# antofuller/jumbo_mae_tpu

Measured on AMD Instinct MI355X. Metric: pretrain images/sec (whole node) ViT-L/16 224 mask75% at 1/2/4/8 MI355X, higher is better.
Workload: dtype bf16; 1 GPU; model=vit_large_patch16 jumbo-MAE (3 CLS, shared jumbo MLP) + decoder 8x512x16h, global_batch=4096, seq_len=52, decoder_seq_len=199, parallelism=dp1, per_gpu_batch=4096, grad_accum=2, micro_batch=2048, grad_ckpt=False, hip_graph=False, optimizer=adamw(0.9,0.95) wd0.05 warmup-cosine

## Files before the change

jumbo_mae_tpu_amd/csrc/bindings.cpp:

```cpp
#include <torch/extension.h>
#include <c10/hip/HIPStream.h>
#include <hip/hip_runtime.h>

#include <climits>

#include "jm_api.h"

namespace {

hipStream_t stream() { return c10::hip::getCurrentHIPStream().stream(); }

#define CHECK_CUDA(x) TORCH_CHECK((x).is_cuda(), #x " must be a GPU tensor")
#define CHECK_CONTIG(x) TORCH_CHECK((x).is_contiguous(), #x " must be contiguous")
#define CHECK_DT(x, d) TORCH_CHECK((x).scalar_type() == (d), #x " has wrong dtype")

const uint16_t* bf(const torch::Tensor& t) { return reinterpret_cast<const uint16_t*>(t.data_ptr()); }
uint16_t* bfm(torch::Tensor& t) { return reinterpret_cast<uint16_t*>(t.data_ptr()); }
uint16_t* bfp(const torch::Tensor& t) { return reinterpret_cast<uint16_t*>(t.data_ptr()); }
const float* fopt(const c10::optional<torch::Tensor>& t) {
  return t.has_value() && t->defined() ? t->data_ptr<float>() : nullptr;
}
float* fopt_m(c10::optional<torch::Tensor>& t) { return t.has_value() && t->defined() ? t->data_ptr<float>() : nullptr; }

void check_rc(int rc, const char* what) { TORCH_CHECK(rc == 0, what, ": unsupported shape (rc=", rc, ")"); }
// ... 40 lines not shown
  return {y, mean, rstd};
}

std::vector<torch::Tensor> layernorm_bwd(torch::Tensor dy, torch::Tensor x, torch::Tensor mean, torch::Tensor rstd,
                                         torch::Tensor gamma, torch::Tensor dgamma, torch::Tensor dbeta, bool accum,
                                         c10::optional<torch::Tensor> dres, c10::optional<torch::Tensor> out,
                                         c10::optional<torch::Tensor> res_y, c10::optional<torch::Tensor> res_scale,
                                         c10::optional<torch::Tensor> res_mask, c10::optional<torch::Tensor> res_dscale,
                                         c10::optional<torch::Tensor> res_dbias, int64_t res_T0,
                                         c10::optional<torch::Tensor> res_out, c10::optional<torch::Tensor> res_seed,
                                         double res_rate, int64_t res_ioff, c10::optional<torch::Tensor> hx,
                                         c10::optional<torch::Tensor> beta) {
  CHECK_CONTIG(dy);
  TORCH_CHECK(x.dim() == 3 && x.stride(2) == 1, "x must be [B,T,D]");
  const int B = x.size(0), T = x.size(1), D = x.size(2);
  TORCH_CHECK(dy.numel() == (long)B * T * D, "dy shape");
  torch::Tensor dx;
  if (out.has_value() && out->defined()) {
    dx = *out;
    TORCH_CHECK(dx.dim() == 3 && dx.size(0) == B && dx.size(1) == T && dx.size(2) == D && dx.stride(2) == 1, "out view");
  } else {
    dx = torch::empty({B, T, D}, x.options());
  }
  const float* rp = nullptr;
  long rB = 0, rT = 0;
  if (dres.has_value() && dres->defined()) {
    TORCH_CHECK(dres->dim() == 3 && dres->size(0) == B && dres->size(1) == T && dres->stride(2) == 1, "dres view");
    rp = dres->data_ptr<float>();
    rB = dres->stride(0);
    rT = dres->stride(1);
  }
  const bool dyb = dy.scalar_type() == torch::kBFloat16;
  TORCH_CHECK(dyb || dy.scalar_type() == torch::kFloat32, "dy dtype");
  const bool has_res = res_y.has_value() && res_y->defined();
  JmLnRes res{};
  torch::Tensor dyr;
  if (has_res) {
    const int Tr = T - (int)res_T0;
    TORCH_CHECK(res_T0 >= 0 && Tr > 0, "res_T0");
    const auto& y = *res_y;
    CHECK_DT(y, torch::kBFloat16);
    long yB, yT;
    if (y.dim() == 3) {
      TORCH_CHECK(y.size(0) == B && y.size(1) == Tr && y.size(2) == D && y.stride(2) == 1, "res_y view");
      yB = y.stride(0);
      yT = y.stride(1);
    } else {
      TORCH_CHECK(y.is_contiguous() && y.numel() == (long)B * Tr * D, "res_y shape");
      yB = (long)Tr * D;
      yT = D;
    }
    if (res_out.has_value() && res_out->defined()) {
      dyr = *res_out;
      CHECK_DT(dyr, torch::kBFloat16);
      TORCH_CHECK(dyr.sizes() == y.sizes() && dyr.strides() == y.strides(), "res_out must match res_y's view");
    } else {
      TORCH_CHECK(y.is_contiguous(), "res_y view needs res_out");
      dyr = torch::empty_like(y);
    }
    res = JmLnRes{bf(y), bfm(dyr), yB, yT, fopt(res_scale), fopt(res_mask), (int)res_T0, fopt_m(res_dscale),
                  fopt_m(res_dbias), make_drop(res_seed, res_rate, y, res_ioff)};
  }
  const uint16_t* hxp = nullptr;
  const float* betap = nullptr;
  if (hx.has_value() && hx->defined()) {
    CHECK_DT((*hx), torch::kBFloat16);
    CHECK_CONTIG((*hx));
    TORCH_CHECK(hx->numel() == (long)B * T * D, "hx shape");
    TORCH_CHECK(beta.has_value() && beta->defined() && beta->numel() == D, "hx needs beta [D]");
    CHECK_DT((*beta), torch::kFloat32);
    hxp = bf(*hx);
    betap = beta->data_ptr<float>();
  }
  const int NP = has_res ? 4 : 2;
  auto ws = torch::empty({(accum || has_res) ? (long)jm_layernorm_bwd_blocks(B * T, D) * NP * D : 1}, x.options());
  check_rc(jm_layernorm_bwd(dy.data_ptr(), dyb, x.data_ptr<float>(), x.stride(0), x.stride(1), B, T, D,
                            mean.data_ptr<float>(), rstd.data_ptr<float>(), gamma.data_ptr<float>(),
                            dx.data_ptr<float>(), dx.stride(0), dx.stride(1), rp, rB, rT, dgamma.data_ptr<float>(),
                            dbeta.data_ptr<float>(), accum, ws.data_ptr<float>(), has_res ? &res : nullptr,
                            stream(), hxp, betap),
           "layernorm_bwd");
  if (has_res) return {dx, dyr};
  return {dx};
}

torch::Tensor gelu_fwd(torch::Tensor h) {
  CHECK_CONTIG(h);
  CHECK_DT(h, torch::kBFloat16);
  auto a = torch::empty_like(h);
  check_rc(jm_gelu_fwd(bf(h), bfm(a), h.numel(), stream()), "gelu_fwd");
  return a;
}

static torch::Tensor rowcol_ws(const torch::Tensor& like, int M, int N, int nacc) {
  const long n = jm_rowcol_ws_floats(M, N, nacc);
  return torch::empty({n > 0 ? n : 1}, like.options().dtype(torch::kFloat32));
}

torch::Tensor gelu_bwd(torch::Tensor h, torch::Tensor da, c10::optional<torch::Tensor> bias_grad, bool deriv) {
  CHECK_CONTIG(h);
  CHECK_CONTIG(da);
  CHECK_DT(h, torch::kBFloat16);
  CHECK_DT(da, torch::kBFloat16);
  const int N = h.size(-1);
  const int M = h.numel() / N;
  auto dh = torch::empty_like(h);
  float* bg = fopt_m(bias_grad);
  torch::Tensor ws;
  if (bg) ws = rowcol_ws(h, M, N, 1);
  check_rc(jm_gelu_bwd(bf(h), bf(da), bfm(dh), bg, M, N, stream(), deriv ? 1 : 0, bg ? ws.data_ptr<float>() : nullptr),
           "gelu_bwd");
  return dh;
}

void colsum(torch::Tensor x, torch::Tensor acc) {
  CHECK_CONTIG(x);
  CHECK_DT(x, torch::kBFloat16);
  const int N = x.size(-1);
  const int M = x.numel() / N;
  auto ws = rowcol_ws(x, M, N, 1);
  check_rc(jm_colsum_bf16(bf(x), acc.data_ptr<float>(), M, N, stream(), ws.data_ptr<float>()), "colsum");
}

void splitk_reduce_add(torch::Tensor part, torch::Tensor g) {
  CHECK_CONTIG(part);
  TORCH_CHECK(g.is_contiguous() && g.numel() * part.size(0) == part.numel(), "splitk_reduce_add shapes");
  check_rc(jm_splitk_reduce_add(part.data_ptr<float>(), g.data_ptr<float>(), g.numel(), part.size(0), stream()),
           "splitk_reduce_add");
}

void colsum_add_f32(torch::Tensor x, torch::Tensor g) {
  CHECK_CUDA(x);
  CHECK_DT(x, torch::kFloat32);
  CHECK_DT(g, torch::kFloat32);
  TORCH_CHECK(x.dim() == 2 && x.stride(1) == 1 && g.is_contiguous() && g.numel() == x.size(1),
              "colsum_add_f32: x [rows, n] with unit column stride, g [n]");
  TORCH_CHECK(reinterpret_cast<uintptr_t>(x.data_ptr()) % 16 == 0 && reinterpret_cast<uintptr_t>(g.data_ptr()) % 16 == 0,
              "colsum_add_f32: 16-byte aligned operands");
  check_rc(jm_colsum_add_f32(x.data_ptr<float>(), x.stride(0), x.size(0), x.size(1), g.data_ptr<float>(), stream()),
           "colsum_add_f32");
}

torch::Tensor residual_fwd(torch::Tensor x, torch::Tensor y, c10::optional<torch::Tensor> scale,
                           c10::optional<torch::Tensor> mask, c10::optional<torch::Tensor> out_opt,
                           c10::optional<torch::Tensor> seed, double rate, int64_t ioff) {
  TORCH_CHECK(x.dim() == 3 && x.stride(2) == 1, "x must be [B,T,D]");
  CHECK_DT(x, torch::kFloat32);
  CHECK_CONTIG(y);
  CHECK_DT(y, torch::kBFloat16);
  const int B = x.size(0), T = x.size(1), D = x.size(2);
  torch::Tensor out;
  if (out_opt.has_value() && out_opt->defined()) {
    out = *out_opt;
    TORCH_CHECK(out.dim() == 3 && out.size(0) == B && out.size(1) == T && out.size(2) == D && out.stride(2) == 1,
                "out view");
  } else {
    out = torch::empty({B, T, D}, x.options());
  }
  check_rc(jm_residual_fwd(x.data_ptr<float>(), x.stride(0), x.stride(1), B, T, D, bf(y), fopt(scale), fopt(mask),
                           out.data_ptr<float>(), out.stride(0), out.stride(1), stream(),
                           make_drop(seed, rate, y, ioff)),
           "residual_fwd");
  return out;
}

torch::Tensor residual_bwd(torch::Tensor dout, c10::optional<torch::Tensor> y, c10::optional<torch::Tensor> scale,
// ... 311 lines not shown
  CHECK_CONTIG(y);
  CHECK_DT(y, torch::kBFloat16);
  CHECK_CONTIG(tok);
  CHECK_CONTIG(pos);
  CHECK_DT(tok, torch::kFloat32);
  CHECK_DT(pos, torch::kFloat32);
  const long sb = ids_bstride(ids_restore);
  const int B = y.size(0), d = y.size(2), K = y.size(1) - C, N = pos.size(0);
  TORCH_CHECK(ids_restore.size(-1) == N && tok.numel() == d && pos.size(1) == d, "unshuffle_fwd shapes");
  auto out = torch::empty({B, C + N, d}, y.options().dtype(torch::kFloat32));
  check_rc(jm_unshuffle_fwd(bfp(y), tok.data_ptr<float>(), ids_restore.data_ptr<int>(), sb, pos.data_ptr<float>(),
                            out.data_ptr<float>(), B, C, K, N, d, stream()),
           "unshuffle_fwd");
  return out;
}

void zero_f32(torch::Tensor t) {
  CHECK_CUDA(t);
  CHECK_CONTIG(t);
  CHECK_DT(t, torch::kFloat32);
  jm_zero_f32(t.data_ptr<float>(), t.numel(), stream());
}

std::vector<torch::Tensor> mask_ids(torch::Tensor noise, int64_t keep) {
  CHECK_CUDA(noise);
  CHECK_CONTIG(noise);
  CHECK_DT(noise, torch::kFloat32);
  TORCH_CHECK(noise.dim() == 1 || noise.dim() == 2, "mask_ids: noise [N] or [R, N]");
  const int N = noise.size(-1), R = noise.dim() == 1 ? 1 : noise.size(0);
  TORCH_CHECK(N <= 1024 && keep >= 0 && keep <= N, "mask_ids: N <= 1024, 0 <= keep <= N");
  auto i64 = noise.options().dtype(torch::kInt64), i32 = noise.options().dtype(torch::kInt32);
  auto shuffle = torch::empty(noise.sizes(), i64), restore = torch::empty(noise.sizes(), i64);
  auto restore32 = torch::empty(noise.sizes(), i32), mask = torch::empty(noise.sizes(), noise.options());
  auto ks = noise.sizes().vec();
  ks.back() = keep;
  auto keep32 = torch::empty(ks, i32);
  check_rc(jm_mask_ids(noise.data_ptr<float>(), R, N, (int)keep, shuffle.data_ptr<int64_t>(),
                       restore.data_ptr<int64_t>(), keep32.data_ptr<int>(), restore32.data_ptr<int>(),
                       mask.data_ptr<float>(), stream()),
           "mask_ids");
  return {shuffle, restore, keep32, restore32, mask};
}

std::vector<torch::Tensor> unshuffle_bwd(torch::Tensor dout, torch::Tensor ids_restore, int64_t C, int64_t K) {
  CHECK_CONTIG(dout);
  CHECK_DT(dout, torch::kFloat32);
  const long sb = ids_bstride(ids_restore);
  const int B = dout.size(0), N = dout.size(1) - C, d = dout.size(2);
  TORCH_CHECK(ids_restore.size(-1) == N, "unshuffle_bwd shapes");
  const int rpb = 64;
  const int nb = jm_unshuffle_bwd_blocks(B, C, N, rpb);
  auto dy = torch::empty({B, C + K, d}, dout.options().dtype(torch::kBFloat16));
  auto part = torch::empty({nb, d}, dout.options().dtype(torch::kFloat64));
  check_rc(jm_unshuffle_bwd(dout.data_ptr<float>(), ids_restore.data_ptr<int>(), sb, bfp(dy), part.data_ptr<double>(), B,
                            C, K, N, d, rpb, stream()),
           "unshuffle_bwd");
  return {dy, part.sum(0, true).to(torch::kFloat32)};
}

torch::Tensor mix_patches(torch::Tensor img, c10::optional<torch::Tensor> perm, c10::optional<torch::Tensor> prm,
                          c10::optional<torch::Tensor> box, int64_t p) {
  CHECK_CONTIG(img);
  CHECK_DT(img, torch::kUInt8);
  TORCH_CHECK(img.size(1) == 3, "mix_patches: 3 channels");
  const int B = img.size(0), H = img.size(2), W = img.size(3);
  const int* pp = nullptr;
  const float* pr = nullptr;
  const int* bx = nullptr;
  if (prm) {
    TORCH_CHECK(perm && box, "mix_patches: prm needs perm and box");
    CHECK_DT((*perm), torch::kInt32);
    CHECK_DT((*prm), torch::kFloat32);
    CHECK_DT((*box), torch::kInt32);
    TORCH_CHECK(perm->numel() == B && prm->numel() >= 2 && box->numel() == 4, "mix_patches: param sizes");
    pp = perm->data_ptr<int>();
    pr = prm->data_ptr<float>();
    bx = box->data_ptr<int>();
  }
  auto out = torch::empty({(long)B * (H / p) * (W / p), 3 * p * p}, img.options().dtype(torch::kBFloat16));
  check_rc(jm_mix_patches(img.data_ptr<uint8_t>(), pp, pr, bx, bfp(out), B, H, W, p, stream()), "mix_patches");
  return out;
}

torch::Tensor patch_mse_fwd(torch::Tensor pred, torch::Tensor img, int64_t p, bool norm_pix) {
  CHECK_DT(pred, torch::kBFloat16);
  TORCH_CHECK(pred.stride(1) == 1, "pred rows must be contiguous");
  CHECK_CONTIG(img);
  CHECK_DT(img, torch::kUInt8);
  const int H = img.size(2), W = img.size(3), N = (H / p) * (W / p);
  TORCH_CHECK(pred.size(0) == img.size(0) * N && pred.size(1) == 3 * p * p, "patch_mse_fwd shapes");
  auto mse = torch::empty({pred.size(0)}, pred.options().dtype(torch::kFloat32));
  check_rc(jm_patch_mse_fwd(bfp(pred), pred.stride(0), img.data_ptr<uint8_t>(), mse.data_ptr<float>(), pred.size(0), N,
                            H, W, p, norm_pix, stream()),
           "patch_mse_fwd");
  return mse;
}

torch::Tensor patch_mse_bwd(torch::Tensor pred, torch::Tensor img, torch::Tensor dmse, int64_t p, bool norm_pix) {
  CHECK_DT(pred, torch::kBFloat16);
  TORCH_CHECK(pred.stride(1) == 1, "pred rows must be contiguous");
  CHECK_CONTIG(img);
  CHECK_CONTIG(dmse);
  CHECK_DT(dmse, torch::kFloat32);
  const int H = img.size(2), W = img.size(3), N = (H / p) * (W / p);
  TORCH_CHECK(dmse.numel() == pred.size(0) && pred.size(0) == img.size(0) * N && pred.size(1) == 3 * p * p,
              "patch_mse_bwd shapes");
  auto dpred = torch::empty({pred.size(0), pred.size(1)}, pred.options());
  check_rc(jm_patch_mse_bwd(bfp(pred), pred.stride(0), img.data_ptr<uint8_t>(), dmse.data_ptr<float>(), bfp(dpred),
                            pred.size(0), N, H, W, p, norm_pix, stream()),
           "patch_mse_bwd");
  return dpred;
}

std::vector<torch::Tensor> recon(torch::Tensor pred, torch::Tensor images, torch::Tensor mask, int64_t p, bool norm_pix,
                                 int64_t fill, c10::optional<std::vector<torch::Tensor>> out) {
  CHECK_CUDA(pred);
  CHECK_CUDA(images);
  CHECK_CUDA(mask);
  TORCH_CHECK(images.device() == pred.device() && mask.device() == pred.device(), "recon: tensors on one device");
  TORCH_CHECK(pred.scalar_type() == torch::kBFloat16 || pred.scalar_type() == torch::kFloat32,
              "recon: pred must be bf16 or fp32");
  CHECK_DT(images, torch::kUInt8);
  CHECK_DT(mask, torch::kFloat32);
  CHECK_CONTIG(pred);
  CHECK_CONTIG(images);
  CHECK_CONTIG(mask);
  TORCH_CHECK(pred.dim() == 2, "recon: pred [B*N, 3p^2]");
  TORCH_CHECK(images.dim() == 4 && images.size(1) == 3, "recon: images [B, 3, H, W]");
  TORCH_CHECK(fill >= 0 && fill <= 255, "recon: fill is a byte");
  const int64_t B = images.size(0), H = images.size(2), W = images.size(3);
  TORCH_CHECK(p > 0 && p % 2 == 0, "recon: patch size must be positive and even, got ", p);
  TORCH_CHECK(H > 0 && W > 0 && H % p == 0 && W % p == 0, "recon: image ", H, " x ", W,
              " is not a whole number of ", p, " x ", p, " patches");
  TORCH_CHECK(H <= INT_MAX && W <= INT_MAX && B <= INT_MAX, "recon: image batch too large");
  const int64_t N = (H / p) * (W / p);
  TORCH_CHECK(B * N <= INT_MAX, "recon: too many patches");
  TORCH_CHECK(pred.size(0) == B * N && pred.size(1) == 3 * p * p, "recon: pred must be [", B * N, ", ", 3 * p * p,
              "], got [", pred.size(0), ", ", pred.size(1), "]");
  TORCH_CHECK((mask.dim() == 1 && mask.size(0) == N) || (mask.dim() == 2 && mask.size(0) == B && mask.size(1) == N),
              "recon: mask must be [", N, "] or [", B, ", ", N, "]");
  const long maskB = mask.dim() == 1 ? 0 : (long)N;
  torch::Tensor rec, paste, masked, err;
  if (out.has_value()) {
    TORCH_CHECK(out->size() == 4, "recon: out = (recon, paste, masked, err)");
    for (int i = 0; i < 3; ++i) {
      const auto& t = (*out)[i];
      TORCH_CHECK(t.is_cuda() && t.device() == pred.device() && t.scalar_type() == torch::kUInt8 &&
                      t.is_contiguous() && t.sizes() == images.sizes(),
                  "recon: out[", i, "] must be a contiguous uint8 tensor shaped like images");
    }
    const auto& e = (*out)[3];
    TORCH_CHECK(e.is_cuda() && e.device() == pred.device() && e.scalar_type() == torch::kFloat32 &&
                    e.is_contiguous() && e.dim() == 2 && e.size(0) == B && e.size(1) == N,
                "recon: out[3] must be a contiguous fp32 [B, N] tensor");
    rec = (*out)[0], paste = (*out)[1], masked = (*out)[2], err = e;
  } else {
    rec = torch::empty_like(images);
    paste = torch::empty_like(images);
    masked = torch::empty_like(images);
    err = torch::empty({B, N}, images.options().dtype(torch::kFloat32));
  }
  check_rc(jm_recon(pred.data_ptr(), pred.scalar_type() == torch::kBFloat16, images.data_ptr<uint8_t>(),
                    mask.data_ptr<float>(), maskB, rec.data_ptr<uint8_t>(), paste.data_ptr<uint8_t>(),
                    masked.data_ptr<uint8_t>(), err.data_ptr<float>(), (int)B, (int)H, (int)W, (int)p, norm_pix,
                    (int)fill, stream()),
           "recon");
  return {rec, paste, masked, err};
}

}

int attach_tail(GemmEpi& ep, torch::Tensor& ws, int M, int N, int K, int epi, const torch::Tensor& like) {
  int r = 0;
  long n = 0;
  const int S = jm_gemm_nt_tail_plan(M, N, K, epi, like.stride(0), &r, &n);
  if (S < 2) return 0;
  ws = torch::empty({n}, like.options().dtype(torch::kFloat32));
  ep.tail = ws.data_ptr<float>();
  ep.tail_S = S;
  ep.t_count = r;
  return r;
}

std::vector<torch::Tensor> gemm_nt(torch::Tensor A, torch::Tensor B, c10::optional<torch::Tensor> bias, bool gelu,
                                   bool gelu_only, bool gelu_deriv, c10::optional<torch::Tensor> seed, double rate) {
  CHECK_DT(A, torch::kBFloat16);
  CHECK_DT(B, torch::kBFloat16);
  TORCH_CHECK(A.dim() == 2 && B.dim() == 2 && A.size(1) == B.size(1), "gemm_nt: A [M,K], B [N,K]");
  TORCH_CHECK(A.stride(1) == 1 && B.stride(1) == 1, "gemm_nt: K must be contiguous");
  const int M = A.size(0), N = B.size(0), K = A.size(1);
  TORCH_CHECK(!gelu_deriv || N % 8 == 0, "gemm_nt: gelu_deriv needs N % 8 == 0");
  auto out = torch::empty({M, N}, gelu_deriv ? A.options().dtype(torch::kUInt8) : A.options());
// ... 372 lines not shown
  segs.n = nb;
  int S = 1;
  const int sps = jm_gemm_tn_plan(grp, M, &S);
  torch::Tensor part;
  if (S > 1) part = torch::empty({S * total}, gs[0].options());
  int64_t off = 0;
  for (int p = 0; p < np; ++p) {
    grp.out[p] = S > 1 ? part.data_ptr<float>() + off : gs[p].data_ptr<float>();
    off += (int64_t)S * grp.N[p] * grp.K[p];
  }
  const int all_store = group_stores(stores, gs, S, np);
  check_rc(jm_gemm_tn(grp, segmented ? &segs : nullptr, M, sps, S, stream(), all_store), what);
  if (S > 1)
    for (int p = 0; p < np; ++p)
      check_rc(jm_splitk_reduce_add(grp.out[p], gs[p].data_ptr<float>(), (long)grp.N[p] * grp.K[p], S, stream(),
                                    p < (int)stores.size() && stores[p]),
               what);
  return S;
}

int64_t gemm_tn_wgrad(torch::Tensor dy, torch::Tensor x, torch::Tensor g, bool store) {
  return tn_wgrad("gemm_tn_wgrad", {Tensors{dy}}, {Tensors{x}}, {g}, {store}, false);
}

int64_t gemm_tn_wgrad_seg(Tensors dys, Tensors xs, torch::Tensor g, bool store) {
  return tn_wgrad("gemm_tn_wgrad_seg", {dys}, {xs}, {g}, {store}, true);
}

int64_t gemm_tn_wgrad_group(Tensors dys, Tensors xs, Tensors gs, std::vector<bool> stores) {
  std::vector<Tensors> d, x;
  for (const auto& t : dys) d.push_back({t});
  for (const auto& t : xs) x.push_back({t});
  return tn_wgrad("gemm_tn_wgrad_group", d, x, gs, stores, false);
}

int64_t gemm_tn_wgrad_seg_group(std::vector<Tensors> dys, std::vector<Tensors> xs, Tensors gs,
                                std::vector<bool> stores) {
  return tn_wgrad("gemm_tn_wgrad_seg_group", dys, xs, gs, stores, true);
}

void zero_ranges(torch::Tensor base, torch::Tensor desc, int64_t blocks) {
  CHECK_CONTIG(base);
  CHECK_DT(base, torch::kFloat32);
  TORCH_CHECK(desc.is_cuda() && desc.scalar_type() == torch::kInt64 && desc.dim() == 2 && desc.size(1) == 2,
              "zero_ranges: desc int64 [n, 2] on the device");
  check_rc(jm_zero_ranges(base.data_ptr<float>(), reinterpret_cast<const long long*>(desc.data_ptr<int64_t>()),
                          (int)desc.size(0), blocks, stream()),
           "zero_ranges");
}

std::vector<torch::Tensor> residual_ln_fwd(torch::Tensor x, torch::Tensor y, c10::optional<torch::Tensor> scale,
                                           c10::optional<torch::Tensor> mask, torch::Tensor gamma,
                                           torch::Tensor beta, double eps, int64_t T0, int64_t R0,
                                           c10::optional<torch::Tensor> out, c10::optional<torch::Tensor> seed,
                                           double rate) {
  CHECK_CUDA(x);
  TORCH_CHECK(x.dim() == 3 && x.stride(2) == 1, "x must be [B,T,D] with contiguous last dim");
  CHECK_DT(x, torch::kFloat32);
  CHECK_DT(y, torch::kBFloat16);
  CHECK_CONTIG(y);
  const int B = x.size(0), T = x.size(1), D = x.size(2);
  TORCH_CHECK(R0 >= 0 && R0 < T, "residual_ln_fwd: R0");
  TORCH_CHECK(y.numel() == (long)B * (T - R0) * D, "residual_ln_fwd: y must be [B*(T-R0), D]");
  TORCH_CHECK(T0 >= 0 && T0 < T, "residual_ln_fwd: T0");
  TORCH_CHECK(R0 == 0 || out.has_value(), "residual_ln_fwd: R0 > 0 needs out (its rows t < R0 are inputs)");
  torch::Tensor x1;
  if (out) {
    CHECK_DT(*out, torch::kFloat32);
    TORCH_CHECK(out->dim() == 3 && out->size(0) == B && out->size(1) == T && out->size(2) == D && out->stride(2) == 1,
                "residual_ln_fwd: out must be [B,T,D] with contiguous last dim");
    x1 = *out;
  } else {
    x1 = torch::empty({B, T, D}, x.options());
  }
  const long R = (long)B * (T - T0);
  auto h = torch::empty({R, D}, y.options());
  auto mean = torch::empty({R}, x.options());
  auto rstd = torch::empty({R}, x.options());
  check_rc(jm_residual_ln_fwd(x.data_ptr<float>(), x.stride(0), x.stride(1), bf(y), fopt(scale), fopt(mask),
                              x1.data_ptr<float>(), x1.stride(0), x1.stride(1), bfm(h), mean.data_ptr<float>(),
                              rstd.data_ptr<float>(), B, T, T0, D, gamma.data_ptr<float>(), beta.data_ptr<float>(),
                              (float)eps, stream(), (int)R0, make_drop(seed, rate, y, 0)),
           "residual_ln_fwd");
  return {x1, h, mean, rstd};
}

static std::pair<const int*, const float*> check_cls_loss(const torch::Tensor& logits, const torch::Tensor& labels,
                                                          const c10::optional<torch::Tensor>& perm,
                                                          const c10::optional<torch::Tensor>& w, double smoothing,
                                                          int64_t mode) {
  CHECK_CUDA(logits);
  TORCH_CHECK(logits.scalar_type() == torch::kBFloat16 || logits.scalar_type() == torch::kFloat32,
              "cls_loss: logits must be bf16 or fp32");
  TORCH_CHECK(logits.dim() == 2 && logits.size(0) >= 1 && logits.size(1) >= 1, "cls_loss: logits must be [B, L]");
  TORCH_CHECK(logits.stride(1) == 1, "cls_loss: logits must have a unit column stride");
  TORCH_CHECK(logits.size(0) == 1 || logits.stride(0) >= logits.size(1), "cls_loss: logits rows must not overlap");
  TORCH_CHECK(logits.size(0) < INT_MAX && logits.size(1) < INT_MAX, "cls_loss: logits too large");
  const int64_t B = logits.size(0);
  TORCH_CHECK(labels.device() == logits.device() && labels.scalar_type() == torch::kInt64 && labels.dim() == 1 &&
                  labels.size(0) == B && labels.is_contiguous(),
              "cls_loss: labels must be int64 [B] on the logits' device");
  TORCH_CHECK(mode == 0 || mode == 1, "cls_loss: mode 0 (ce) or 1 (bce)");
  TORCH_CHECK(smoothing >= 0.0 && smoothing < 1.0, "cls_loss: smoothing must be in [0, 1)");
  const bool hp = perm.has_value() && perm->defined(), hw = w.has_value() && w->defined();
  TORCH_CHECK(hp == hw, "cls_loss: perm and w come together");
  if (!hp) return {nullptr, nullptr};
  TORCH_CHECK(perm->device() == logits.device() && perm->scalar_type() == torch::kInt32 && perm->dim() == 1 &&
                  perm->size(0) == B && perm->is_contiguous(),
              "cls_loss: perm must be int32 [B] on the logits' device");
  TORCH_CHECK(w->device() == logits.device() && w->scalar_type() == torch::kFloat32 && w->numel() == 1,
              "cls_loss: w must be one fp32 element on the logits' device");
  return {perm->data_ptr<int>(), w->data_ptr<float>()};
}

static long row_stride(const torch::Tensor& logits) { return logits.size(0) == 1 ? logits.size(1) : logits.stride(0); }

std::vector<torch::Tensor> cls_loss_fwd(torch::Tensor logits, torch::Tensor labels, c10::optional<torch::Tensor> perm,
                                        c10::optional<torch::Tensor> w, double smoothing, int64_t mode) {
  const auto pw = check_cls_loss(logits, labels, perm, w, smoothing, mode);
  const int64_t B = logits.size(0);
  auto loss = torch::empty({B}, logits.options().dtype(torch::kFloat32));
  auto hit = torch::empty({B, 2}, logits.options().dtype(torch::kBool));
  auto lse = torch::empty({B, 2}, logits.options().dtype(torch::kFloat32));
  check_rc(jm_cls_loss_fwd(logits.data_ptr(), logits.scalar_type() == torch::kBFloat16, row_stride(logits),
                           labels.data_ptr<int64_t>(), pw.first, pw.second, smoothing, (int)mode, (int)B,
                           (int)logits.size(1), loss.data_ptr<float>(), reinterpret_cast<uint8_t*>(hit.data_ptr()),
                           lse.data_ptr<float>(), stream()),
           "cls_loss_fwd");
  return {loss, hit, lse};
}

torch::Tensor cls_loss_bwd(torch::Tensor dloss, torch::Tensor logits, torch::Tensor labels,
                           c10::optional<torch::Tensor> perm, c10::optional<torch::Tensor> w, double smoothing,
                           int64_t mode, torch::Tensor lse) {
  const auto pw = check_cls_loss(logits, labels, perm, w, smoothing, mode);
  const int64_t B = logits.size(0), L = logits.size(1);
  TORCH_CHECK(lse.device() == logits.device() && lse.scalar_type() == torch::kFloat32 && lse.dim() == 2 &&
                  lse.size(0) == B && lse.size(1) == 2 && lse.is_contiguous(),
              "cls_loss_bwd: lse must be the forward's fp32 [B, 2]");
  TORCH_CHECK(dloss.device() == logits.device() && dloss.scalar_type() == torch::kFloat32 && dloss.dim() == 1 &&
                  dloss.size(0) == B && dloss.is_contiguous(),
              "cls_loss_bwd: dloss must be fp32 [B] on the logits' device");
  auto dlogits = torch::empty({B, L}, logits.options());
  check_rc(jm_cls_loss_bwd(logits.data_ptr(), logits.scalar_type() == torch::kBFloat16, row_stride(logits),
                           labels.data_ptr<int64_t>(), pw.first, pw.second, smoothing, (int)mode, (int)B, (int)L,
                           lse.data_ptr<float>(), dloss.data_ptr<float>(), dlogits.data_ptr(), L, stream()),
           "cls_loss_bwd");
  return dlogits;
}

static void check_bn_mat(const torch::Tensor& t, const char* fn, const char* what, bool bf16_ok) {
  TORCH_CHECK(t.scalar_type() == torch::kFloat32 || (bf16_ok && t.scalar_type() == torch::kBFloat16), fn, ": ", what,
              bf16_ok ? " must be bf16 or fp32" : " must be fp32");
  TORCH_CHECK(t.dim() == 2 && t.size(0) >= 1 && t.size(1) >= 1, fn, ": ", what, " must be [B, J]");
  TORCH_CHECK(t.stride(1) == 1, fn, ": ", what, " must have a unit column stride");
  TORCH_CHECK(t.size(0) == 1 || t.stride(0) >= t.size(1), fn, ": ", what, " rows must not overlap");
  TORCH_CHECK(t.size(0) < INT_MAX && t.size(1) < INT_MAX, fn, ": ", what, " too large");
}

static void check_bn_like(const torch::Tensor& t, const torch::Tensor& x, const char* fn, const char* what,
                          bool bf16_ok) {
  check_bn_mat(t, fn, what, bf16_ok);
  TORCH_CHECK(t.size(0) == x.size(0) && t.size(1) == x.size(1), fn, ": ", what, " must have the shape of x");
}

static void check_bn_vec(const torch::Tensor& t, int64_t n, const char* fn, const char* what, const char* shape) {
// ... 303 lines not shown
  m.def("rrc_resize", &rrc_resize, py::arg("src"), py::arg("tab"), py::arg("size"), py::arg("tmp_bytes"),
        py::arg("tmp_rows_max"));
  m.def("rrc_kmax", &jm_rrc_kmax);
  m.def("window_resize", &window_resize, py::arg("src"), py::arg("tab"), py::arg("size"), py::arg("tmp_bytes"),
        py::arg("tmp_rows_max"));
  m.def("window_tab", &jm_window_tab);
  m.def("aug_chain", &aug_chain, py::arg("images"), py::arg("chain"), py::arg("scratch"));
  m.def("augmix_mix", &augmix_mix, py::arg("orig"), py::arg("chains"), py::arg("table"), py::arg("blended"));
  m.def("erase_paste", &erase_paste, py::arg("images"), py::arg("table"), py::arg("fill"),
        py::arg("box_bytes_max") = 0);
  m.def("gelu_drop", &gelu_drop, py::arg("a"), py::arg("b") = py::none(), py::arg("seed"), py::arg("rate"));
  m.def("softmax_dropout_fwd", &softmax_dropout_fwd);
  m.def("softmax_dropout_bwd", &softmax_dropout_bwd);
  m.def("gelu_bwd", &gelu_bwd, py::arg("h"), py::arg("da"), py::arg("bias_grad") = py::none(),
        py::arg("deriv") = false);
  m.def("colsum", &colsum);
  m.def("splitk_reduce_add", &splitk_reduce_add);
  m.def("residual_ln_fwd", &residual_ln_fwd, py::arg("x"), py::arg("y"), py::arg("scale"), py::arg("mask"),
        py::arg("gamma"), py::arg("beta"), py::arg("eps"), py::arg("T0"), py::arg("R0") = 0,
        py::arg("out") = py::none(), py::arg("seed") = py::none(), py::arg("rate") = 0.0);
  m.def("transpose_bf16", &transpose_bf16);
  m.def("residual_fwd", &residual_fwd, py::arg("x"), py::arg("y"), py::arg("scale"), py::arg("mask"),
        py::arg("out") = py::none(), py::arg("seed") = py::none(), py::arg("rate") = 0.0, py::arg("ioff") = 0);
  m.def("residual_bwd", &residual_bwd, py::arg("dout"), py::arg("y"), py::arg("scale"), py::arg("mask"),
        py::arg("dscale"), py::arg("ydtype"), py::arg("dbias") = py::none(), py::arg("out") = py::none(),
        py::arg("seed") = py::none(), py::arg("rate") = 0.0, py::arg("ioff") = 0);
  m.def("attn_fwd", &attn_fwd, py::arg("qkv"), py::arg("heads"), py::arg("seed") = py::none(), py::arg("rate") = 0.0);
  m.def("attn_bwd", &attn_bwd, py::arg("dO"), py::arg("qkv"), py::arg("o"), py::arg("lse"), py::arg("heads"),
        py::arg("dbias") = py::none(), py::arg("seed") = py::none(), py::arg("rate") = 0.0);
  m.def("attn_max_seq", &jm_attn_max_seq);
  m.def("attn_head_dims", &attn_head_dims);
  m.def("attn_fused_bias", &attn_fused_bias, py::arg("S"), py::arg("hd"));
  m.def("attn_dropout", &attn_dropout, py::arg("S"), py::arg("hd"));
  m.def("gemm_tn_wgrad", &gemm_tn_wgrad, py::arg("dy"), py::arg("x"), py::arg("g"), py::arg("store") = false);
  m.def("gemm_tn_wgrad_seg", &gemm_tn_wgrad_seg, py::arg("dys"), py::arg("xs"), py::arg("g"), py::arg("store") = false);
  m.def("zero_ranges", &zero_ranges, "zero float ranges of a flat buffer (one launch)");
  m.def("colsum_add_f32", &colsum_add_f32, "g += x.sum(0) for a row-strided fp32 [rows, n] view");
  m.def("gemm_tn_wgrad_seg_group", &gemm_tn_wgrad_seg_group, py::arg("dys"), py::arg("xs"), py::arg("gs"),
        py::arg("stores") = std::vector<bool>{}, "grouped segmented weight gradients (<= 2 problems)");
  m.def("gemm_tn_wgrad_group", &gemm_tn_wgrad_group, py::arg("dys"), py::arg("xs"), py::arg("gs"),
        py::arg("stores") = std::vector<bool>{}, "grouped weight gradients over one M (<= 4 problems)");
  m.def("gemm_test_force", &jm_gemm_test_force, py::arg("path"), py::arg("rows") = 0,
        "numerics tests only: NT GEMM kernel path 0 = by shape, 1 = 64-deep main loop everywhere, "
        "2 = 4-phase kernels at every M without tail split (rows = forced tile height)");
  m.def("gemm_nt_tiles", &jm_gemm_nt_tiles, py::arg("M"), py::arg("N"), py::arg("K") = 1024, py::arg("epi") = 0,
        py::arg("lda") = 0, "output tiles (workgroups before split-K) of an NT launch");
  m.def(
      "gemm_nt_tail_plan",
      [](int M, int N, int K, int epi, long lda) {
        int r = 0;
        long n = 0;
        const int S = jm_gemm_nt_tail_plan(M, N, K, epi, lda, &r, &n);
        return std::make_pair(S, r);
      },
      py::arg("M"), py::arg("N"), py::arg("K"), py::arg("epi") = 0, py::arg("lda") = 0,
      "(S, tail tiles) of the tail split of an NT launch (S = 0: none); read-only");
  m.def("transpose_bf16_batch", &transpose_bf16_batch);
  m.def("gemm_nt_splitk", &gemm_nt_splitk, py::arg("A"), py::arg("B"), py::arg("bias") = py::none(),
        py::arg("splits") = 8, py::arg("add") = py::none());
  m.def("gemm_nt_dgelu", &gemm_nt_dgelu, py::arg("A"), py::arg("B"), py::arg("pre"), py::arg("dbias") = py::none(),
        py::arg("deriv") = false, py::arg("rate") = 0.0);
  m.def("gemm_nt_f32", &gemm_nt_f32, py::arg("A"), py::arg("B"));
  m.def("gemm_nt", &gemm_nt, py::arg("A"), py::arg("B"), py::arg("bias") = py::none(), py::arg("gelu") = false,
        py::arg("gelu_only") = false, py::arg("gelu_deriv") = false, py::arg("seed") = py::none(),
        py::arg("rate") = 0.0);
  m.def("opt_sumsq", &opt_sumsq);
  m.def("opt_adamw", &opt_adamw);
  m.def("opt_lamb_phase1", &opt_lamb_phase1);
  m.def("opt_lars_norms", &opt_lars_norms);
  m.def("opt_apply_trust", &opt_apply_trust);
  m.def("opt_sgd", &opt_sgd);
  m.def("opt_ema", &opt_ema, py::arg("master"), py::arg("ema"), py::arg("rows"), py::arg("meta"),
        py::arg("ema_hyper"));
  m.def("ema_swap", &ema_swap, py::arg("master"), py::arg("ema"), py::arg("shadow"), py::arg("rows"));
  m.def("opt_seg_stats", &opt_seg_stats, py::arg("master"), py::arg("grad"), py::arg("p_old"), py::arg("rows"),
        py::arg("meta"), py::arg("out") = py::none());
  m.def("patchify_normalize", &patchify_normalize);
  m.def("gather_patches", &gather_patches);
  m.def("embed_finish", &embed_finish);
  m.def("zero_f32", &zero_f32, "fp32 zero fill kernel (the store-mode gradients' pre-reduce fill)");
  m.def("mask_ids", &mask_ids, "random-masking permutation ids + mask from noise (one workgroup per row)");
  m.def("unshuffle_fwd", &unshuffle_fwd);
  m.def("unshuffle_bwd", &unshuffle_bwd);
  m.def("patch_mse_fwd", &patch_mse_fwd);
  m.def("mix_patches", &mix_patches);
  m.def("patch_mse_bwd", &patch_mse_bwd);
  m.def("recon", &recon, py::arg("pred"), py::arg("images"), py::arg("mask"), py::arg("p"), py::arg("norm_pix"),
        py::arg("fill") = 127, py::arg("out") = py::none(),
        "MAE reconstruction panels -> (recon, paste, masked uint8 [B, 3, H, W], err fp32 [B, N])");
  m.def("cls_loss_fwd", &cls_loss_fwd, py::arg("logits"), py::arg("labels"), py::arg("perm") = py::none(),
        py::arg("w") = py::none(), py::arg("smoothing") = 0.0, py::arg("mode") = 0);
  m.def("cls_loss_bwd", &cls_loss_bwd, py::arg("dloss"), py::arg("logits"), py::arg("labels"),
        py::arg("perm"), py::arg("w"), py::arg("smoothing"), py::arg("mode"), py::arg("lse"));
  m.def("knn_topk", &knn_topk, py::arg("q"), py::arg("bank"), py::arg("k"), py::arg("self_idx") = py::none(),
        py::arg("splits") = 0, py::arg("out_idx") = py::none(), py::arg("out_sim") = py::none(),
        "fused similarity + top-k -> (idx int32, sim fp32) [Nq, k], ties by ascending bank index");
  m.def("knn_splits", &jm_knn_splits, py::arg("Nq"), py::arg("Nb"), py::arg("splits") = 0,
        "bank slices of a knn_topk launch");
  m.def("knn_vote", &knn_vote, py::arg("idx"), py::arg("sim"), py::arg("bank_labels"), py::arg("labels"), py::arg("T"),
        "weighted k-NN vote -> (pred int32 [Nq, 5], hit1, hit5 bool [Nq])");
  m.def("bn_stats", &bn_stats, py::arg("x"));
  m.def("bn_apply", &bn_apply, py::arg("x"), py::arg("packed"), py::arg("gamma"), py::arg("beta"),
        py::arg("running_mean"), py::arg("running_var"), py::arg("eps"), py::arg("momentum"), py::arg("out_dtype"),
        py::arg("out") = py::none());
  m.def("bn_apply_eval", &bn_apply_eval, py::arg("x"), py::arg("running_mean"), py::arg("running_var"),
        py::arg("gamma"), py::arg("beta"), py::arg("eps"), py::arg("out_dtype"), py::arg("out") = py::none());
  m.def("bn_bwd_reduce", &bn_bwd_reduce, py::arg("dy"), py::arg("x"), py::arg("stats"), py::arg("gamma"),
        py::arg("dgamma") = py::none(), py::arg("dbeta") = py::none());
  m.def("bn_bwd_dx", &bn_bwd_dx, py::arg("dy"), py::arg("x"), py::arg("stats"), py::arg("gamma"), py::arg("packed_g"),
        py::arg("n"), py::arg("out") = py::none());
  m.def("bn_chunk_rows", &jm_bn_chunk_rows, "rows per workgroup of the BatchNorm kernels");
  m.def("bn_block_cols", &jm_bn_block_cols, "columns per workgroup of the BatchNorm kernels");
  m.def("attn_stats", &attn_stats, py::arg("qkv"), py::arg("heads"), py::arg("n_cls"),
        py::arg("rows_out") = py::none(), "per-head attention statistics, fp64 [H, 6]");
  m.def("debug_lines", &debug_lines);
  m.def("debug_selftest", &debug_selftest);
#ifdef JM_DEBUG
  m.attr("debug_build") = true;
#else
  m.attr("debug_build") = false;
#endif
}
```

jumbo_mae_tpu_amd/csrc/jm_api.h:

```cpp
#pragma once
#include <cstddef>
#include <cstdint>

#include <hip/hip_runtime.h>

struct JmDrop {
  const int64_t* seed;
  uint32_t thr;
  float scale;
  long ioff;
};

struct JmLnRes {
  const uint16_t* y;
  uint16_t* dy;
  long yB, yT;
  const float* scale;
  const float* mask;
  int T0;
  float* dscale;
  float* dbias;
  JmDrop drop;
};

struct TnGroup {
  const uint16_t* a[4];
  const uint16_t* b[4];
  long lda[4], ldb[4];
  int N[4], K[4];
  float* out[4];
  int tile0[5];
  int n;
};

struct TnSegs {
  const uint16_t* a[64];
  const uint16_t* b[64];
  int rows;
  int n;
};

struct GemmEpi {
  const float* bias;
  uint16_t* out;
  long ldo;
  uint16_t* out2;
  const uint16_t* aux;
  float* colpart;
  float* part;
  int splits;
  float* tail;
  int tail_S;
  int t_begin;
  int t_count;
  const int64_t* dseed;
  uint32_t dthr;
  float dscale;
  uint8_t* dq;
  const uint8_t* dqa;
  float dqs;
};


int jm_layernorm_fwd(const float* x, long sB, long sT, int B, int T, int D, const float* gamma, const float* beta,
                     float eps, void* y, int out_bf16, float* mean, float* rstd, hipStream_t st, uint16_t* y2 = nullptr);
int jm_layernorm_bwd(const void* dy, int dy_bf16, const float* x, long sB, long sT, int B, int T, int D,
                     const float* mean, const float* rstd, const float* gamma, float* dx_ptr, long oB, long oT,
                     const float* dres, long rB, long rT, float* dgamma, float* dbeta, int accum_params, float* ws,
                     const JmLnRes* res, hipStream_t st, const uint16_t* hx = nullptr,
                     const float* beta = nullptr);
int jm_layernorm_bwd_blocks(int rows, int D);
int jm_residual_ln_fwd(const float* x, long sB, long sT, const uint16_t* y, const float* scale, const float* mask,
                       float* x1, long oB, long oT, uint16_t* h, float* mean, float* rstd, int B, int T, int T0,
                       int D, const float* gamma, const float* beta, float eps, hipStream_t st, int R0 = 0,
                       JmDrop drop = JmDrop{nullptr, 0u, 1.f, 0});
int jm_debug_line_layernorm();

int jm_gelu_fwd(const uint16_t* h, uint16_t* a, long n, hipStream_t st);
long jm_rowcol_ws_floats(int M, int N, int nacc);
int jm_gelu_bwd(const uint16_t* h, const uint16_t* da, uint16_t* dh, float* bias_grad, int M, int N, hipStream_t st,
                int deriv, float* ws);
int jm_colsum_bf16(const uint16_t* x, float* acc, int M, int N, hipStream_t st, float* ws);
int jm_residual_fwd(const float* x, long sB, long sT, int B, int T, int D, const uint16_t* y, const float* scale,
                    const float* mask, float* out, long oB, long oT, hipStream_t st, JmDrop drop);
int jm_residual_bwd(const float* dout, long dB, long dT, const uint16_t* y, const float* scale, const float* mask,
                    float* dscale, uint16_t* dy, int B, int T, int D, float* dbias, long yB, long yT, hipStream_t st,
                    JmDrop drop, float* ws);
void jm_zero_f32(float* p, long n, hipStream_t st);
int jm_splitk_reduce_add(const float* part, float* g, long n, int S, hipStream_t st, int store = 0);
int jm_colsum_add_f32(const float* x, long ld, int rows, long n, float* g, hipStream_t st);
int jm_zero_ranges(float* base, const long long* desc, int n, long long blocks, hipStream_t st);
int jm_transpose_bf16(const uint16_t* src, uint16_t* dst, int R, int C, hipStream_t st);
int jm_transpose_bf16_batch(const long long* desc, int n, int tiles, hipStream_t st);
int jm_splitk_reduce_bf16(const float* part, int S, long n, int N, const float* bias, uint16_t* out, hipStream_t st);
int jm_splitk_reduce_f32(const float* part, int S, int M, int N, const float* bias, const float* add, long add_ld,
                         float* out, hipStream_t st);
int jm_debug_line_elementwise();
void jm_debug_selftest(int v, hipStream_t st);

int jm_attn_fwd(const uint16_t* qkv, uint16_t* o, float* lse, int B, int S, int H, int hd, const int64_t* dseed,
                uint32_t dthr, float dscale, hipStream_t st);
int jm_attn_bwd(const uint16_t* qkv, const uint16_t* o, const uint16_t* dO, const float* lse, uint16_t* dqkv, int B,
                int S, int H, int hd, float* dbias_part, const int64_t* dseed, uint32_t dthr, float dscale,
                hipStream_t st);
int jm_attn_bwd_long(const uint16_t* qkv, const uint16_t* o, const uint16_t* dO, const float* lse, uint16_t* dqkv,
                     float* delta, int B, int S, int H, int hd, const int64_t* dseed, uint32_t dthr, float dscale,
                     hipStream_t st);
int jm_attn_max_seq();
int jm_attn_head_dims(const int** dims);
int jm_attn_tiled(int S, int hd);
int jm_attn_fused_bias(int S, int hd);
int jm_attn_bwd_part_rows(int B, int S, int hd);
int jm_attn_dropout(int S, int hd);
int jm_debug_line_attention();

void jm_opt_sumsq(const float* x, const int* chunks, int nchunks, float* out, float* cpart, hipStream_t st);
void jm_opt_adamw(float* p, const float* g, float* mu, float* nu, uint16_t* shadow, const int* chunks, int nchunks,
                  const float* meta, const float* hyper, const float* gnorm_sq, hipStream_t st);
void jm_opt_lamb_phase1(const float* p, const float* g, float* mu, float* nu, float* u, const int* chunks, int nchunks,
                        const float* meta, const float* hyper, const float* gnorm_sq, float* norms, float* cpart,
                        hipStream_t st);
void jm_opt_lars_norms(const float* p, const float* g, const int* chunks, int nchunks, const float* hyper,
                       const float* gnorm_sq, float* norms, float* cpart, hipStream_t st);
void jm_opt_apply_trust(float* p, const float* u_or_g, float* trace, uint16_t* shadow, const int* chunks, int nchunks,
                        const float* meta, const float* hyper, const float* norms, const float* gnorm_sq, int mode,
                        float momentum, float trust_coef, hipStream_t st);
void jm_opt_sgd(float* p, const float* g, float* trace, uint16_t* shadow, const int* chunks, int nchunks,
                const float* meta, const float* hyper, const float* gnorm_sq, float momentum, hipStream_t st);
void jm_opt_ema(const float* p, float* ema, const int* chunks, int nchunks, const float* meta, int nseg,
                const float* ema_hyper, long n, hipStream_t st);
void jm_ema_swap(float* p, float* ema, uint16_t* shadow, const int* chunks, int nchunks, long n, hipStream_t st);
constexpr int JM_SEG_STATS_COLS = 7;
void jm_opt_seg_stats(const float* p, const float* g, const float* p_old, const int* chunks, int nchunks,
                      const float* meta, int nseg, long n, double* part, double* out, hipStream_t st);
int jm_debug_line_optim();

int jm_patchify_normalize(const uint8_t* img, float* out, int B, int H, int W, int p, hipStream_t st);
int jm_gather_patches(const uint8_t* img, const int* ids, long idsB, uint16_t* out, int B, int K, int H, int W, int p,
                      hipStream_t st);
int jm_embed_finish(const uint16_t* e, const float* pos, const int* ids, long idsB, const float* cls, float* out,
                    int B, int C, int K, int D, hipStream_t st);
int jm_mask_ids(const float* noise, int R, int N, int keep, int64_t* shuffle, int64_t* restore, int* keep32,
                int* restore32, float* mask, hipStream_t st);
int jm_unshuffle_fwd(const uint16_t* y, const float* tok, const int* restore, long rsB, const float* pos, float* out,
                     int B, int C, int K, int N, int d, hipStream_t st);
int jm_unshuffle_bwd_blocks(int B, int C, int N, int rows_per_block);
int jm_unshuffle_bwd(const float* dout, const int* restore, long rsB, uint16_t* dy, double* part, int B, int C, int K,
                     int N, int d, int rows_per_block, hipStream_t st);
int jm_mix_patches(const uint8_t* img, const int* perm, const float* prm, const int* box, uint16_t* out, int B, int H,
                   int W, int p, hipStream_t st);
int jm_patch_mse_fwd(const uint16_t* pred, long ldp, const uint8_t* img, float* mse, long rows, int N, int H, int W,
                     int p, int norm_pix, hipStream_t st);
int jm_patch_mse_bwd(const uint16_t* pred, long ldp, const uint8_t* img, const float* dmse, uint16_t* dpred, long rows,
                     int N, int H, int W, int p, int norm_pix, hipStream_t st);
int jm_debug_line_mae();

int jm_recon(const void* pred, int pred_bf16, const uint8_t* img, const float* mask, long maskB, uint8_t* recon,
             uint8_t* paste, uint8_t* masked, float* err, int B, int H, int W, int p, int norm_pix, int fill,
             hipStream_t st);
int jm_debug_line_recon();

int jm_gemm_nt(const uint16_t* A, long lda, const uint16_t* B, long ldb, int M, int N, int K, int epi,
               const GemmEpi& ep, hipStream_t st);
int jm_gemm_nt_tiles(int M, int N, int K, int epi, long lda);
int jm_gemm_nt_colpart_rows(int M, int N, int K, int epi, long lda);
int jm_gemm_nt_tail_plan(int M, int N, int K, int epi, long lda, int* tail_r, long* ws_floats);
void jm_gemm_test_force(int path, int rows);
int jm_debug_line_gemm();

size_t jm_gemm_tn_smem();
int jm_gemm_tn_plan(const TnGroup& grp, int M, int* S_out);
int jm_gemm_tn(const TnGroup& grp, const TnSegs* segs, int M, int sps, int S, hipStream_t st, int store);
int jm_debug_line_gemm_tn();

int jm_dropout_apply(const void* x, void* y, long n, int bf16, const int64_t* seed, uint32_t thr, float scale,
                     hipStream_t st);
int jm_gelu_drop(const uint16_t* h, uint16_t* g, uint16_t* gp, long n, const int64_t* seed, uint32_t thr, float scale,
                 hipStream_t st);
int jm_softmax_dropout_fwd(const float* z, float* p, float* pd, long rows, int S, const int64_t* seed, uint32_t thr,
                           float scale, hipStream_t st);
int jm_softmax_dropout_bwd(const float* dpd, const float* p, float* dz, long rows, int S, const int64_t* seed,
                           uint32_t thr, float scale, hipStream_t st);
int jm_debug_line_dropout();

int jm_rrc_resize(const uint8_t* src, const int64_t* tab, int B, int S, uint8_t* tmp, int tmp_rows_max, uint8_t* out,
                  hipStream_t st);
int jm_window_resize(const uint8_t* src, const int64_t* tab, int B, int S, uint8_t* tmp, int tmp_rows_max,
                     uint8_t* out, hipStream_t st);
int jm_window_tab();
int jm_rrc_kmax();
int jm_debug_line_augment();

int jm_aug_stat_words();
int jm_aug_record_len();
int jm_aug_chain(uint8_t* images, uint8_t* scratch, const double* chain, int B, int slots, int S, uint32_t* stats,
                 hipStream_t st);
int jm_augmix_mix(const uint8_t* orig, const uint8_t* chains, const float* table, uint8_t* out, int B, int W, int S,
                  int blended, hipStream_t st);
int jm_erase_paste(uint8_t* images, const int64_t* table, const uint8_t* fill, long fill_len, int B, int S,
                   long box_bytes_max, hipStream_t st);
int jm_debug_line_augment_chain();

int jm_cls_loss_fwd(const void* logits, int bf16, long ld, const int64_t* labels, const int* perm, const float* w,
                    double smoothing, int mode, int B, int L, float* loss, uint8_t* hit, float* lse, hipStream_t st);
int jm_cls_loss_bwd(const void* logits, int bf16, long ld, const int64_t* labels, const int* perm, const float* w,
                    double smoothing, int mode, int B, int L, const float* lse, const float* dloss, void* dlogits,
                    long ldo, hipStream_t st);
int jm_debug_line_loss();

int jm_bn_chunks(int B);
int jm_bn_chunk_rows();
int jm_bn_block_cols();
int jm_bn_stats(const float* x, long ld, int B, int J, double* part, float* packed, hipStream_t st);
int jm_bn_apply(const float* x, long ld, int B, int J, const float* packed, const float* gamma, const float* beta,
                double eps, double momentum, void* y, int y_bf16, long ldy, float* stats, float* running_mean,
                float* running_var, hipStream_t st);
int jm_bn_apply_eval(const float* x, long ld, int B, int J, const float* running_mean, const float* running_var,
                     const float* gamma, const float* beta, double eps, void* y, int y_bf16, long ldy,
                     hipStream_t st);
int jm_bn_bwd_reduce(const void* dy, int dy_bf16, long lddy, const float* x, long ld, int B, int J,
                     const float* stats, const float* gamma, double* part, float* dgamma, float* dbeta, int accum,
                     float* packed_g, hipStream_t st);
int jm_bn_bwd_dx(const void* dy, int dy_bf16, long lddy, const float* x, long ld, int B, int J, const float* stats,
                 const float* gamma, const float* packed_g, double n, float* dx, long lddx, hipStream_t st);
int jm_debug_line_batchnorm();

int jm_knn_splits(int Nq, int Nb, int splits);
int jm_knn_topk(const void* q, long ldq, const void* bank, long ldb, const int* self_idx, int Nq, int Nb, int D, int k,
                int splits, int* idx, float* sim, int* sidx, float* ssim, hipStream_t st);
int jm_knn_vote(const int* idx, const float* sim, const int* bank_labels, const int* labels, double T, int Nq, int Nb,
                int k, int* pred, uint8_t* hit1, uint8_t* hit5, hipStream_t st);
int jm_debug_line_knn();

constexpr int JM_ATTN_STATS_COLS = 6;
long jm_attn_stats_part(int B, int S, int H);
int jm_attn_stats(const void* qkv, int B, int S, int H, int hd, int n_cls, double* part, float* rows_out,
                  hipStream_t st);
// ... 3 lines not shown
```

jumbo_mae_tpu_amd/csrc/layernorm.hip:

```cpp
#include <type_traits>

#include "common.h"
#include "jm_api.h"

namespace {

template <int V, typename TO>
__global__ __launch_bounds__(256) void ln_fwd_kernel(const float* __restrict__ x, long sB, long sT, int T,
                                                     int rows, int D, const float* __restrict__ gamma,
                                                     const float* __restrict__ beta, float eps,
                                                     TO* __restrict__ y, float* __restrict__ mean_out,
                                                     float* __restrict__ rstd_out, uint16_t* __restrict__ y2) {
  const int wave = threadIdx.x >> 6, lane = threadIdx.x & 63;
  const int row = blockIdx.x * 4 + wave;
  if (row >= rows) return;
  const int b = row / T, t = row - b * T;
  const float* xr = x + b * sB + t * sT;
  float v[V][4];
  float s = 0.f;
#pragma unroll
  for (int i = 0; i < V; ++i) {
    const int col = (i * 64 + lane) * 4;
    if (col < D) {
      load4(xr + col, v[i]);
// ... 48 lines not shown
  float* mean;
  float* rstd;
  DropIO drop;
};

template <int V>
__global__ __launch_bounds__(256) void res_ln_fwd_kernel(ResLnIO io, int T, int T0, int R0, int rows, int D,
                                                         const float* __restrict__ gamma,
                                                         const float* __restrict__ beta, float eps) {
  const int wave = threadIdx.x >> 6, lane = threadIdx.x & 63;
  const int row = blockIdx.x * 4 + wave;
  if (row >= rows) return;
  const int b = row / T, t = row - b * T;
  const bool rrow = t >= R0;
  float* x1r = io.x1 + b * io.oB + t * io.oT;
  const float* xr = rrow ? io.x + b * io.sB + t * io.sT : x1r;
  const uint16_t* yr = io.y + ((long)b * (T - R0) + (t - R0)) * D;
  const float m = io.mask ? io.mask[b] : 1.f;
  float v[V][4];
  float s = 0.f;
#pragma unroll
  for (int i = 0; i < V; ++i) {
    const int col = (i * 64 + lane) * 4;
    if (col < D) {
      float xv[4];
      load4(xr + col, xv);
      if (rrow) {
        float yv[4], sc[4] = {1.f, 1.f, 1.f, 1.f};
        load4(yr + col, yv);
        if (io.scale) load4(io.scale + col, sc);
        if (io.drop.seed) {
          float f[4];
          drop_factors<4>(io.drop, io.drop.ioff + (yr - io.y) + col, f);
#pragma unroll
          for (int j = 0; j < 4; ++j) yv[j] *= f[j];
        }
#pragma unroll
        for (int j = 0; j < 4; ++j) v[i][j] = xv[j] + m * sc[j] * yv[j];
        store4(x1r + col, v[i]);
      } else {
#pragma unroll
        for (int j = 0; j < 4; ++j) v[i][j] = xv[j];
      }
    } else {
      v[i][0] = v[i][1] = v[i][2] = v[i][3] = 0.f;
    }
    s += v[i][0] + v[i][1] + v[i][2] + v[i][3];
  }
  if (t < T0) return;
  const float mean = wave_sum(s) / D;
  float s2 = 0.f;
#pragma unroll
  for (int i = 0; i < V; ++i) {
    const int col = (i * 64 + lane) * 4;
    if (col < D) {
#pragma unroll
      for (int j = 0; j < 4; ++j) {
        const float d = v[i][j] - mean;
        s2 += d * d;
      }
    }
  }
  const float rstd = rsqrtf(wave_sum(s2) / D + eps);
  const long hrow = (long)b * (T - T0) + (t - T0);
  uint16_t* hr = io.h + hrow * D;
#pragma unroll
  for (int i = 0; i < V; ++i) {
    const int col = (i * 64 + lane) * 4;
    if (col < D) {
      float gg[4], bb[4], o[4];
      load4(gamma + col, gg);
      load4(beta + col, bb);
#pragma unroll
      for (int j = 0; j < 4; ++j) o[j] = (v[i][j] - mean) * rstd * gg[j] + bb[j];
      store4(hr + col, o);
    }
  }
  if (lane == 0) {
    io.mean[hrow] = mean;
    io.rstd[hrow] = rstd;
  }
}

struct LnBwdIO {
  float* dx;
  long oB, oT;
  const float* dres;
  long rB, rT;
  const uint16_t* hx;
  const float* beta;
};

JM_DEVICE bool ln_h_ok(float g, float b) { return fabsf(g) >= 1e-20f && fabsf(b) <= fabsf(g); }

struct LnResIO {
  const uint16_t* y;
  uint16_t* dy;
  long yB, yT;
  const float* scale;
  const float* mask;
  int T0;
  DropIO drop;
};

struct ParamOuts {
  float* p[4];
};

template <int V, typename TI, bool RES, bool ER = false, bool SC = true, int R = 1>
__global__ __launch_bounds__(256) void ln_bwd_kernel(const TI* __restrict__ dy, const float* __restrict__ x,
                                                     long sB, long sT, int T, int rows, int D,
                                                     const float* __restrict__ mean, const float* __restrict__ rstd,
                                                     const float* __restrict__ gamma, LnBwdIO io, LnResIO rio,
                                                     float* __restrict__ ws, int accum_params, ParamOuts outs) {
  JM_DGUARD(blockDim.x == 256 && D % 4 == 0 && D <= V * 256);
  static_assert(R == 1 || R == 2, "rows per wave");
  constexpr int NP = RES ? 4 : 2;
  constexpr int LPR = 64 / R, VL = V * R;
  extern __shared__ __attribute__((aligned(16))) float red[];
  const int wave = threadIdx.x >> 6, lane = threadIdx.x & 63;
  const int sub = lane / LPR, l = lane % LPR;
  const bool partials = accum_params || RES;
  auto acc_add = [&](float (&acc)[NP][VL][4], int k, int i, int j, float v) { acc[k][i][j] += v; };
  auto row_sum = [&](float v) {
    if constexpr (R == 1) {
      return wave_sum(v);
    } else {
      v = row16_sum(v);
      const int iv = __builtin_bit_cast(int, v);
      const float lo = __builtin_bit_cast(float, __builtin_amdgcn_readlane(iv, 0)) +
                       __builtin_bit_cast(float, __builtin_amdgcn_readlane(iv, 16));
      const float hi = __builtin_bit_cast(float, __builtin_amdgcn_readlane(iv, 32)) +
                       __builtin_bit_cast(float, __builtin_amdgcn_readlane(iv, 48));
      return sub ? hi : lo;
    }
  };
  float acc[NP][VL][4], gg[VL][4], sc[VL][4];
  float* hbi = red + (partials ? NP * D : 0);
  const bool use_h = io.hx != nullptr;
  uint32_t xchunk = 0;
#pragma unroll
  for (int i = 0; i < VL; ++i) {
    const int col = (i * LPR + l) * 4;
#pragma unroll
    for (int j = 0; j < 4; ++j) {
#pragma unroll
      for (int k = 0; k < NP; ++k) acc[k][i][j] = 0.f;
      sc[i][j] = 1.f;
    }
    if (col < D) {
      load4(gamma + col, gg[i]);
      if constexpr (RES && SC) {
        if (rio.scale) load4(rio.scale + col, sc[i]);
      }
      if (use_h) {
        float bb[4], ig[4];
        load4(io.beta + col, bb);
        bool ok = true;
#pragma unroll
        for (int j = 0; j < 4; ++j) {
          ok = ok && ln_h_ok(gg[i][j], bb[j]);
          ig[j] = 1.f / gg[i][j];
        }
        if (!ok) xchunk |= 1u << i;
        if (wave == 0 && sub == 0) {
          store4(hbi + col, bb);
          store4(hbi + D + col, ig);
        }
      }
    }
  }
  const bool hpath = use_h && !__syncthreads_or(xchunk != 0u);
  auto row_loop = [&](auto hp) {
    constexpr bool HP = decltype(hp)::value;
    for (int rw = blockIdx.x * 4 + wave; rw * R < rows; rw += gridDim.x * 4) {
      const int row = rw * R + sub;
      const bool valid = R == 1 || row < rows;
      const int b = row / T, t = row - b * T;
      const float* xr = x + b * sB + t * sT;
      const TI* dyr = dy + (long)row * D;
      const float mu = valid ? mean[row] : 0.f, rs = valid ? rstd[row] : 0.f;
      const bool rrow = RES && t >= rio.T0;
      const long yoff = RES ? b * rio.yB + (long)(t - rio.T0) * rio.yT : 0;
      float xh[VL][4], g[VL][4], yv[VL][4];
      float rvp[ER ? VL : 1][4];
      const float* rr = io.dres ? io.dres + b * io.rB + t * io.rT : nullptr;
      float sg = 0.f, sgx = 0.f;
      if constexpr (HP) {
        const uint16_t* hr = io.hx + (long)row * D;
#pragma unroll
        for (int i = 0; i < VL; ++i) {
          const int col = (i * LPR + l) * 4;
          if (valid && col < D) load4(hr + col, xh[i]);
        }
      } else {
#pragma unroll
        for (int i = 0; i < VL; ++i) {
          const int col = (i * LPR + l) * 4;
          if (valid && col < D) load4(xr + col, xh[i]);
        }
      }
#pragma unroll
      for (int i = 0; i < VL; ++i) {
        const int col = (i * LPR + l) * 4;
        if (valid && col < D) {
          float dv[4];
          if constexpr (HP) {
            float bb[4], ig[4];
            load4(hbi + col, bb);
            load4(hbi + D + col, ig);
#pragma unroll
            for (int j = 0; j < 4; ++j) xh[i][j] = (xh[i][j] - bb[j]) * ig[j];
          } else {
#pragma unroll
            for (int j = 0; j < 4; ++j) xh[i][j] = (xh[i][j] - mu) * rs;
          }
          load4(dyr + col, dv);
          if constexpr (RES && SC) {
            if (rrow && rio.scale) load4(rio.y + yoff + col, yv[i]);
          }
          if constexpr (ER) {
            if (rr) load4(rr + col, rvp[i]);
            else rvp[i][0] = rvp[i][1] = rvp[i][2] = rvp[i][3] = 0.f;
          }
#pragma unroll
          for (int j = 0; j < 4; ++j) {
            g[i][j] = dv[j] * gg[i][j];
            sg += g[i][j];
            sgx += g[i][j] * xh[i][j];
            acc_add(acc, 0, i, j, dv[j] * xh[i][j]);
            acc_add(acc, 1, i, j, dv[j]);
          }
        } else {
#pragma unroll
          for (int j = 0; j < 4; ++j) xh[i][j] = g[i][j] = 0.f;
        }
      }
      sg = row_sum(sg) / D;
      sgx = row_sum(sgx) / D;
      float* dxr = io.dx + b * io.oB + t * io.oT;
      const float m = (RES && rio.mask) ? rio.mask[valid ? b : 0] : 1.f;
#pragma unroll
      for (int i = 0; i < VL; ++i) {
        const int col = (i * LPR + l) * 4;
        if (valid && col < D) {
          float o[4], rv[4] = {0.f, 0.f, 0.f, 0.f};
          if constexpr (ER) {
#pragma unroll
            for (int j = 0; j < 4; ++j) rv[j] = rvp[i][j];
          } else if (rr) {
            load4(rr + col, rv);
          }
#pragma unroll
          for (int j = 0; j < 4; ++j) o[j] = rs * (g[i][j] - sg - xh[i][j] * sgx) + rv[j];
          store4(dxr + col, o);
          if (RES && rrow) {
            float d[4], f[4] = {1.f, 1.f, 1.f, 1.f};
            if (rio.drop.seed) drop_factors<4>(rio.drop, rio.drop.ioff + yoff + col, f);
#pragma unroll
            for (int j = 0; j < 4; ++j) {
              const float md = m * o[j] * f[j];
              d[j] = SC ? md * sc[i][j] : md;
              if constexpr (SC) {
                if (rio.scale) acc_add(acc, 2, i, j, md * yv[i][j]);
              }
              acc_add(acc, 3 % NP, i, j, bf2f(f2bf(d[j])));
            }
            store4(rio.dy + yoff + col, d);
          }
        }
      }
    }
  };
  if (hpath) row_loop(std::true_type{});
  else row_loop(std::false_type{});
  if (!partials) return;
  if constexpr (R == 2) {
#pragma unroll
    for (int k = 0; k < NP; ++k)
#pragma unroll
      for (int i = 0; i < VL; ++i)
#pragma unroll
        for (int j = 0; j < 4; ++j) acc[k][i][j] += __shfl_xor(acc[k][i][j], 32, WAVE);
  }
  for (int w = 0; w < 4; ++w) {
    if (wave == w && sub == 0) {
#pragma unroll
      for (int i = 0; i < VL; ++i) {
        const int col = (i * LPR + l) * 4;
        if (col < D) {
#pragma unroll
          for (int k = 0; k < NP; ++k) {
            float a[4] = {0.f, 0.f, 0.f, 0.f};
            if (w > 0) load4(red + k * D + col, a);
#pragma unroll
            for (int j = 0; j < 4; ++j) a[j] += acc[k][i][j];
            store4(red + k * D + col, a);
          }
        }
      }
    }
    __syncthreads();
  }
  for (int i = threadIdx.x * 4; i < NP * D; i += 256 * 4) {
    float a[4];
    load4(red + i, a);
    store4(ws + (long)blockIdx.x * NP * D + i, a);
  }
}

template <int RL>
__global__ __launch_bounds__(256) void ln_param_reduce_kernel(const float* __restrict__ ws, int nb, int D, int NP,
                                                              ParamOuts outs) {
  constexpr int CW = 256 / RL;
  __shared__ float4 red[256];
  const int c = threadIdx.x % CW, rl = threadIdx.x / CW;
  const int i4 = blockIdx.x * CW + c;
  const int n4 = NP * D / 4;
  const long l4 = (long)NP * D / 4;
  float4 acc = make_float4(0.f, 0.f, 0.f, 0.f);
  if (i4 < n4) {
    const float4* p = reinterpret_cast<const float4*>(ws) + i4;
    int b = rl;
    for (; b + 3 * RL < nb; b += 4 * RL) {
      const float4 a0 = p[b * l4], a1 = p[(b + RL) * l4], a2 = p[(b + 2 * RL) * l4], a3 = p[(b + 3 * RL) * l4];
      acc.x += (a0.x + a1.x) + (a2.x + a3.x);
      acc.y += (a0.y + a1.y) + (a2.y + a3.y);
      acc.z += (a0.z + a1.z) + (a2.z + a3.z);
// ... 121 lines not shown
  if (threadIdx.x == 0) {
    mean_out[row] = mean;
    rstd_out[row] = rstd;
  }
}

template <int VW, typename TI>
__global__ __launch_bounds__(256) void ln_bwd_wide_kernel(const TI* __restrict__ dy, const float* __restrict__ x,
                                                          long sB, long sT, int T, int rows, int D,
                                                          const float* __restrict__ mean,
                                                          const float* __restrict__ rstd,
                                                          const float* __restrict__ gamma, LnBwdIO io,
                                                          float* __restrict__ ws, int accum_params) {
  JM_DGUARD(blockDim.x == 256 && D % 4 == 0 && D <= VW * 1024);
  __shared__ float red[4];
  float ag[VW][4], ab[VW][4], gg[VW][4];
#pragma unroll
  for (int i = 0; i < VW; ++i) {
    const int col = (i * 256 + threadIdx.x) * 4;
#pragma unroll
    for (int j = 0; j < 4; ++j) ag[i][j] = ab[i][j] = gg[i][j] = 0.f;
    if (col < D) load4(gamma + col, gg[i]);
  }
  for (int row = blockIdx.x; row < rows; row += gridDim.x) {
    const int b = row / T, t = row - b * T;
    const float* xr = x + b * sB + t * sT;
    const TI* dyr = dy + (long)row * D;
    const float* rr = io.dres ? io.dres + b * io.rB + t * io.rT : nullptr;
    const float mu = mean[row], rs = rstd[row];
    float xh[VW][4], g[VW][4], rv[VW][4];
    float sg = 0.f, sgx = 0.f;
#pragma unroll
    for (int i = 0; i < VW; ++i) {
      const int col = (i * 256 + threadIdx.x) * 4;
#pragma unroll
      for (int j = 0; j < 4; ++j) xh[i][j] = g[i][j] = rv[i][j] = 0.f;
      if (col < D) {
        float xv[4], dv[4];
        load4(xr + col, xv);
        load4(dyr + col, dv);
        if (rr) load4(rr + col, rv[i]);
#pragma unroll
        for (int j = 0; j < 4; ++j) {
          xh[i][j] = (xv[j] - mu) * rs;
          g[i][j] = dv[j] * gg[i][j];
          sg += g[i][j];
          sgx += g[i][j] * xh[i][j];
          ag[i][j] += dv[j] * xh[i][j];
          ab[i][j] += dv[j];
        }
      }
    }
    sg = block_sum256(sg, red) / D;
    sgx = block_sum256(sgx, red) / D;
    float* dxr = io.dx + b * io.oB + t * io.oT;
#pragma unroll
    for (int i = 0; i < VW; ++i) {
      const int col = (i * 256 + threadIdx.x) * 4;
      if (col < D) {
        float o[4];
#pragma unroll
        for (int j = 0; j < 4; ++j) o[j] = rs * (g[i][j] - sg - xh[i][j] * sgx) + rv[i][j];
        store4(dxr + col, o);
      }
    }
  }
  if (!accum_params) return;
#pragma unroll
  for (int i = 0; i < VW; ++i) {
    const int col = (i * 256 + threadIdx.x) * 4;
    if (col < D) {
      store4(ws + (long)blockIdx.x * 2 * D + col, ag[i]);
      store4(ws + (long)blockIdx.x * 2 * D + D + col, ab[i]);
    }
  }
}

constexpr int LN_WIDE_MAX_ROWS = 8192;
int pick_vw(int D) { return D <= 2048 ? 2 : D <= 3072 ? 3 : D <= 4096 ? 4 : -1; }
bool use_wide(int rows, int D) { return D > 1024 && rows <= LN_WIDE_MAX_ROWS && pick_vw(D) > 0; }


#define LN_BWD_R(VV) ((VV) == 2 ? 2 : 1)
template <typename TI, bool RES, bool SC = true>
void launch_bwd(int V, dim3 grid, size_t smem, hipStream_t st, const TI* dy, const float* x, long sB, long sT,
                int T, int rows, int D, const float* m, const float* r, const float* g, LnBwdIO dx, LnResIO rio,
                float* ws, int acc, ParamOuts outs) {
#define JM_LNB(VV)                                                                                          \
  case VV:                                                                                                  \
    ln_bwd_kernel<VV, TI, RES, (VV >= 2 && VV <= 4), SC, LN_BWD_R(VV)><<<grid, 256, smem, st>>>(             \
        dy, x, sB, sT, T, rows, D, m, r, g, dx, rio, ws, acc, outs);                                         \
    break;
  switch (V) {
    JM_LNB(1) JM_LNB(2) JM_LNB(3) JM_LNB(4) JM_LNB(6) JM_LNB(8) JM_LNB(9) JM_LNB(12) JM_LNB(16)
    default: break;
  }
#undef JM_LNB
}

int pick_v(int D) {
  const int need = (D + 255) / 256;
  const int opts[] = {1, 2, 3, 4, 6, 8, 9, 12, 16};
  for (int o : opts)
    if (o >= need) return o;
  return -1;
}

}

int jm_layernorm_fwd(const float* x, long sB, long sT, int B, int T, int D, const float* gamma,
                     const float* beta, float eps, void* y, int out_bf16, float* mean, float* rstd,
                     hipStream_t st, uint16_t* y2) {
  const int V = pick_v(D);
  if (V < 0 || (D % 4) != 0) return -1;
  const int rows = B * T;
  if (use_wide(rows, D)) {
    const int VW = pick_vw(D);
#define JM_LNFW(VV, TO, YP, Y2)                                                                                    \
  case VV:                                                                                                         \
    ln_fwd_wide_kernel<VV, TO><<<rows, 256, 0, st>>>(x, sB, sT, T, rows, D, gamma, beta, eps, YP, mean, rstd, Y2); \
    break;
    if (out_bf16) {
      switch (VW) { JM_LNFW(2, uint16_t, (uint16_t*)y, nullptr) JM_LNFW(3, uint16_t, (uint16_t*)y, nullptr)
                    JM_LNFW(4, uint16_t, (uint16_t*)y, nullptr) default: return -1; }
    } else {
      switch (VW) { JM_LNFW(2, float, (float*)y, y2) JM_LNFW(3, float, (float*)y, y2) JM_LNFW(4, float, (float*)y, y2)
                    default: return -1; }
    }
#undef JM_LNFW
    return 0;
  }
  dim3 grid((rows + 3) / 4);
  if (out_bf16)
    launch_fwd<uint16_t>(V, grid, st, x, sB, sT, T, rows, D, gamma, beta, eps, (uint16_t*)y, mean, rstd, nullptr);
  else
    launch_fwd<float>(V, grid, st, x, sB, sT, T, rows, D, gamma, beta, eps, (float*)y, mean, rstd, y2);
  return 0;
}

int jm_residual_ln_fwd(const float* x, long sB, long sT, const uint16_t* y, const float* scale, const float* mask,
                       float* x1, long oB, long oT, uint16_t* h, float* mean, float* rstd, int B, int T, int T0,
                       int D, const float* gamma, const float* beta, float eps, hipStream_t st, int R0,
                       JmDrop drop) {
  const ResLnIO io{x, sB, sT, y, scale, mask, x1, oB, oT, h, mean, rstd, drop};
  if (R0 < 0 || R0 >= T) return -2;
  const int V = pick_v(D);
  if (V < 0 || (D % 4) != 0) return -1;
  const int rows = B * T;
  dim3 grid((rows + 3) / 4);
#define JM_RLN(VV) \
  case VV: res_ln_fwd_kernel<VV><<<grid, 256, 0, st>>>(io, T, T0, R0, rows, D, gamma, beta, eps); break;
  switch (V) {
    JM_RLN(1) JM_RLN(2) JM_RLN(3) JM_RLN(4) JM_RLN(6) JM_RLN(8) JM_RLN(9) JM_RLN(12) JM_RLN(16)
    default: return -1;
  }
#undef JM_RLN
  return 0;
}

constexpr int LN_BWD_CUS = 256;
int ln_bwd_blocks_per_cu(int V) { return V <= 1 ? 4 : V <= 4 ? 3 : 2; }

int jm_layernorm_bwd_blocks(int rows, int D) {
  if (use_wide(rows, D)) return rows > 1024 ? 1024 : rows;
  const int V = pick_v(D), cap = LN_BWD_CUS * ln_bwd_blocks_per_cu(V < 0 ? 16 : V);
  const int rpb = 4 * LN_BWD_R(V);
  int nb = (rows + rpb - 1) / rpb;
  return nb > cap ? cap : nb;
}

int jm_layernorm_bwd(const void* dy, int dy_bf16, const float* x, long sB, long sT, int B, int T, int D,
                     const float* mean, const float* rstd, const float* gamma, float* dx_ptr, long oB, long oT,
                     const float* dres, long rB, long rT, float* dgamma, float* dbeta, int accum_params, float* ws,
                     const JmLnRes* res, hipStream_t st, const uint16_t* hx, const float* beta) {
  if (hx != nullptr && beta == nullptr) return -3;
  const LnBwdIO dx{dx_ptr, oB, oT, dres, rB, rT, hx, beta};
  const int V = pick_v(D);
  if (V < 0 || (D % 4) != 0) return -1;
  const int rows = B * T;
  const int nb = jm_layernorm_bwd_blocks(rows, D);
  dim3 grid(nb);
  const int NP = res ? 4 : 2;
  const bool partials = accum_params || res;
  if (!res && use_wide(rows, D)) {
    const int VW = pick_vw(D);
#define JM_LNBW(VV, TI)                                                                                     \
  case VV:                                                                                                  \
    ln_bwd_wide_kernel<VV, TI><<<nb, 256, 0, st>>>((const TI*)dy, x, sB, sT, T, rows, D, mean, rstd, gamma, \
                                                   dx, ws, accum_params);                                   \
    break;
    if (dy_bf16) {
      switch (VW) { JM_LNBW(2, uint16_t) JM_LNBW(3, uint16_t) JM_LNBW(4, uint16_t) default: return -1; }
    } else {
      switch (VW) { JM_LNBW(2, float) JM_LNBW(3, float) JM_LNBW(4, float) default: return -1; }
    }
#undef JM_LNBW
    if (accum_params) {
      ParamOuts outs{{dgamma, dbeta, nullptr, nullptr}};
      launch_param_reduce(ws, nb, D, 2, outs, st);
    }
    return 0;
  }
  const size_t smem = ((partials ? NP * D : 0) + (hx ? 2 * D : 0)) * sizeof(float);
  const ParamOuts outs{{accum_params ? dgamma : nullptr, accum_params ? dbeta : nullptr,
                        res ? res->dscale : nullptr, res ? res->dbias : nullptr}};
  float* wsk = ws;
  LnResIO rio{nullptr, nullptr, 0, 0, nullptr, nullptr, 0, JmDrop{nullptr, 0u, 1.f, 0}};
  if (res) rio = LnResIO{res->y, res->dy, res->yB, res->yT, res->scale, res->mask, res->T0, res->drop};
  if (dy_bf16) {
    if (res && res->scale)
      launch_bwd<uint16_t, true>(V, grid, smem, st, (const uint16_t*)dy, x, sB, sT, T, rows, D, mean, rstd, gamma,
                                 dx, rio, wsk, accum_params, outs);
    else if (res)
      launch_bwd<uint16_t, true, false>(V, grid, smem, st, (const uint16_t*)dy, x, sB, sT, T, rows, D, mean, rstd,
                                        gamma, dx, rio, wsk, accum_params, outs);
    else
      launch_bwd<uint16_t, false>(V, grid, smem, st, (const uint16_t*)dy, x, sB, sT, T, rows, D, mean, rstd, gamma,
                                  dx, rio, wsk, accum_params, outs);
  } else {
    if (res && res->scale)
      launch_bwd<float, true>(V, grid, smem, st, (const float*)dy, x, sB, sT, T, rows, D, mean, rstd, gamma, dx, rio,
                              wsk, accum_params, outs);
    else if (res)
      launch_bwd<float, true, false>(V, grid, smem, st, (const float*)dy, x, sB, sT, T, rows, D, mean, rstd, gamma,
                                     dx, rio, wsk, accum_params, outs);
    else
      launch_bwd<float, false>(V, grid, smem, st, (const float*)dy, x, sB, sT, T, rows, D, mean, rstd, gamma, dx, rio,
                               wsk, accum_params, outs);
  }
  if (partials)
    launch_param_reduce(ws, nb, D, NP, outs, st);
  return 0;
}

JM_DEBUG_EXPORT(layernorm)
```

jumbo_mae_tpu_amd/csrc/mae.hip:

```cpp
#include "common.h"
#include "jm_api.h"

namespace {

__constant__ float c_mean[3] = {0.485f, 0.456f, 0.406f};
__constant__ float c_std[3] = {0.229f, 0.224f, 0.225f};

__global__ __launch_bounds__(256) void patchify_kernel(const uint8_t* __restrict__ img, float* __restrict__ out, int H,
                                                       int W, int p, int word) {
  extern __shared__ __attribute__((aligned(16))) uint8_t strip[];
  const int g = W / p;
  const int gh = H / p;
  const int b = blockIdx.x / gh, gy = blockIdx.x - (blockIdx.x / gh) * gh;
  const int W4 = W / 4;
  if (word) {
    for (int i = threadIdx.x; i < 3 * p * W4; i += 256) {
      const int c = i / (p * W4);
      const int rem = i - c * p * W4;
      const int ph = rem / W4, x4 = rem - ph * W4;
      const uint32_t v =
          *reinterpret_cast<const uint32_t*>(img + (((long)b * 3 + c) * H + gy * p + ph) * W + x4 * 4);
      *reinterpret_cast<uint32_t*>(strip + (c * p + ph) * W + x4 * 4) = v;
    }
  } else {
// ... 226 lines not shown
      const int ph = o / (3 * p), r = o - ph * 3 * p;
      const int pw = r / 3, c = r - (r / 3) * 3;
      v = norm_px64(lds[(c * p + ph) * p + pw], c);
    }
    t[j] = v;
  }
  if (norm_pix) {
    double s = 0.0;
#pragma unroll
    for (int j = 0; j < NJ; ++j) s += t[j];
    const double mean = wave_sum_f64(s) / P3;
    double v = 0.0;
#pragma unroll
    for (int j = 0; j < NJ; ++j) {
      const int o = lane + 64 * j;
      const double dlt = o < P3 ? t[j] - mean : 0.0;
      v += dlt * dlt;
    }
    const double rs = 1.0 / sqrt(wave_sum_f64(v) / P3 + 1e-6);
#pragma unroll
    for (int j = 0; j < NJ; ++j) t[j] = (t[j] - mean) * rs;
  }
}

constexpr int P16_PRED = 1, P16_IMG = 2;

JM_DEVICE void p16_load_pred(const uint16_t* __restrict__ pr, float* f, bool vec) {
  if (!vec) {
#pragma unroll
    for (int j = 0; j < 12; ++j) f[j] = bf2f(pr[j]);
    return;
  }
#pragma unroll
  for (int q = 0; q < 3; ++q) {
    const uint2 v = *reinterpret_cast<const uint2*>(pr + 4 * q);
    f[4 * q + 0] = __uint_as_float(v.x << 16);
    f[4 * q + 1] = __uint_as_float(v.x & 0xffff0000u);
    f[4 * q + 2] = __uint_as_float(v.y << 16);
    f[4 * q + 3] = __uint_as_float(v.y & 0xffff0000u);
  }
}

JM_DEVICE void p16_target(const uint8_t* __restrict__ img, long row, int N, int H, int W, bool norm_pix, bool img16,
                          uint8_t* lds, double* t) {
  const int g = W / 16;
  const int b = (int)(row / N), n = (int)(row - (long)b * N);
  const int gy = n / g, gx = n - (n / g) * g;
  const int lane = threadIdx.x & 63;
  const uint8_t* src = img + ((long)b * 3 * H + gy * 16) * W + gx * 16;
  if (img16) {
    if (lane < 48) {
      const int c = lane >> 4, ph = lane & 15;
      *reinterpret_cast<uint4*>(lds + lane * 16) = *reinterpret_cast<const uint4*>(src + ((long)c * H + ph) * W);
    }
  } else {
    for (int i = lane; i < 768; i += 64) lds[i] = src[((long)(i >> 8) * H + ((i >> 4) & 15)) * W + (i & 15)];
  }
  __builtin_amdgcn_wave_barrier();
  __builtin_amdgcn_fence(__ATOMIC_RELEASE, "wavefront");
  __builtin_amdgcn_s_waitcnt(0xc07f);
  __builtin_amdgcn_wave_barrier();
  const int ph = lane >> 2, pw0 = (lane & 3) * 4;
#pragma unroll
  for (int c = 0; c < 3; ++c) {
    const uint32_t px = *reinterpret_cast<const uint32_t*>(lds + (c * 16 + ph) * 16 + pw0);
#pragma unroll
    for (int k = 0; k < 4; ++k)
      t[3 * k + c] = norm_px64((px >> (8 * k)) & 0xffu, c);
  }
  if (norm_pix) {
    double s = 0.0;
#pragma unroll
    for (int j = 0; j < 12; ++j) s += t[j];
    const double mean = wave_sum_f64(s) / 768.0;
    double v = 0.0;
#pragma unroll
    for (int j = 0; j < 12; ++j) v += (t[j] - mean) * (t[j] - mean);
    const double rs = 1.0 / sqrt(wave_sum_f64(v) / 768.0 + 1e-6);
#pragma unroll
    for (int j = 0; j < 12; ++j) t[j] = (t[j] - mean) * rs;
  }
}

template <int NJ, bool P16>
__global__ __launch_bounds__(256) void patch_mse_fwd_kernel(const uint16_t* __restrict__ pred, long ldp,
                                                            const uint8_t* __restrict__ img, float* __restrict__ mse,
                                                            long rows, int N, int H, int W, int p, int norm_pix,
                                                            int vec) {
  const long row = (long)blockIdx.x * 4 + (threadIdx.x >> 6);
  if (row >= rows) return;
  const int P3 = 3 * p * p;
  __shared__ __attribute__((aligned(16))) uint8_t pix[4][64 * NJ];
  double t[NJ];
  const int lane = threadIdx.x & 63;
  if constexpr (P16) {
    float f[12];
    p16_load_pred(pred + row * ldp + 12 * lane, f, vec & P16_PRED);
    p16_target(img, row, N, H, W, norm_pix != 0, vec & P16_IMG, pix[threadIdx.x >> 6], t);
    double s = 0.0;
#pragma unroll
    for (int j = 0; j < 12; ++j) s += (t[j] - (double)f[j]) * (t[j] - (double)f[j]);
    s = wave_sum_f64(s);
    if (lane == 0) mse[row] = (float)(s / 768.0);
    return;
  }
  patch_target<NJ>(img, row, N, H, W, p, P3, norm_pix != 0, pix[threadIdx.x >> 6], t);
  double s = 0.0;
#pragma unroll
  for (int j = 0; j < NJ; ++j) {
    const int o = lane + 64 * j;
    if (o < P3) {
      const double dlt = t[j] - (double)bf2f(pred[row * ldp + o]);
      s += dlt * dlt;
    }
  }
  s = wave_sum_f64(s);
  if (lane == 0) mse[row] = (float)(s / P3);
}

template <int NJ, bool P16>
__global__ __launch_bounds__(256) void patch_mse_bwd_kernel(const uint16_t* __restrict__ pred, long ldp,
                                                            const uint8_t* __restrict__ img,
                                                            const float* __restrict__ dmse, uint16_t* __restrict__ dpred,
                                                            long rows, int N, int H, int W, int p, int norm_pix,
                                                            int vec) {
  const long row = (long)blockIdx.x * 4 + (threadIdx.x >> 6);
  if (row >= rows) return;
  const int P3 = 3 * p * p;
  const int lane = threadIdx.x & 63;
  const float gsc = dmse[row];
  __shared__ __attribute__((aligned(16))) uint8_t pix[4][64 * NJ];
  double t[NJ];
  if constexpr (P16) {
    const bool pv = vec & P16_PRED;
    uint16_t* o1 = dpred + row * 768 + 12 * lane;
    uint2* o = reinterpret_cast<uint2*>(o1);
    if (gsc == 0.f) {
      if (pv) {
#pragma unroll
        for (int q = 0; q < 3; ++q) o[q] = make_uint2(0u, 0u);
      } else {
#pragma unroll
        for (int j = 0; j < 12; ++j) o1[j] = 0;
      }
      return;
    }
    float f[12];
    p16_load_pred(pred + row * ldp + 12 * lane, f, pv);
    p16_target(img, row, N, H, W, norm_pix != 0, vec & P16_IMG, pix[threadIdx.x >> 6], t);
    const double k = 2.0 * (double)gsc / 768.0;
    float r[12];
#pragma unroll
    for (int j = 0; j < 12; ++j) r[j] = (float)(k * ((double)f[j] - t[j]));
    if (pv) {
#pragma unroll
      for (int q = 0; q < 3; ++q)
        o[q] = make_uint2(pack_bf2(r[4 * q], r[4 * q + 1]), pack_bf2(r[4 * q + 2], r[4 * q + 3]));
    } else {
#pragma unroll
      for (int j = 0; j < 12; ++j) o1[j] = f2bf(r[j]);
    }
    return;
  }
  if (gsc == 0.f) {
    for (int o = lane; o < P3; o += 64) dpred[row * P3 + o] = 0;
    return;
  }
  patch_target<NJ>(img, row, N, H, W, p, P3, norm_pix != 0, pix[threadIdx.x >> 6], t);
  const double k = 2.0 * (double)gsc / P3;
#pragma unroll
  for (int j = 0; j < NJ; ++j) {
    const int o = lane + 64 * j;
    if (o < P3) dpred[row * P3 + o] = f2bf((float)(k * ((double)bf2f(pred[row * ldp + o]) - t[j])));
  }
}

inline int cdiv(long a, long b) { return (int)((a + b - 1) / b); }

}

int jm_gather_patches(const uint8_t* img, const int* ids, long idsB, uint16_t* out, int B, int K, int H, int W, int p,
                      hipStream_t st) {
  if ((3 * p * p) % 4 || H % p || W % p) return -1;
  const long n = (long)B * K * (3 * p * p / 4);
  if (n == 0) return 0;
  if (p == 16 && W % 4 == 0 && (reinterpret_cast<uintptr_t>(img) & 3) == 0) {
    gather_patches16_kernel<<<cdiv((long)B * K * 64, 256), 256, 0, st>>>(img, ids, idsB, out, B, K, H, W);
    return 0;
  }
  gather_patches_kernel<<<cdiv(n, 256), 256, 0, st>>>(img, ids, idsB, out, B, K, H, W, p);
  return 0;
}

int jm_embed_finish(const uint16_t* e, const float* pos, const int* ids, long idsB, const float* cls, float* out,
                    int B, int C, int K, int D, hipStream_t st) {
  if (D % 4) return -1;
  const long n = (long)B * (C + K) * (D / 4);
  if (n == 0) return 0;
  embed_finish_kernel<<<cdiv(n, 256), 256, 0, st>>>(e, pos, ids, idsB, cls, out, B, C, K, D);
  return 0;
}

int jm_unshuffle_fwd(const uint16_t* y, const float* tok, const int* restore, long rsB, const float* pos, float* out,
                     int B, int C, int K, int N, int d, hipStream_t st) {
  if (d % 4) return -1;
  const long n = (long)B * (C + N) * (d / 4);
  if (n == 0) return 0;
  unshuffle_fwd_kernel<<<cdiv(n, 256), 256, 0, st>>>(y, tok, restore, rsB, pos, out, B, C, K, N, d);
  return 0;
}

int jm_unshuffle_bwd_blocks(int B, int C, int N, int rows_per_block) {
  return cdiv((long)B * (C + N), rows_per_block);
}

int jm_unshuffle_bwd(const float* dout, const int* restore, long rsB, uint16_t* dy, double* part, int B, int C, int K,
                     int N, int d, int rows_per_block, hipStream_t st) {
  if (d % 4 || d / 4 > 256) return -1;
  const int nb = jm_unshuffle_bwd_blocks(B, C, N, rows_per_block);
  const size_t sm = (size_t)(256 / (d / 4)) * d * sizeof(double);
  unshuffle_bwd_kernel<<<nb, 256, sm, st>>>(dout, restore, rsB, dy, part, B, C, K, N, d, rows_per_block);
  return 0;
}

int jm_patch_mse_fwd(const uint16_t* pred, long ldp, const uint8_t* img, float* mse, long rows, int N, int H, int W,
                     int p, int norm_pix, hipStream_t st) {
  const int P3 = 3 * p * p;
  if (H % p || W % p || P3 > 64 * 16) return -1;
  const int nb = cdiv(rows, 4);
  if (nb == 0) return 0;
  if (p == 16) {
    const int vec = (ldp % 4 == 0 && aligned(pred, 8) ? P16_PRED : 0) | (aligned(img, 16) ? P16_IMG : 0);
    patch_mse_fwd_kernel<12, true><<<nb, 256, 0, st>>>(pred, ldp, img, mse, rows, N, H, W, p, norm_pix, vec);
  } else if (P3 <= 64 * 4)
    patch_mse_fwd_kernel<4, false><<<nb, 256, 0, st>>>(pred, ldp, img, mse, rows, N, H, W, p, norm_pix, 0);
  else if (P3 <= 64 * 12)
    patch_mse_fwd_kernel<12, false><<<nb, 256, 0, st>>>(pred, ldp, img, mse, rows, N, H, W, p, norm_pix, 0);
  else patch_mse_fwd_kernel<16, false><<<nb, 256, 0, st>>>(pred, ldp, img, mse, rows, N, H, W, p, norm_pix, 0);
  return 0;
}

int jm_patch_mse_bwd(const uint16_t* pred, long ldp, const uint8_t* img, const float* dmse, uint16_t* dpred, long rows,
                     int N, int H, int W, int p, int norm_pix, hipStream_t st) {
  const int P3 = 3 * p * p;
  if (H % p || W % p || P3 > 64 * 16) return -1;
  const int nb = cdiv(rows, 4);
  if (nb == 0) return 0;
  if (p == 16) {
    const int vec =
        (ldp % 4 == 0 && aligned(pred, 8) && aligned(dpred, 8) ? P16_PRED : 0) | (aligned(img, 16) ? P16_IMG : 0);
    patch_mse_bwd_kernel<12, true><<<nb, 256, 0, st>>>(pred, ldp, img, dmse, dpred, rows, N, H, W, p, norm_pix, vec);
  } else if (P3 <= 64 * 4)
    patch_mse_bwd_kernel<4, false><<<nb, 256, 0, st>>>(pred, ldp, img, dmse, dpred, rows, N, H, W, p, norm_pix, 0);
  else if (P3 <= 64 * 12)
    patch_mse_bwd_kernel<12, false><<<nb, 256, 0, st>>>(pred, ldp, img, dmse, dpred, rows, N, H, W, p, norm_pix, 0);
  else
    patch_mse_bwd_kernel<16, false><<<nb, 256, 0, st>>>(pred, ldp, img, dmse, dpred, rows, N, H, W, p, norm_pix, 0);
  return 0;
}

namespace {
__global__ __launch_bounds__(256) void mix_patches_kernel(const uint8_t* __restrict__ img, const int* __restrict__ perm,
                                                          const float* __restrict__ prm, const int* __restrict__ box,
                                                          uint16_t* __restrict__ out, int B, int H, int W, int p) {
  const int P3 = 3 * p * p, q = P3 / 4, g = W / p, N = (H / p) * g;
  const long i = (long)blockIdx.x * 256 + threadIdx.x;
  if (i >= (long)B * N * q) return;
  const int mode = prm ? (int)prm[0] : 0;
  const float r = prm ? prm[1] : 1.f;
  int y0 = 0, y1 = 0, x0 = 0, x1 = 0;
  if (mode == 2) {
    y0 = box[0];
    y1 = box[1];
    x0 = box[2];
    x1 = box[3];
  }
  const long row = i / q;
  const int o0 = (int)(i - row * q) * 4;
  const int b = (int)(row / N), n = (int)(row - (long)b * N);
  const int gy = n / g, gx = n - (n / g) * g;
  const int bo = mode ? perm[b] : b;
  float f[4];
#pragma unroll
  for (int j = 0; j < 4; ++j) {
    const int o = o0 + j;
    const int ph = o / (3 * p);
    const int rr = o - ph * 3 * p;
    const int pw = rr / 3;
    const int y = gy * p + ph, x = gx * p + pw;
    const float a = patch_pixel(img, b, H, W, p, gy, gx, o);
    if (mode == 1) {
      f[j] = r * a + (1.f - r) * patch_pixel(img, bo, H, W, p, gy, gx, o);
    } else if (mode == 2 && y >= y0 && y < y1 && x >= x0 && x < x1) {
      f[j] = patch_pixel(img, bo, H, W, p, gy, gx, o);
    } else {
      f[j] = a;
    }
  }
  store4(out + row * P3 + o0, f);
}

__global__ __launch_bounds__(256) void mix_patches16_kernel(const uint8_t* __restrict__ img,
                                                            const int* __restrict__ perm,
                                                            const float* __restrict__ prm,
                                                            const int* __restrict__ box,
                                                            uint16_t* __restrict__ out, int B, int H, int W) {
  const int g = W / 16, N = (H / 16) * g;
  const long i = (long)blockIdx.x * 256 + threadIdx.x;
  if (i >= (long)B * N * 64) return;
  const int mode = prm ? (int)prm[0] : 0;
  const float r = prm ? prm[1] : 1.f;
  const long row = i >> 6;
  const int lane = (int)(i & 63);
  const int b = (int)(row / N), n = (int)(row - (long)b * N);
  const int gy = n / g, gx = n - (n / g) * g;
  uint32_t pa[3], pb[3];
  p16_raw(img, b, H, W, gy, gx, lane, pa);
  float f[12];
  if (mode == 0) {
#pragma unroll
    for (int j = 0; j < 12; ++j) f[j] = p16_norm(pa, j);
  } else {
    p16_raw(img, perm[b], H, W, gy, gx, lane, pb);
    if (mode == 1) {
#pragma unroll
      for (int j = 0; j < 12; ++j) f[j] = r * p16_norm(pa, j) + (1.f - r) * p16_norm(pb, j);
    } else {
      const int y = gy * 16 + (lane >> 2), x0 = gx * 16 + (lane & 3) * 4;
      const bool yin = y >= box[0] && y < box[1];
#pragma unroll
      for (int j = 0; j < 12; ++j) {
        const int x = x0 + j / 3;
        f[j] = (yin && x >= box[2] && x < box[3]) ? p16_norm(pb, j) : p16_norm(pa, j);
      }
    }
  }
  p16_store12(out + row * 768 + 12 * lane, f);
}
}

int jm_mix_patches(const uint8_t* img, const int* perm, const float* prm, const int* box, uint16_t* out, int B, int H,
                   int W, int p, hipStream_t st) {
  if ((3 * p * p) % 4 || H % p || W % p) return -1;
  if (prm != nullptr && (perm == nullptr || box == nullptr)) return -2;
  const long n = (long)B * (H / p) * (W / p) * (3 * p * p / 4);
  if (n == 0) return 0;
  if (p == 16 && W % 4 == 0 && (reinterpret_cast<uintptr_t>(img) & 3) == 0) {
    mix_patches16_kernel<<<cdiv((long)B * (H / 16) * (W / 16) * 64, 256), 256, 0, st>>>(img, perm, prm, box, out, B,
                                                                                         H, W);
    return 0;
  }
  mix_patches_kernel<<<cdiv(n, 256), 256, 0, st>>>(img, perm, prm, box, out, B, H, W, p);
  return 0;
}

namespace {
__global__ __launch_bounds__(256) void mask_ids_kernel(const float* __restrict__ noise, int N, int keep,
                                                       int64_t* __restrict__ shuffle, int64_t* __restrict__ restore,
                                                       int* __restrict__ keep32, int* __restrict__ restore32,
                                                       float* __restrict__ mask) {
  __shared__ float v[1024];
  const long r = blockIdx.x;
  for (int i = threadIdx.x; i < N; i += 256) v[i] = noise[r * N + i];
  __syncthreads();
  for (int i = threadIdx.x; i < N; i += 256) {
    const float x = v[i];
    int rank = 0;
    for (int j = 0; j < N; ++j) {
      const float y = v[j];
      rank += (y < x) || (y == x && j < i);
    }
    shuffle[r * N + rank] = i;
    restore[r * N + i] = rank;
    restore32[r * N + i] = rank;
    if (rank < keep) keep32[r * keep + rank] = i;
    mask[r * N + i] = rank >= keep ? 1.f : 0.f;
  }
}
}

int jm_mask_ids(const float* noise, int R, int N, int keep, int64_t* shuffle, int64_t* restore, int* keep32,
                int* restore32, float* mask, hipStream_t st) {
  if (N > 1024 || keep > N || keep < 0 || R <= 0) return -1;
  mask_ids_kernel<<<R, 256, 0, st>>>(noise, N, keep, shuffle, restore, keep32, restore32, mask);
  return 0;
}

JM_DEBUG_EXPORT(mae)
```

jumbo_mae_tpu_amd/models/mae.py:

```python

from __future__ import annotations

import torch

from ..config import DecoderConfig, ViTConfig
from ..data.constants import IMAGENET_DEFAULT_MEAN, IMAGENET_DEFAULT_STD
from ..ops import attn_stats as AS
from ..ops import mae as mae_ops
from ..utils.mae import masking_ids
from .params import ParamStore, trunc_normal_
from .vit import Dense, JumboViT, MAEDecoder, cls_features


class PretrainModel:
    def __init__(self, vit_cfg: ViTConfig, dec_cfg: DecoderConfig, norm_pix_loss: bool = False,
                 mask_mode: str = "shared"):
        assert vit_cfg.image_mask_ratio is not None
        self.cfg, self.dec_cfg = vit_cfg, dec_cfg
        self.norm_pix_loss = norm_pix_loss
        self.mask_mode = mask_mode
        self.store = ParamStore()
        s = self.store
        self.encoder = JumboViT(s, vit_cfg, ("model",))
        d = dec_cfg.dec_dim
        self.mask_token = s.handle(s.add(("image_mask_embedding",), (1, 1, d), trunc_normal_))
        self.decoder_proj = Dense(s, ("decoder_proj",), vit_cfg.dim, d)
        s.pad()
        self.decoder = MAEDecoder(s, dec_cfg, ("decoder_model",))
        self.decoder_image_output = Dense(s, ("decoder_image_output",), d, vit_cfg.patch_size ** 2 * 3)
        s.pad()

    def to(self, device, compute_dtype=torch.float32, seed: int = 0):
        g = torch.Generator(device=device).manual_seed(seed)
        self.store.finalize(device, compute_dtype, g)
        return self

    @property
    def device(self):
        return self.store.master.device

    def normalize(self, images_u8: torch.Tensor) -> torch.Tensor:
        return mae_ops.normalized_patches(images_u8, self.cfg.patch_size)

    def draw_mask(self, batch: int, noise_rng: torch.Generator | None, noise: torch.Tensor | None = None):
        n = self.cfg.seq_patches
        if noise is None:
            shape = (n,) if self.mask_mode == "shared" else (batch, n)
            noise = torch.rand(shape, generator=noise_rng, device=self.device)
        return masking_ids(noise, self.cfg.keep_len)

    def _predict(self, images_u8: torch.Tensor, rngs: dict, det: bool, enc_det: bool,
                 noise: torch.Tensor | None):
        cfg = self.cfg
        B = images_u8.shape[0]
        C = cfg.num_cls_tokens
        N, K = cfg.seq_patches, cfg.keep_len
        ids_shuffle, ids_restore, ids_keep, mask = self.draw_mask(B, rngs.get("noise"), noise)
        rows = mae_ops.kept_patches(images_u8, ids_keep, cfg.patch_size, self.store.compute_dtype)
        drop = rngs.get("dropout")
        x = self.encoder.embed_rows(rows, ids_keep, B)
        x = self.encoder.blocks(x, drop, det=enc_det)
        h = self.encoder.norm(x)
        y = self.decoder_proj(h).view(B, C + K, -1)
        dec_in = mae_ops.unshuffle_fused(y, self.mask_token, ids_restore, self.decoder.posemb_table(y.device), C)
        xd = self.decoder.blocks(dec_in, drop, det=det)
        hd = self.decoder.dec_norm(xd, row0=C)
        pred = self.decoder_image_output(hd)
        return pred.view(B, N, -1), mask, (ids_shuffle, ids_restore, ids_keep)

    def forward(self, images_u8: torch.Tensor, rngs: dict | None = None, det: bool = False,
                noise: torch.Tensor | None = None, per_sample: bool = False) -> dict:
        pred, mask, _ = self._predict(images_u8, rngs or {}, det, False, noise)
        per_patch = mae_ops.patch_mse(pred, images_u8, self.cfg.patch_size, self.norm_pix_loss)
        loss = mae_ops.masked_mean_loss(per_patch, mask, per_sample)
        return {"loss": loss}

    __call__ = forward

    @torch.no_grad()
    def reconstruct(self, images_u8: torch.Tensor, noise: torch.Tensor | None = None, rngs: dict | None = None,
                    det: bool = True, fill: int = 127) -> dict:
        B = images_u8.shape[0]
        pred, mask, _ = self._predict(images_u8, rngs or {}, det, det, noise)
        out = mae_ops.reconstruct_panels(pred, images_u8, mask, self.cfg.patch_size, self.norm_pix_loss, fill)
        mask = (mask if mask.dim() == 2 else mask.unsqueeze(0).expand(B, mask.shape[0])).contiguous()
        mse = (out["err"] * mask).sum(-1) / mask.sum(-1)
        out["mask"] = mask
        out["psnr_masked"] = -10.0 * torch.log10(mse)
        return out

    @torch.no_grad()
    def features(self, images_u8: torch.Tensor) -> torch.Tensor:
        rows = mae_ops.mixed_patches(images_u8, None, self.cfg.patch_size, self.store.compute_dtype)
        return cls_features(self.encoder, rows, images_u8.shape[0], None, True)

    @torch.no_grad()
    def attention_stats(self, images_u8: torch.Tensor, noise: torch.Tensor | None = None) -> dict:
        names = [f"layer_{i}" for i in range(len(self.encoder.layers))] + \
                [f"decoder/dec_layer_{i}" for i in range(len(self.decoder.layers))]
        return AS.collect_layers(names, lambda: self._predict(images_u8, {}, True, True, noise),
                                 self.cfg.num_cls_tokens)

    @torch.no_grad()
    def evaluate(self, images_u8: torch.Tensor, valid: torch.Tensor | None = None, rngs: dict | None = None) -> dict:
        per = self.forward(images_u8, rngs, det=False, per_sample=True)["loss"]
        v = torch.ones_like(per) if valid is None else valid.float()
        return {"loss": (per * v).sum(), "num_samples": v.sum()}

    def flax_params(self) -> dict:
        return self.store.to_flax_tree()

    def load_flax_params(self, tree: dict, strict: bool = True):
        return self.store.load_flax_tree(tree, strict=strict)


IMAGENET_MEAN = IMAGENET_DEFAULT_MEAN
IMAGENET_STD = IMAGENET_DEFAULT_STD
```

jumbo_mae_tpu_amd/models/vit.py:

```python

from __future__ import annotations

import math
import os

import numpy as np
import torch

from ..config import DecoderConfig, ViTConfig
from ..ops import attn_stats as AS
from ..ops import blocks
from ..ops import dropout as Dr
from ..ops import functional as Fn
from ..ops import mae as mae_ops
from ..utils.posemb import fixed_sincos2d_embeddings
from .params import ParamStore, const_, ones_, trunc_normal_, trunc_normal_t, zeros_


def use_fused_blocks() -> bool:
    return os.environ.get("JMAE_PER_OP", "0") != "1"


def _dense_kernel(store: ParamStore, path, in_shape, out_shape, trainable=True):
    fin, fout = int(np.prod(in_shape)), int(np.prod(out_shape))
# ... 160 lines not shown
        return masks[k]
    return droppath_mask(rate, batch, rng, device, det)


class JumboLayer:

    def __init__(self, store, path, cfg: ViTConfig, jumbo_mlp: FeedForward, trainable=True):
        D, J = cfg.dim, cfg.jumbo_dim
        self.cfg = cfg
        self.C = cfg.num_cls_tokens
        self.attn = Attention(store, path + ("attn",), D, cfg.heads, cfg.dropout, trainable)
        self.ff = FeedForward(store, path + ("ff",), D, cfg.hidden_dim, cfg.dropout, trainable)
        self.norm1 = LayerNorm(store, path + ("norm1",), D, trainable)
        self.norm2 = LayerNorm(store, path + ("norm2",), D, trainable)
        self.norm3 = LayerNorm(store, path + ("norm3",), J, trainable)
        self.jumbo_mlp = jumbo_mlp
        self.scale1 = self.scale2 = self.scale3 = None
        if cfg.layerscale:
            self.scale1 = store.handle(store.add(path + ("scale1",), (D,), const_(1e-4), trainable=trainable))
            self.scale2 = store.handle(store.add(path + ("scale2",), (D,), const_(1e-4), trainable=trainable))
            self.scale3 = store.handle(store.add(path + ("scale3",), (J,), const_(1e-4), trainable=trainable))

    n_droppath = 3
    n_seeds = 6

    @property
    def droppath_rate(self):
        return self.cfg.droppath

    @property
    def dropout_rate(self):
        return self.cfg.dropout

    def __call__(self, x, rng=None, det=True, link_in=None, link_out=None, masks=None, seeds=None):
        B, S, D = x.shape
        C = self.C
        p = self.cfg.droppath
        sd = seeds if seeds is not None else _layer_seeds(self.cfg.dropout, rng, x.device, det, 6)
        if use_fused_blocks() and self.cfg.dropout < 1.0:
            m1 = _mask(masks, 0, p, B, rng, x.device, det)
            m3 = _mask(masks, 1, p, B, rng, x.device, det)
            m2 = _mask(masks, 2, p, B, rng, x.device, det)
            return blocks.jumbo_block(self, x, m1, m2, m3, link_in, link_out, _drops(sd, self.cfg.dropout, True))
        h = self.norm1(x)
        a = self.attn(h, B, S, rng, det, sd and sd[0:2])
        x = Fn.residual(x, a, self.scale1, _mask(masks, 0, p, B, rng, x.device, det))

        cls = x[:, :C].reshape(B, 1, C * D)
        hc = self.norm3(cls, out_dtype=torch.float32)
        yc = self.jumbo_mlp(hc.to(self.norm3.g.store.compute_dtype), rng, det, sd and sd[2:4])
        xc = Fn.residual(hc.view(B, 1, C * D), yc, self.scale3, _mask(masks, 1, p, B, rng, x.device, det))

        pt = x[:, C:]
        hp = self.norm2(pt)
        yp = self.ff(hp, rng, det, sd and sd[4:6])
        xp = Fn.residual(pt, yp, self.scale2, _mask(masks, 2, p, B, rng, x.device, det))
        return torch.cat([xc.view(B, C, D), xp], 1)


class ViTLayer:

    def __init__(self, store, path, dim, heads, layerscale, dropout, droppath, trainable=True):
        self.attn = Attention(store, path + ("attn",), dim, heads, dropout, trainable)
        self.ff = FeedForward(store, path + ("ff",), dim, 4 * dim, dropout, trainable)
        self.norm1 = LayerNorm(store, path + ("norm1",), dim, trainable)
        self.norm2 = LayerNorm(store, path + ("norm2",), dim, trainable)
        self.droppath = droppath
        self.scale1 = self.scale2 = None
        if layerscale:
            self.scale1 = store.handle(store.add(path + ("scale1",), (dim,), const_(1e-4), trainable=trainable))
            self.scale2 = store.handle(store.add(path + ("scale2",), (dim,), const_(1e-4), trainable=trainable))

    n_droppath = 2
    n_seeds = 4

    @property
    def droppath_rate(self):
        return self.droppath

    @property
    def dropout_rate(self):
        return self.attn.dropout

    def __call__(self, x, rng=None, det=True, link_in=None, link_out=None, masks=None, seeds=None):
        B, S, D = x.shape
        p = self.droppath
        sd = seeds if seeds is not None else _layer_seeds(self.attn.dropout, rng, x.device, det, 4)
        if use_fused_blocks() and self.attn.dropout < 1.0:
            m1 = _mask(masks, 0, p, B, rng, x.device, det)
            m2 = _mask(masks, 1, p, B, rng, x.device, det)
            return blocks.vit_block(self, x, m1, m2, link_in, link_out, _drops(sd, self.attn.dropout, False))
        h = self.norm1(x)
        a = self.attn(h, B, S, rng, det, sd and sd[0:2])
        x = Fn.residual(x, a, self.scale1, _mask(masks, 0, p, B, rng, x.device, det))
        h = self.norm2(x)
        f = self.ff(h, rng, det, sd and sd[2:4])
        return Fn.residual(x, f, self.scale2, _mask(masks, 1, p, B, rng, x.device, det))


class JumboViT:

    def __init__(self, store: ParamStore, cfg: ViTConfig, prefix=("model",), trainable=True):
        self.cfg = cfg
        D, p, g = cfg.dim, cfg.patch_size, cfg.grid
        P = prefix
        self.wte_k = store.handle(_dense_kernel(store, P + ("embed", "wte", "kernel"), (p, p, 3), (D,), trainable))
        self.wte_b = store.handle(_bias(store, P + ("embed", "wte", "bias"), (D,), trainable))
        self.wpe = None
        if cfg.posemb == "learnable":
            self.wpe = store.handle(store.add(P + ("embed", "wpe"), (g * g, D), trunc_normal_,
                                              flax_shape=(g, g, D),
                                              to_flax=lambda a, s=(g, g, D): a.reshape(s),
                                              from_flax=lambda a, n=g * g, d=D: a.reshape(n, d),
                                              trainable=trainable))
        self.cls_tokens = store.handle(store.add(P + ("cls_tokens",), (1, cfg.num_cls_tokens, D), zeros_,
                                                 trainable=trainable))
        self.jumbo_mlp = FeedForward(store, P + ("jumbo_mlp",), cfg.jumbo_dim, 4 * cfg.jumbo_dim,
                                     cfg.dropout, trainable)
        self.jumbo_mlp.w1.k.defer_wgrad = True
        self.jumbo_mlp.w2.k.defer_wgrad = True
        store.pad()
        self.layers = []
        for i in range(cfg.layers):
            self.layers.append(JumboLayer(store, P + (f"layer_{i}",), cfg, self.jumbo_mlp, trainable))
            store.pad()
        self.norm = LayerNorm(store, P + ("norm",), D, trainable)
        store.pad()
        self._posemb_cache = {}

    def posemb_table(self, device) -> torch.Tensor | None:
        if self.cfg.posemb != "sincos2d":
            return None
        key = str(device)
        if key not in self._posemb_cache:
            g = self.cfg.grid
            self._posemb_cache[key] = fixed_sincos2d_embeddings(g, g, self.cfg.dim, device).reshape(g * g, -1)
        return self._posemb_cache[key]

    def embed(self, patches: torch.Tensor, ids: torch.Tensor | None) -> torch.Tensor:
        B, n, K = patches.shape
        dt = self.wte_k.store.compute_dtype
        return self.embed_rows(patches.reshape(B * n, K).to(dt), ids, B)

    def embed_rows(self, rows: torch.Tensor, ids: torch.Tensor | None, B: int) -> torch.Tensor:
        e = Fn.linear(rows, self.wte_k, self.wte_b)
        if ids is None:
            ids = self._arange(rows.shape[0] // B, rows.device)
        return mae_ops.embed_finish(e, self.cls_tokens, self.wpe, self.posemb_table(rows.device), ids, B)

    def _arange(self, n, device):
        key = ("arange", n, str(device))
        if key not in self._posemb_cache:
            self._posemb_cache[key] = torch.arange(n, device=device)
        return self._posemb_cache[key]

    def blocks(self, x: torch.Tensor, rng=None, det=True) -> torch.Tensor:
        return _run_layers(self.layers, x, rng, det, self.cfg.grad_ckpt, in_dropout=self.cfg.dropout)


def cls_features(encoder: "JumboViT", rows: torch.Tensor, B: int, drop=None, det: bool = True) -> torch.Tensor:
    cfg = encoder.cfg
    x = encoder.embed_rows(rows, None, B)
    x = encoder.blocks(x, drop, det)
    C = cfg.num_cls_tokens
    h = Fn.layer_norm(x[:, :C], encoder.norm.g, encoder.norm.b, torch.float32)
    return h.reshape(B, C * cfg.dim)


def _run_layers(layers, x, rng, det, grad_ckpt, in_dropout=0.0):
    masks = droppath_masks(layers, x.shape[0], rng, x.device, det)
    x, seeds = dropout_seed_pool(layers, rng, x.device, det, head=(x, in_dropout))
    if grad_ckpt and torch.is_grad_enabled():
        for layer, m, sd in zip(layers, masks, seeds):
            x = _checkpointed(layer, x, rng, det, m, sd)
        return x
    link = None
    for i, layer in enumerate(layers):
        nxt = None
        if blocks.LINKS and torch.is_grad_enabled():
            up = layers[i + 1] if i + 1 < len(layers) else None
            ln1 = (up.norm1.g, up.norm1.b) if up is not None and blocks.FWD_LINKS else None
            nxt = blocks.Link(ln1)
        x = layer(x, rng, det, link_in=link, link_out=nxt, masks=masks[i], seeds=seeds[i])
        link = nxt
    return x


def _checkpointed(layer, x, rng, det, masks=None, seeds=None):
    store = layer.norm1.g.store
    state = rng.get_state() if rng is not None else None
    calls = [0]

    def run(inp):
        calls[0] += 1
        if calls[0] == 1:
            return layer(inp, rng, det, masks=masks, seeds=seeds)
        g = None
        if rng is not None:
            g = torch.Generator(device=rng.device)
            g.set_state(state)
        with store.uses_suppressed():
            return layer(inp, g, det, masks=masks, seeds=seeds)

    return torch.utils.checkpoint.checkpoint(run, x, use_reentrant=False)


class MAEDecoder:

    def __init__(self, store: ParamStore, cfg: DecoderConfig, prefix=("decoder_model",)):
        self.cfg = cfg
        self.layers = []
        for i in range(cfg.dec_layers):
            self.layers.append(ViTLayer(store, prefix + (f"dec_layer_{i}",), cfg.dec_dim, cfg.dec_heads,
                                        cfg.dec_layerscale, cfg.dec_dropout, cfg.dec_droppath))
            store.pad()
        self.dec_norm = LayerNorm(store, prefix + ("dec_norm",), cfg.dec_dim)
        store.pad()
        self._posemb_cache = {}

    def posemb_table(self, device) -> torch.Tensor:
        key = str(device)
        if key not in self._posemb_cache:
            g = self.cfg.grid
            self._posemb_cache[key] = fixed_sincos2d_embeddings(g, g, self.cfg.dec_dim, device).reshape(g * g, -1)
        return self._posemb_cache[key]

    def blocks(self, x, rng=None, det=True):
        return _run_layers(self.layers, x, rng, det, self.cfg.grad_ckpt)


class LinearCLS:

    def __init__(self, store: ParamStore, path, dim: int, labels: int, batch_norm: bool):
        self.batch_norm = batch_norm
        self.bn_scale = self.bn_bias = None
        if batch_norm:
            self.bn_scale = store.handle(store.add(path + ("BatchNorm_0", "scale"), (dim,), ones_))
            self.bn_bias = store.handle(store.add(path + ("BatchNorm_0", "bias"), (dim,), zeros_))
        self.dense = Dense(store, path + ("Dense_0",), dim, labels)
        store.pad()
        self.dim = dim
        self.running_mean: torch.Tensor | None = None
        self.running_var: torch.Tensor | None = None

    def init_stats(self, device):
        if self.batch_norm:
            self.running_mean = torch.zeros(self.dim, device=device)
            self.running_var = torch.ones(self.dim, device=device)

    def __call__(self, x: torch.Tensor, det: bool, group=None, raw: bool = False) -> torch.Tensor:
        if self.batch_norm:
            from ..parallel.syncbn import sync_batch_norm
            x = sync_batch_norm(x, self.bn_scale, self.bn_bias, self.running_mean, self.running_var,
                                training=not det, momentum=0.99, eps=1e-5, group=group,
                                out_dtype=self.dense.k.store.compute_dtype)
        dt = self.dense.k.store.compute_dtype
        y = self.dense(x.to(dt))
        return y if raw else y.float()
```

jumbo_mae_tpu_amd/ops/blocks.py:

```python

from __future__ import annotations


import torch

from typing import NamedTuple

from . import attn_stats as AS
from . import dropout as Dr
from . import prims as P


LINKS = True
FWD_LINKS = True


class Link:

    __slots__ = ("spec", "dy", "done", "dx_key", "ln1", "h1")

    def __init__(self, ln1=None):
        self.spec = None
        self.dy = None
        self.done = False
# ... 112 lines not shown
        ctx.save_for_backward(x, mu1, rs1, h1, qkv, o, lse, a, x1, muc, rsc, hcb, jpre, jg, jy,
                              hp, mup, rsp, fpre, fg, fy, m1, m2, m3)
        ctx.layer = layer
        ctx.link_in, ctx.link_out = link_in, link_out
        ctx.gelu_deriv = (jd, fd)
        ctx.gelu_rate = rate
        ctx.dr = dr
        if link_out is not None:
            link_out.spec = P.ResSpec(fy, layer.scale2, m2, layer.ff.w2.b, C, drop=_od(dr, "fo", fy))
        return x2

    @staticmethod
    def backward(ctx, dx2):
        with P.paired_wgrads():
            dx = _jumbo_bwd(ctx, dx2)
        return dx, None, None, None, None, None, None, None, None, None


def _jumbo_bwd(ctx, dx2):
    (x, mu1, rs1, h1, qkv, o, lse, a, x1, muc, rsc, hcb, jpre, jg, jy,
     hp, mup, rsp, fpre, fg, fy, m1, m2, m3) = ctx.saved_tensors
    layer = ctx.layer
    dr = ctx.dr
    B, S, D = x.shape
    C = layer.C
    J = C * D
    dt = h1.dtype
    dx2 = dx2.contiguous()
    dx1 = torch.empty_like(dx2)
    a3 = a.view(B, S, D)
    da = torch.empty_like(a)
    da3 = da.view(B, S, D)
    dcls = dx2[:, :C].reshape(B, 1, J)
    djy, bd = P.residual_bwd(dcls, jy, layer.scale3, m3, dt, layer.jumbo_mlp.w2.b, drop=_od(dr, "jo", jy))
    dhc = _ff_bwd(layer.jumbo_mlp, djy, hcb, jpre, jg, bd, dx_add=dcls.reshape(B, J),
                  deriv=ctx.gelu_deriv[0], rate=ctx.gelu_rate)
    P.ln_bwd(dhc, x1[:, :C].reshape(B, 1, J), muc, rsc, layer.norm3.g, layer.norm3.b,
             out=dx1[:, :C].reshape(B, 1, J))
    P.residual_bwd(dx1[:, :C], a3[:, :C], layer.scale1, m1, dt, layer.attn.wo_b, out=da3[:, :C], mark_ready=False,
                   drop=_od(dr, "wo", a))
    fused = ctx.link_out.take(dx2) if ctx.link_out is not None else None
    if fused is not None:
        dfy, bd = fused
    else:
        dfy, bd = P.residual_bwd(dx2[:, C:], fy, layer.scale2, m2, dt, layer.ff.w2.b, drop=_od(dr, "fo", fy))
    dhp = _ff_bwd(layer.ff, dfy, hp, fpre, fg, bd, deriv=ctx.gelu_deriv[1], rate=ctx.gelu_rate)
    _, _, bd = P.ln_bwd(dhp, x1[:, C:], mup, rsp, layer.norm2.g, layer.norm2.b, dres=dx2[:, C:],
                        out=dx1[:, C:],
                        res=P.ResSpec(a3[:, C:], layer.scale1, m1, layer.attn.wo_b, 0, da3[:, C:],
                                      drop=_od(dr, "wo", a)), h=hp)
    dh1 = _attn_bwd(layer.attn, da, h1, qkv, o, lse, B, S, bd, dr)
    return _ln1_bwd(ctx, dh1, x, mu1, rs1, layer, dx1, h1)


def _ln1_fwd(x, layer, link_in, dt):
    pre = link_in.take_h1(x) if link_in is not None else None
    if pre is not None:
        return pre
    return P.ln_fwd(x, layer.norm1.g, layer.norm1.b, dt)


def _ln1_bwd(ctx, dh1, x, mu1, rs1, layer, dx1, h1=None):
    li = ctx.link_in
    if li is None or li.spec is None:
        return P.ln_bwd(dh1, x, mu1, rs1, layer.norm1.g, layer.norm1.b, dres=dx1, out=dx1, h=h1)
    dx, li.dy, li.done = P.ln_bwd(dh1, x, mu1, rs1, layer.norm1.g, layer.norm1.b, dres=dx1, out=dx1, res=li.spec,
                                  h=h1)
    li.dx_key = (dx.data_ptr(), tuple(dx.shape))
    li.spec = None
    return dx


def jumbo_block(layer, x, m1=None, m2=None, m3=None, link_in: Link | None = None, link_out: Link | None = None,
                dr: Drops | None = None):
    _note_uses(layer.norm1.g, layer.norm1.b, layer.norm2.g, layer.norm2.b, layer.norm3.g, layer.norm3.b,
               layer.scale1, layer.scale2, layer.scale3, *_attn_handles(layer.attn), *_ff_handles(layer.ff),
               *_ff_handles(layer.jumbo_mlp))
    return JumboBlockFn.apply(x.contiguous(), layer.norm1.g.param, layer, m1, m2, m3, link_in, link_out,
                              torch.is_grad_enabled(), dr)


class ViTBlockFn(torch.autograd.Function):
    @staticmethod
    def forward(ctx, x, anchor, layer, m1, m2, link_in, link_out, train=True, dr=None):
        B, S, D = x.shape
        dt = layer.norm1.g.store.compute_dtype
        h1, mu1, rs1 = _ln1_fwd(x, layer, link_in, dt)
        qkv, o, lse, a = _attn_fwd(layer.attn, h1, B, S, dr)
        x1, h2, mu2, rs2 = P.residual_ln_fwd(x, a, layer.scale1, m1, layer.norm2.g, layer.norm2.b, 0,
                                             drop=_od(dr, "wo", a))
        fpre, fg, fy, fd = _ff_fwd(layer.ff, h2, train, dr.rate if dr is not None else 0.0, dr and dr.fh,
                                   dr and dr.fo)
        nl = link_out.ln1 if link_out is not None else None
        if nl is not None:
            x2, h1n, mun, rsn = P.residual_ln_fwd(x1, fy, layer.scale2, m2, nl[0], nl[1], 0, drop=_od(dr, "fo", fy))
            link_out.put_h1(x2, h1n, mun, rsn)
        else:
            x2 = P.residual_fwd(x1, fy, layer.scale2, m2, drop=_od(dr, "fo", fy))
        ctx.save_for_backward(x, mu1, rs1, h1, qkv, o, lse, a, x1, mu2, rs2, h2, fpre, fg, fy, m1, m2)
        ctx.layer = layer
        ctx.link_in, ctx.link_out = link_in, link_out
        ctx.gelu_deriv = (False, fd)
        ctx.gelu_rate = dr.rate if dr is not None else 0.0
        ctx.dr = dr
        if link_out is not None:
            link_out.spec = P.ResSpec(fy, layer.scale2, m2, layer.ff.w2.b, 0, drop=_od(dr, "fo", fy))
        return x2

    @staticmethod
    def backward(ctx, dx2):
        with P.paired_wgrads():
            dx = _vit_bwd(ctx, dx2)
        return dx, None, None, None, None, None, None, None, None


def _vit_bwd(ctx, dx2):
    x, mu1, rs1, h1, qkv, o, lse, a, x1, mu2, rs2, h2, fpre, fg, fy, m1, m2 = ctx.saved_tensors
    layer = ctx.layer
    dr = ctx.dr
    B, S, D = x.shape
    dt = h1.dtype
    dx2 = dx2.contiguous()
    fused = ctx.link_out.take(dx2) if ctx.link_out is not None else None
    if fused is not None:
        dfy, bd = fused
    else:
        dfy, bd = P.residual_bwd(dx2, fy, layer.scale2, m2, dt, layer.ff.w2.b, drop=_od(dr, "fo", fy))
    dh2 = _ff_bwd(layer.ff, dfy, h2, fpre, fg, bd, deriv=ctx.gelu_deriv[1], rate=ctx.gelu_rate)
    dx1, da, bd = P.ln_bwd(dh2, x1, mu2, rs2, layer.norm2.g, layer.norm2.b, dres=dx2,
                           res=P.ResSpec(a, layer.scale1, m1, layer.attn.wo_b, drop=_od(dr, "wo", a)), h=h2)
    dh1 = _attn_bwd(layer.attn, da, h1, qkv, o, lse, B, S, bd, dr)
    return _ln1_bwd(ctx, dh1, x, mu1, rs1, layer, dx1, h1)


def vit_block(layer, x, m1=None, m2=None, link_in: Link | None = None, link_out: Link | None = None,
              dr: Drops | None = None):
    _note_uses(layer.norm1.g, layer.norm1.b, layer.norm2.g, layer.norm2.b, layer.scale1, layer.scale2,
               *_attn_handles(layer.attn), *_ff_handles(layer.ff))
    return ViTBlockFn.apply(x.contiguous(), layer.norm1.g.param, layer, m1, m2, link_in, link_out,
                            torch.is_grad_enabled(), dr)
```

jumbo_mae_tpu_amd/ops/mae.py:

```python

from __future__ import annotations

import torch

from ..data.constants import IMAGENET_DEFAULT_MEAN, IMAGENET_DEFAULT_STD
from ..utils.mae import extract_patches_nchw, index_sequence, patch_mse_loss
from . import _ext

_MEAN_STD_CACHE: dict = {}


def _mean_std(device):
    key = str(device)
    if key not in _MEAN_STD_CACHE:
        m = torch.tensor(IMAGENET_DEFAULT_MEAN, dtype=torch.float32, device=device).view(1, 3, 1, 1)
        s = torch.tensor(IMAGENET_DEFAULT_STD, dtype=torch.float32, device=device).view(1, 3, 1, 1)
        _MEAN_STD_CACHE[key] = (m, s)
    return _MEAN_STD_CACHE[key]


def normalize_images(images_u8: torch.Tensor) -> torch.Tensor:
    m, s = _mean_std(images_u8.device)
    return (images_u8.float() / 255.0 - m) / s

# ... 48 lines not shown
        return _ext.load().gather_patches(images_u8.contiguous(), _i32(ids_keep), patch_size)
    kept = index_sequence(normalized_patches(images_u8, patch_size), ids_keep)
    return kept.reshape(B * kept.shape[1], -1).to(dtype)


class _EmbedFinish(torch.autograd.Function):

    @staticmethod
    def forward(ctx, e, cls_p, wpe_p, h_cls, h_wpe, pos, ids, B):
        D = e.shape[-1]
        C = h_cls.numel // D
        K = ids.shape[-1]
        if _ext.use_hip(e) and e.dtype == torch.bfloat16:
            out = _ext.load().embed_finish(e.contiguous(), pos, _i32(ids), h_cls.master.contiguous(), B)
        else:
            ev = e.float().view(B, K, D)
            if pos is not None:
                ev = ev + (pos[ids] if ids.dim() == 1 else pos[ids])
            out = torch.cat([h_cls.master.view(1, C, D).expand(B, C, D), ev], 1)
        ctx.h_cls, ctx.h_wpe, ctx.C, ctx.B, ctx.K = h_cls, h_wpe, C, B, K
        ctx.edtype = e.dtype
        ctx.save_for_backward(ids)
        return out

    @staticmethod
    def backward(ctx, dx):
        (ids,) = ctx.saved_tensors
        C, B, K = ctx.C, ctx.B, ctx.K
        D = dx.shape[-1]
        dpatch = dx[:, C:]
        if ctx.h_cls.segs[0].trainable:
            ctx.h_cls.accumulate_grad_rows(dx[:, :C].reshape(B, C * D))
        h = ctx.h_wpe
        if h is not None and h.segs[0].trainable:
            if ids.dim() == 1:
                h.grad.index_add_(0, ids, dpatch.sum(0))
            else:
                h.grad.index_add_(0, ids.reshape(-1), dpatch.reshape(-1, D))
            h.ready()
        de = dpatch.to(ctx.edtype).reshape(B * K, D)
        return de, None, None, None, None, None, None, None


def embed_finish(e: torch.Tensor, h_cls, h_wpe, pos: torch.Tensor | None, ids: torch.Tensor, B: int) -> torch.Tensor:
    h_cls.note_use()
    if h_wpe is not None:
        h_wpe.note_use()
        pos = h_wpe.master
    return _EmbedFinish.apply(e, h_cls.param, h_wpe.param if h_wpe is not None else None, h_cls, h_wpe,
                              pos, ids, B)


class _Unshuffle(torch.autograd.Function):

    @staticmethod
    def forward(ctx, y, tok_p, h_tok, ids_restore, pos, C):
        ids32 = _i32(ids_restore)
        out = _ext.load().unshuffle_fwd(y.contiguous(), h_tok.master.reshape(-1).contiguous(), ids32,
                                        pos.contiguous(), C)
        ctx.save_for_backward(ids32)
        ctx.h_tok, ctx.C, ctx.K = h_tok, C, y.shape[1] - C
        return out

    @staticmethod
    def backward(ctx, dout):
        (ids32,) = ctx.saved_tensors
        dy, dtok_part = _ext.load().unshuffle_bwd(dout.contiguous(), ids32, ctx.C, ctx.K)
        if ctx.h_tok.segs[0].trainable:
            ctx.h_tok.accumulate_grad_rows(dtok_part)
        return dy, None, None, None, None, None


def unshuffle_fused(y: torch.Tensor, h_tok, ids_restore: torch.Tensor, pos: torch.Tensor, num_cls: int):
    if _ext.use_hip(y) and y.dtype == torch.bfloat16 and y.shape[-1] % 4 == 0 and y.shape[-1] <= 1024:
        h_tok.note_use()
        return _Unshuffle.apply(y, h_tok.param, h_tok, ids_restore, pos, num_cls)
    from .params_fn import param_value
    return unshuffle(y, param_value(h_tok).view(-1), ids_restore, pos, num_cls)


class _PatchMSE(torch.autograd.Function):

    @staticmethod
    def forward(ctx, pred, images_u8, patch_size, norm_pix):
        B = images_u8.shape[0]
        pred2 = pred.reshape(-1, pred.shape[-1])
        mse = _ext.load().patch_mse_fwd(pred2, images_u8.contiguous(), patch_size, norm_pix)
        ctx.save_for_backward(pred2, images_u8)
        ctx.p, ctx.norm_pix, ctx.pshape = patch_size, norm_pix, pred.shape
        return mse.view(B, -1)

    @staticmethod
    def backward(ctx, dmse):
        pred2, images_u8 = ctx.saved_tensors
        dpred = _ext.load().patch_mse_bwd(pred2, images_u8.contiguous(), dmse.reshape(-1).contiguous().float(),
                                          ctx.p, ctx.norm_pix)
        return dpred.view(ctx.pshape), None, None, None


def patch_mse(pred: torch.Tensor, images_u8: torch.Tensor, patch_size: int, norm_pix_loss: bool) -> torch.Tensor:
    B = images_u8.shape[0]
    fits = 3 * patch_size * patch_size <= 1024
    if fits and _ext.use_hip(pred) and pred.dtype == torch.bfloat16 and pred.stride(-1) == 1:
        return _PatchMSE.apply(pred, images_u8, patch_size, bool(norm_pix_loss))
    t = normalized_patches(images_u8, patch_size)
    if norm_pix_loss:
        t = norm_pix(t)
    return (t - pred.float().view(B, t.shape[1], -1)).square().mean(-1)


def masked_mean_loss(per_patch: torch.Tensor, mask: torch.Tensor, per_sample: bool = False) -> torch.Tensor:
    if mask.dim() == 1:
        mask = mask.unsqueeze(0).expand_as(per_patch)
    if per_sample:
        return (per_patch * mask).sum(-1) / mask.sum(-1)
    valid_ratio = mask.sum(-1) / mask.shape[-1]
    pp = torch.where(mask > 0.0, per_patch, torch.zeros_like(per_patch))
    return (pp.mean(-1) / valid_ratio).mean()


def unpatchify(patches: torch.Tensor, p: int, H: int, W: int) -> torch.Tensor:
    B = patches.shape[0]
    gh, gw = H // p, W // p
    x = patches.reshape(B, gh, gw, p, p, 3)
    return x.permute(0, 5, 1, 3, 2, 4).reshape(B, 3, H, W)


def _pixel_mask(mask: torch.Tensor, B: int, p: int, H: int, W: int) -> torch.Tensor:
    gh, gw = H // p, W // p
    m = (mask if mask.dim() == 2 else mask.unsqueeze(0).expand(B, gh * gw)) > 0
    return m.reshape(B, 1, gh, gw).repeat_interleave(p, 2).repeat_interleave(p, 3)


def reconstruct_torch(pred: torch.Tensor, images_u8: torch.Tensor, mask: torch.Tensor, p: int, norm_pix: bool,
                      fill: int = 127, fp64: bool = False) -> dict:
    dt = torch.float64 if fp64 else torch.float32
    B, _, H, W = images_u8.shape
    N = (H // p) * (W // p)
    m, s = _mean_std(images_u8.device)
    m, s = m.to(dt), s.to(dt)
    orig = images_u8.to(dt) / 255.0
    v = pred.to(dt).reshape(B, N, 3 * p * p)
    if norm_pix:
        t = extract_patches_nchw((orig - m) / s, p)
        mean = t.mean(-1, keepdim=True)
        var = t.var(-1, keepdim=True, unbiased=False)
        v = v * torch.sqrt(var + 1e-6) + mean
    x = (unpatchify(v, p, H, W) * s + m) * 255.0
    x = torch.where(x > 0, x, torch.zeros_like(x)).clamp(max=255.0)
    recon = torch.round(x).to(torch.uint8)
    err = extract_patches_nchw((x / 255.0 - orig).square(), p).mean(-1)
    mpix = _pixel_mask(mask, B, p, H, W)
    return {"recon": recon, "paste": torch.where(mpix, recon, images_u8),
            "masked": torch.where(mpix, torch.full_like(images_u8, fill), images_u8), "err": err, "x": x}


def reconstruct_panels(pred: torch.Tensor, images_u8: torch.Tensor, mask: torch.Tensor, p: int, norm_pix: bool,
                       fill: int = 127) -> dict:
    if _ext.use_hip(pred):
        B = images_u8.shape[0]
        pr = pred.reshape(-1, pred.shape[-1])
        if pr.dtype != torch.bfloat16:
            pr = pr.float()
        rec, paste, masked, err = _ext.load().recon(pr.contiguous(), images_u8.contiguous(),
                                                    mask.float().contiguous(), p, bool(norm_pix), fill)
        return {"recon": rec, "paste": paste, "masked": masked, "err": err.view(B, -1)}
    out = reconstruct_torch(pred, images_u8, mask, p, norm_pix, fill)
    del out["x"]
    return out


def mixed_patches(images_u8: torch.Tensor, plan: dict | None, patch_size: int, dtype) -> torch.Tensor:
    from ..utils.mixup import Mixup

    B = images_u8.shape[0]
    if _ext.use_hip(images_u8) and dtype == torch.bfloat16:
        if plan is None:
            return _ext.load().mix_patches(images_u8.contiguous(), None, None, None, patch_size)
        d = plan["dev"]
        return _ext.load().mix_patches(images_u8.contiguous(), d["perm"], d["params"], d["box"], patch_size)
    x = Mixup.mix_images(normalize_images(images_u8), plan)
    return extract_patches_nchw(x, patch_size).reshape(B * (x.shape[-1] // patch_size) ** 2, -1).to(dtype)
```

jumbo_mae_tpu_amd/ops/prims.py:

```python

from __future__ import annotations

import contextlib
import math
import os

from typing import NamedTuple

import torch
import torch.nn.functional as F

from ..models.params import Handle
from . import _ext

LN_EPS = 1e-6
_GELU_C = math.sqrt(2.0 / math.pi)


def hip(t: torch.Tensor) -> bool:
    return _ext.use_hip(t)


def _trainable(h: Handle | None) -> bool:
    return h is not None and h.segs[0].trainable
# ... 19 lines not shown
def wgrad(h: Handle, dy: torch.Tensor, x: torch.Tensor, rows: tuple[int, int] | None = None) -> None:
    g = h.grad if rows is None else h.grad[rows[0]:rows[1]]
    if dy.is_cuda and dy.dtype != torch.float32:
        M, N = dy.shape
        K = x.shape[1]
        if _tn_ok(dy, x):
            store = h.take_store() if rows is None else False
            if rows is not None:
                h.settle()
            _ext.load().gemm_tn_wgrad(dy, x, g, store)
            return
        h.settle()
        if (_WGRAD_OURS and hip(dy) and dy.dtype == torch.bfloat16 and x.dtype == torch.bfloat16
                and M < NARROW_MAX_M and K % 8 == 0):
            g.add_(_ext.load().gemm_nt_f32(_pad_cols(dy.t()), _pad_cols(x.t())))
            return
        s = wgrad_split(M, N, K)
        if s > 1:
            part = torch.bmm(dy.view(s, M // s, N).transpose(1, 2), x.view(s, M // s, K), out_dtype=torch.float32)
            if hip(part):
                _ext.load().splitk_reduce_add(part, g)
            else:
                g.add_(part.sum(0))
        else:
            torch.addmm(g, dy.t(), x, out_dtype=torch.float32, out=g)
    else:
        g.addmm_(dy.t().float(), x.float())


PAIR_WGRAD = True
_pair: dict = {"depth": 0, "held": None}


@contextlib.contextmanager
def paired_wgrads():
    _pair["depth"] += 1
    try:
        yield
    finally:
        _pair["depth"] -= 1
        if _pair["depth"] == 0:
            _flush_pair()


def _flush_pair() -> None:
    held, _pair["held"] = _pair["held"], None
    if held is not None:
        hw, dy, x = held
        wgrad(hw, dy, x)
        hw.ready()


def _wgrad_ready(hw: Handle, dy: torch.Tensor, x: torch.Tensor) -> None:
    if PAIR_WGRAD and _pair["depth"] > 0 and _tn_ok(dy, x):
        held = _pair["held"]
        if held is not None and held[1].shape[0] == dy.shape[0] and held[0] is not hw:
            _pair["held"] = None
            _ext.load().gemm_tn_wgrad_group([held[1], dy], [held[2], x], [held[0].grad, hw.grad],
                                            [held[0].take_store(), hw.take_store()])
            held[0].ready()
            hw.ready()
            return
        _flush_pair()
        _pair["held"] = (hw, dy, x)
        return
    wgrad(hw, dy, x)
    hw.ready()


def bias_grad(hb: Handle, dy: torch.Tensor) -> None:
    if hip(dy) and dy.dtype == torch.bfloat16 and dy.shape[-1] % 8 == 0 and dy.stride(-1) == 1:
        _ext.load().colsum(dy, hb.grad)
    else:
        hb.grad.add_(dy.sum(0, dtype=torch.float32))


_GEMM_MODE = "auto"
_DGRAD_OURS = True
_CLS_LOSS_OURS = True
_BN_OURS = True
_KNN_OURS = True
_NORMS_OURS = True
_ATTN_STATS_OURS = True


NARROW_MAX_M = 4096
_NARROW_FUSED_MIN_TILES = 160


def nt_tiles(M: int, N: int) -> int:
    if M < NARROW_MAX_M:
        return -(-M // 128) * -(-N // 192)
    return -(-M // 256) * -(-N // 256)


def use_our_gemm(M: int, N: int, K: int, fused_gelu: bool = False, kind: str = "fwd") -> bool:
    if _GEMM_MODE == "blas" or K % 64 or N % 8:
        return False
    if M >= NARROW_MAX_M:
        return True
    return not fused_gelu or nt_tiles(M, N) >= _NARROW_FUSED_MIN_TILES


def splitk_plan(M: int, N: int, K: int) -> int:
    if _GEMM_MODE == "blas" or M >= NARROW_MAX_M or K % 64 or N % 8:
        return 0
    if nt_tiles(M, N) >= _NARROW_FUSED_MIN_TILES:
        return 0
    s = min(256 // nt_tiles(M, N), K // 512, 16)
    return s if s >= 2 else 0


def _pad_cols(t: torch.Tensor, mult: int = 64) -> torch.Tensor:
    c = t.shape[1]
    pad = -c % mult
    return F.pad(t, (0, pad)) if pad else t.contiguous()


def linear_fwd(x2: torch.Tensor, hw: Handle, hb: Handle | None) -> torch.Tensor:
    w = hw.weight()
    if hip(x2) and x2.dtype == torch.bfloat16:
        s = splitk_plan(x2.shape[0], w.shape[0], x2.shape[1])
        if s:
            return _ext.load().gemm_nt_splitk(x2, w, hb.master if hb is not None else None, s)
    if hip(x2) and x2.dtype == torch.bfloat16 and use_our_gemm(x2.shape[0], w.shape[0], x2.shape[1]):
        return _ext.load().gemm_nt(x2, w, hb.master if hb is not None else None, False)[0]
    if hb is not None:
        return torch.addmm(hb.weight(), x2, w.t())
    return x2 @ w.t()


def linear_gelu_fwd(x2: torch.Tensor, hw: Handle, hb: Handle | None, need_pre: bool = True):
    w = hw.weight()
    if hip(x2) and x2.dtype == torch.bfloat16 and use_our_gemm(x2.shape[0], w.shape[0], x2.shape[1], True):
        if not need_pre:
            return None, _ext.load().gemm_nt(x2, w, hb.master if hb is not None else None, True, True)[0]
        pre, g = _ext.load().gemm_nt(x2, w, hb.master if hb is not None else None, True)
        return pre, g
    pre = linear_fwd(x2, hw, hb)
    return pre, gelu_fwd(pre)


_GELU_DERIV = os.environ.get("JMAE_GELU_CODES", "1") != "0"


GD_Q, GD_Z = 195.0, 34


def gd_encode(d: torch.Tensor) -> torch.Tensor:
    return torch.clamp(torch.round(d.float() * GD_Q + GD_Z), 0, 255).to(torch.uint8)


def gd_decode(q: torch.Tensor, rate: float = 0.0, dtype=torch.bfloat16) -> torch.Tensor:
    s = (1.0 / (1.0 - rate) if rate > 0 else 1.0) / GD_Q
    return ((q.float() - GD_Z) * s).to(dtype)


def linear_gelu_fwd_saved(x2: torch.Tensor, hw: Handle, hb: Handle | None, need_pre: bool = True, drop=None):
    w = hw.weight()
    if (_GELU_DERIV and need_pre and hip(x2) and x2.dtype == torch.bfloat16 and w.shape[0] % 8 == 0
            and use_our_gemm(x2.shape[0], w.shape[0], x2.shape[1], True)):
        bias = hb.master if hb is not None else None
        if drop is not None:
            gp, g = _ext.load().gemm_nt(x2, w, bias, True, False, True, drop[0], drop[1])
            return gp, g, True, True
        gp, g = _ext.load().gemm_nt(x2, w, bias, True, False, True)
# ... 229 lines not shown


_FUSE_LN_RES = True


class ResSpec(NamedTuple):
    y: torch.Tensor
    hs: Handle | None
    mask: torch.Tensor | None
    hbias: Handle | None
    t0: int = 0
    out: torch.Tensor | None = None
    drop: tuple | None = None


def _drop_args(y: torch.Tensor, drop) -> tuple:
    if drop is None:
        return None, 0.0, 0
    seed, rate, base = drop
    return seed, rate, y.storage_offset() - base.storage_offset()


def _drop_factor(y: torch.Tensor, drop) -> torch.Tensor:
    from . import dropout as Dr
    seed, rate, base = drop
    _, scale = Dr.keep_threshold(rate)
    full = Dr.keep_mask(seed.cpu(), base.numel(), rate).to(y.device).float() * scale
    return full.as_strided(y.shape, y.stride(), y.storage_offset() - base.storage_offset())


_LN_BWD_FROM_H = False


def ln_bwd(dy: torch.Tensor, x3: torch.Tensor, mean, rstd, hg: Handle, hb: Handle, dres=None, out=None,
           res: ResSpec | None = None, h: torch.Tensor | None = None):
    B, T, D = x3.shape
    dy = dy.contiguous()
    tr = _trainable(hg)
    fused = res is not None and _FUSE_LN_RES and hip(x3) and res.y.dtype == torch.bfloat16
    dyr = None
    if hip(x3):
        hx = h if (_LN_BWD_FROM_H and h is not None and h.dtype == torch.bfloat16 and h.is_contiguous()
                   and h.numel() == dy.numel()) else None
        beta = hb.master if hx is not None else None
        if fused:
            hs, hbias = res.hs, res.hbias
            dseed, drate, dioff = _drop_args(res.y, res.drop)
            dx, dyr = _ext.load().layernorm_bwd(
                dy, x3, mean, rstd, hg.master, hg.grad, hb.grad, tr, dres, out, res.y,
                hs.master if hs is not None else None, res.mask, hs.grad if _trainable(hs) else None,
                hbias.grad if _trainable(hbias) else None, res.t0, res.out, dseed, drate, dioff, hx, beta)
        else:
            dx = _ext.load().layernorm_bwd(dy, x3, mean, rstd, hg.master, hg.grad, hb.grad, tr, dres, out,
                                           hx=hx, beta=beta)[0]
    else:
        xf = x3.reshape(B * T, D).float()
        xhat = (xf - mean[:, None]) * rstd[:, None]
        dyf = dy.reshape(B * T, D).float()
        if tr:
            hg.grad.add_((dyf * xhat).sum(0))
            hb.grad.add_(dyf.sum(0))
        g = dyf * hg.master
        dx = rstd[:, None] * (g - g.mean(-1, keepdim=True) - xhat * (g * xhat).mean(-1, keepdim=True))
        dx = dx.reshape(B, T, D)
        if dres is not None:
            dx = dx + dres
        if out is not None:
            out.copy_(dx)
            dx = out
    if tr:
        hg.ready()
        hb.ready()
    if res is None:
        return dx
    if fused:
        if _trainable(res.hs):
            res.hs.ready()
        return dx, dyr, _trainable(res.hbias)
    dyr, done = residual_bwd(dx[:, res.t0:], res.y, res.hs, res.mask, res.y.dtype, res.hbias, out=res.out,
                             drop=res.drop)
    return dx, dyr, done


def residual_fwd(x3: torch.Tensor, y2: torch.Tensor, hs: Handle | None, mask, out=None, drop=None) -> torch.Tensor:
    B, T, D = x3.shape
    if hip(x3):
        y2r = y2.reshape(B * T, D)
        dseed, drate, dioff = _drop_args(y2r, drop)
        return _ext.load().residual_fwd(x3, y2r, hs.master if hs is not None else None, mask, out, dseed, drate,
                                        dioff)
    r = y2.float()
    if drop is not None:
        r = r * _drop_factor(y2, drop)
    r = r.reshape(B, T, D)
    if hs is not None:
        r = r * hs.master
    if mask is not None:
        r = r * mask.view(B, 1, 1)
    res = x3.float() + r
    if out is not None:
        out.copy_(res)
        return out
    return res


def residual_ln_fwd(x3: torch.Tensor, y2: torch.Tensor, hs: Handle | None, mask, hg: Handle, hb: Handle,
                    t0: int = 0, r0: int = 0, out: torch.Tensor | None = None, drop=None):
    B, T, D = x3.shape
    if hip(x3) and y2.dtype == torch.bfloat16:
        if drop is not None:
            assert y2.data_ptr() == drop[2].data_ptr() and y2.numel() == drop[2].numel()
        return tuple(_ext.load().residual_ln_fwd(x3, y2.reshape(B * (T - r0), D),
                                                 hs.master if hs is not None else None, mask, hg.master, hb.master,
                                                 LN_EPS, t0, r0, out, drop[0] if drop else None,
                                                 drop[1] if drop else 0.0))
    if r0 == 0 and out is None:
        x1 = residual_fwd(x3, y2, hs, mask, drop=drop)
    else:
        x1 = out if out is not None else torch.empty_like(x3)
        residual_fwd(x3[:, r0:], y2, hs, mask, out=x1[:, r0:], drop=drop)
    h, mean, rstd = ln_fwd(x1[:, t0:], hg, hb, hg.store.compute_dtype)
    return x1, h, mean, rstd


def residual_bwd(dout3: torch.Tensor, y2: torch.Tensor | None, hs: Handle | None, mask, ydtype,
                 hbias: Handle | None = None, out: torch.Tensor | None = None, mark_ready: bool = True, drop=None):
    B, T, D = dout3.shape
    bg = hbias.grad if _trainable(hbias) else None
    if hip(dout3) and ydtype == torch.bfloat16 and (hs is not None or mask is not None or bg is not None
                                                    or drop is not None):
        dseed, drate, dioff = _drop_args(y2 if y2 is not None else out, drop)
        dy = _ext.load().residual_bwd(dout3, y2, hs.master if hs is not None else None, mask,
                                      hs.grad if _trainable(hs) else None, ydtype, bg, out, dseed, drate, dioff)
        done = bg is not None
    else:
        d = dout3.float()
        if mask is not None:
            d = d * mask.view(B, 1, 1)
        if drop is not None:
            d = d * _drop_factor(y2, drop).reshape(B, T, D)
        if hs is not None:
            if _trainable(hs):
                hs.grad.add_((d * y2.float().reshape(B, T, D)).sum((0, 1)))
            d = d * hs.master
        dy = d.to(ydtype)
        if out is not None:
            out.copy_(dy.reshape(out.shape))
            dy = out
        else:
            dy = dy.reshape(B * T, D)
        done = False
    if mark_ready and _trainable(hs):
        hs.ready()
    return dy, done


def _attn_hip(qkv: torch.Tensor, heads: int) -> bool:
    if not hip(qkv):
        return False
    hd = qkv.shape[2] // 3 // heads
    return hd in _ext.load().attn_head_dims()


_ATTN_DROP_TILED = True


def _attn_drop_hip(S: int, hd: int) -> bool:
    ext = _ext.load()
    return ext.attn_dropout(S, hd) and (_ATTN_DROP_TILED or ext.attn_fused_bias(S, hd))


def _drop_mask(drop, B: int, heads: int, S: int, device):
    from . import dropout as Dr
    seed, rate = drop
    _, scale = Dr.keep_threshold(rate)
    m = Dr.keep_mask_rows(seed.cpu(), B * heads * S, S, rate).view(B, heads, S, S).to(device)
    return m.float() * scale


def attn_fwd(qkv: torch.Tensor, heads: int, drop=None):
    B, S, three_d = qkv.shape
    D = three_d // 3
    hd = D // heads
    if _attn_hip(qkv, heads) and (drop is None or _attn_drop_hip(S, hd)):
        if drop is None:
            return _ext.load().attn_fwd(qkv, heads)
        return _ext.load().attn_fwd(qkv, heads, drop[0], drop[1])
    q, k, v = qkv.float().view(B, S, 3, heads, hd).unbind(2)
    z = torch.einsum("bqhd,bkhd->bhqk", q / math.sqrt(hd), k)
    lse = torch.logsumexp(z, -1)
    p = torch.exp(z - lse[..., None])
    if drop is not None:
        p = p * _drop_mask(drop, B, heads, S, qkv.device)
    o = torch.einsum("bhqk,bkhd->bqhd", p, v).reshape(B, S, D).to(qkv.dtype)
    return o, lse


def attn_bwd(do: torch.Tensor, qkv: torch.Tensor, o: torch.Tensor, lse: torch.Tensor, heads: int,
             hbias: Handle | None = None, drop=None):
    B, S, three_d = qkv.shape
    D = three_d // 3
    hd = D // heads
    do = do.contiguous().view(B, S, D)
    if _attn_hip(qkv, heads) and (drop is None or _attn_drop_hip(S, hd)):
        ext = _ext.load()
# ... 20 lines not shown
```

Measured before the change: 6690 images/sec.

## Prune decoder last block MLP and loss to masked rows only

Adds a masked-row index path so the decoder's final block computes the post-attention residual+LayerNorm, MLP, prediction head and patch MSE only for masked patch rows (compact [B*Nm, D]). Visible rows and CLS tokens carry no loss there, so this skips roughly a quarter of the last-block MLP and head GEMM work plus the loss work on unmasked rows. Backward scatters gradients back through an inverse index map in a new LayerNorm-backward variant. It adds gather/scatter indexing and a mask_rows kernel, and does not support dropout on that path.

```diff
diff --git a/jumbo_mae_tpu_amd/csrc/bindings.cpp b/jumbo_mae_tpu_amd/csrc/bindings.cpp
--- a/jumbo_mae_tpu_amd/csrc/bindings.cpp
+++ b/jumbo_mae_tpu_amd/csrc/bindings.cpp
@@ -146,6 +146,89 @@
            "layernorm_bwd");
   if (has_res) return {dx, dyr};
   return {dx};
+}
+
+static long idx_bstride(const torch::Tensor& ids, int64_t B, int64_t n, const char* what) {
+  CHECK_CUDA(ids);
+  CHECK_DT(ids, torch::kInt32);
+  CHECK_CONTIG(ids);
+  TORCH_CHECK((ids.dim() == 1 && ids.size(0) == n) || (ids.dim() == 2 && ids.size(0) == B && ids.size(1) == n), what,
+              ": index tensor must be int32 [n] or [B, n]");
+  return ids.dim() == 1 ? 0 : n;
+}
+
+std::vector<torch::Tensor> layernorm_bwd_rows(torch::Tensor dy, torch::Tensor x, torch::Tensor mean, torch::Tensor rstd,
+                                              torch::Tensor gamma, torch::Tensor dgamma, torch::Tensor dbeta, bool accum,
+                                              c10::optional<torch::Tensor> dres, torch::Tensor inv, int64_t B,
+                                              torch::Tensor res_y, c10::optional<torch::Tensor> res_scale,
+                                              c10::optional<torch::Tensor> res_mask,
+                                              c10::optional<torch::Tensor> res_dscale,
+                                              c10::optional<torch::Tensor> res_dbias,
+                                              c10::optional<torch::Tensor> res_seed, double res_rate, int64_t res_ioff,
+                                              c10::optional<torch::Tensor> hx, c10::optional<torch::Tensor> beta,
+                                              c10::optional<torch::Tensor> out, c10::optional<torch::Tensor> res_out) {
+  CHECK_CUDA(dy);
+  CHECK_CONTIG(dy);
+  CHECK_DT(dy, torch::kBFloat16);
+  CHECK_CONTIG(x);
+  CHECK_DT(x, torch::kFloat32);
+  CHECK_CONTIG(mean);
+  CHECK_CONTIG(rstd);
+  CHECK_CONTIG(res_y);
+  CHECK_DT(res_y, torch::kBFloat16);
+  TORCH_CHECK(B > 0 && res_y.dim() == 2 && res_y.size(0) % B == 0, "layernorm_bwd_rows: res_y must be [B*T, D]");
+  const int T = res_y.size(0) / B, D = res_y.size(1);
+  TORCH_CHECK(x.numel() % ((long)B * D) == 0, "layernorm_bwd_rows: x must be [B*Nm, D]");
+  const int Nm = x.numel() / ((long)B * D);
+  const long R = (long)B * Nm;
+  TORCH_CHECK(Nm > 0 && Nm <= T && dy.numel() == R * D && mean.numel() == R && rstd.numel() == R,
+              "layernorm_bwd_rows: compact shapes");
+  TORCH_CHECK(gamma.numel() == D && dgamma.numel() == D && dbeta.numel() == D, "layernorm_bwd_rows: parameter shapes");
+  const long ib = idx_bstride(inv, B, T, "layernorm_bwd_rows");
+  const float* rp = nullptr;
+  if (dres.has_value() && dres->defined()) {
+    CHECK_CONTIG((*dres));
+    CHECK_DT((*dres), torch::kFloat32);
+    TORCH_CHECK(dres->numel() == R * D, "layernorm_bwd_rows: dres must be [B*Nm, D]");
+    rp = dres->data_ptr<float>();
+  }
+  const uint16_t* hxp = nullptr;
+  const float* betap = nullptr;
+  if (hx.has_value() && hx->defined()) {
+    CHECK_DT((*hx), torch::kBFloat16);
+    CHECK_CONTIG((*hx));
+    TORCH_CHECK(hx->numel() == R * D, "hx shape");
+    TORCH_CHECK(beta.has_value() && beta->defined() && beta->numel() == D, "hx needs beta [D]");
+    CHECK_DT((*beta), torch::kFloat32);
+    hxp = bf(*hx);
+    betap = beta->data_ptr<float>();
+  }
+  torch::Tensor dx, dyr;
+  if (out.has_value() && out->defined()) {
+    dx = *out;
+    CHECK_CONTIG(dx);
+    CHECK_DT(dx, torch::kFloat32);
+    TORCH_CHECK(dx.dim() == 3 && dx.size(0) == B && dx.size(1) == T && dx.size(2) == D, "layernorm_bwd_rows: out [B,T,D]");
+  } else {
+    dx = torch::empty({(long)B, T, D}, x.options());
+  }
+  if (res_out.has_value() && res_out->defined()) {
+    dyr = *res_out;
+    CHECK_CONTIG(dyr);
+    CHECK_DT(dyr, torch::kBFloat16);
+    TORCH_CHECK(dyr.sizes() == res_y.sizes(), "layernorm_bwd_rows: res_out must match res_y");
+  } else {
+    dyr = torch::empty_like(res_y);
+  }
+  JmLnRes res{bf(res_y), bfm(dyr), (long)T * D, D, fopt(res_scale), fopt(res_mask), 0, fopt_m(res_dscale),
+              fopt_m(res_dbias), make_drop(res_seed, res_rate, res_y, res_ioff)};
+  auto ws = torch::empty({(long)jm_layernorm_bwd_blocks(B * T, D) * 4 * D}, x.options());
+  check_rc(jm_layernorm_bwd(dy.data_ptr(), 1, x.data_ptr<float>(), 0, 0, B, T, D, mean.data_ptr<float>(),
+                            rstd.data_ptr<float>(), gamma.data_ptr<float>(), dx.data_ptr<float>(), dx.stride(0),
+                            dx.stride(1), rp, 0, 0, dgamma.data_ptr<float>(), dbeta.data_ptr<float>(), accum,
+                            ws.data_ptr<float>(), &res, stream(), hxp, betap, inv.data_ptr<int>(), ib, Nm),
+           "layernorm_bwd_rows");
+  return {dx, dyr};
 }
 
 torch::Tensor gelu_fwd(torch::Tensor h) {
@@ -623,32 +706,70 @@
   return out;
 }
 
-torch::Tensor patch_mse_fwd(torch::Tensor pred, torch::Tensor img, int64_t p, bool norm_pix) {
+std::vector<torch::Tensor> mask_rows(torch::Tensor mask, int64_t C, int64_t Nm) {
+  CHECK_CUDA(mask);
+  CHECK_CONTIG(mask);
+  CHECK_DT(mask, torch::kFloat32);
+  TORCH_CHECK(mask.dim() == 1 || mask.dim() == 2, "mask_rows: mask [N] or [R, N]");
+  const int N = mask.size(-1), R = mask.dim() == 1 ? 1 : mask.size(0);
+  TORCH_CHECK(N >= 1 && N <= 1024 && Nm >= 1 && Nm <= N && C >= 0, "mask_rows: 1 <= Nm <= N <= 1024, C >= 0");
+  auto i32 = mask.options().dtype(torch::kInt32);
+  auto rs = mask.sizes().vec(), is = mask.sizes().vec();
+  rs.back() = Nm;
+  is.back() = C + N;
+  auto rows = torch::empty(rs, i32), inv = torch::empty(is, i32);
+  check_rc(jm_mask_rows(mask.data_ptr<float>(), R, N, (int)C, (int)Nm, rows.data_ptr<int>(), inv.data_ptr<int>(),
+                        stream()),
+           "mask_rows");
+  return {rows, inv};
+}
+
+struct MseIdx {
+  const int* idx = nullptr;
+  long idsB = 0;
+  int Nm = 0;
+};
+static MseIdx mse_idx(const c10::optional<torch::Tensor>& rows, int64_t B, const char* what) {
+  MseIdx m;
+  if (rows.has_value() && rows->defined()) {
+    m.Nm = rows->size(-1);
+    m.idsB = idx_bstride(*rows, B, m.Nm, what);
+    m.idx = rows->data_ptr<int>();
+  }
+  return m;
+}
+
+torch::Tensor patch_mse_fwd(torch::Tensor pred, torch::Tensor img, int64_t p, bool norm_pix,
+                            c10::optional<torch::Tensor> rows, int64_t C) {
   CHECK_DT(pred, torch::kBFloat16);
   TORCH_CHECK(pred.stride(1) == 1, "pred rows must be contiguous");
   CHECK_CONTIG(img);
   CHECK_DT(img, torch::kUInt8);
   const int H = img.size(2), W = img.size(3), N = (H / p) * (W / p);
-  TORCH_CHECK(pred.size(0) == img.size(0) * N && pred.size(1) == 3 * p * p, "patch_mse_fwd shapes");
+  const MseIdx mi = mse_idx(rows, img.size(0), "patch_mse_fwd");
+  TORCH_CHECK(pred.size(0) == img.size(0) * (mi.idx ? mi.Nm : N) && pred.size(1) == 3 * p * p, "patch_mse_fwd shapes");
   auto mse = torch::empty({pred.size(0)}, pred.options().dtype(torch::kFloat32));
   check_rc(jm_patch_mse_fwd(bfp(pred), pred.stride(0), img.data_ptr<uint8_t>(), mse.data_ptr<float>(), pred.size(0), N,
-                            H, W, p, norm_pix, stream()),
+                            H, W, p, norm_pix, stream(), mi.idx, mi.idsB, mi.Nm, (int)C),
            "patch_mse_fwd");
   return mse;
 }
 
-torch::Tensor patch_mse_bwd(torch::Tensor pred, torch::Tensor img, torch::Tensor dmse, int64_t p, bool norm_pix) {
+torch::Tensor patch_mse_bwd(torch::Tensor pred, torch::Tensor img, torch::Tensor dmse, int64_t p, bool norm_pix,
+                            c10::optional<torch::Tensor> rows, int64_t C) {
   CHECK_DT(pred, torch::kBFloat16);
   TORCH_CHECK(pred.stride(1) == 1, "pred rows must be contiguous");
   CHECK_CONTIG(img);
   CHECK_CONTIG(dmse);
   CHECK_DT(dmse, torch::kFloat32);
   const int H = img.size(2), W = img.size(3), N = (H / p) * (W / p);
-  TORCH_CHECK(dmse.numel() == pred.size(0) && pred.size(0) == img.size(0) * N && pred.size(1) == 3 * p * p,
+  const MseIdx mi = mse_idx(rows, img.size(0), "patch_mse_bwd");
+  TORCH_CHECK(dmse.numel() == pred.size(0) && pred.size(0) == img.size(0) * (mi.idx ? mi.Nm : N) &&
+                  pred.size(1) == 3 * p * p,
               "patch_mse_bwd shapes");
   auto dpred = torch::empty({pred.size(0), pred.size(1)}, pred.options());
   check_rc(jm_patch_mse_bwd(bfp(pred), pred.stride(0), img.data_ptr<uint8_t>(), dmse.data_ptr<float>(), bfp(dpred),
-                            pred.size(0), N, H, W, p, norm_pix, stream()),
+                            pred.size(0), N, H, W, p, norm_pix, stream(), mi.idx, mi.idsB, mi.Nm, (int)C),
            "patch_mse_bwd");
   return dpred;
 }
@@ -1187,6 +1308,34 @@
                               rstd.data_ptr<float>(), B, T, T0, D, gamma.data_ptr<float>(), beta.data_ptr<float>(),
                               (float)eps, stream(), (int)R0, make_drop(seed, rate, y, 0)),
            "residual_ln_fwd");
+  return {x1, h, mean, rstd};
+}
+
+std::vector<torch::Tensor> residual_ln_fwd_rows(torch::Tensor x, torch::Tensor y, c10::optional<torch::Tensor> scale,
+                                                c10::optional<torch::Tensor> mask, torch::Tensor gamma,
+                                                torch::Tensor beta, double eps, torch::Tensor rows,
+                                                c10::optional<torch::Tensor> seed, double rate) {
+  CHECK_CUDA(x);
+  TORCH_CHECK(x.dim() == 3 && x.stride(2) == 1, "x must be [B,T,D] with contiguous last dim");
+  CHECK_DT(x, torch::kFloat32);
+  CHECK_DT(y, torch::kBFloat16);
+  CHECK_CONTIG(y);
+  const int B = x.size(0), T = x.size(1), D = x.size(2);
+  TORCH_CHECK(y.numel() == (long)B * T * D, "residual_ln_fwd_rows: y must be [B*T, D]");
+  TORCH_CHECK(gamma.numel() == D && beta.numel() == D, "residual_ln_fwd_rows: parameter shapes");
+  const int Nm = rows.size(-1);
+  TORCH_CHECK(Nm >= 1 && Nm <= T, "residual_ln_fwd_rows: 1 <= Nm <= T");
+  const long ib = idx_bstride(rows, B, Nm, "residual_ln_fwd_rows");
+  const long R = (long)B * Nm;
+  auto x1 = torch::empty({B, Nm, D}, x.options());
+  auto h = torch::empty({R, D}, y.options());
+  auto mean = torch::empty({R}, x.options());
+  auto rstd = torch::empty({R}, x.options());
+  check_rc(jm_residual_ln_fwd_idx(x.data_ptr<float>(), x.stride(0), x.stride(1), bf(y), fopt(scale), fopt(mask),
+                                  rows.data_ptr<int>(), ib, x1.data_ptr<float>(), bfm(h), mean.data_ptr<float>(),
+                                  rstd.data_ptr<float>(), B, T, Nm, D, gamma.data_ptr<float>(), beta.data_ptr<float>(),
+                                  (float)eps, stream(), make_drop(seed, rate, y, 0)),
+           "residual_ln_fwd_rows");
   return {x1, h, mean, rstd};
 }
 
@@ -1656,9 +1805,21 @@
   m.def("mask_ids", &mask_ids, "random-masking permutation ids + mask from noise (one workgroup per row)");
   m.def("unshuffle_fwd", &unshuffle_fwd);
   m.def("unshuffle_bwd", &unshuffle_bwd);
-  m.def("patch_mse_fwd", &patch_mse_fwd);
+  m.def("patch_mse_fwd", &patch_mse_fwd, py::arg("pred"), py::arg("img"), py::arg("p"), py::arg("norm_pix"),
+        py::arg("rows") = py::none(), py::arg("C") = 0);
+  m.def("mask_rows", &mask_rows, "masked decoder rows (ascending) and their inverse map from the patch mask");
+  m.def("residual_ln_fwd_rows", &residual_ln_fwd_rows, py::arg("x"), py::arg("y"), py::arg("scale"), py::arg("mask"),
+        py::arg("gamma"), py::arg("beta"), py::arg("eps"), py::arg("rows"), py::arg("seed") = py::none(),
+        py::arg("rate") = 0.0);
+  m.def("layernorm_bwd_rows", &layernorm_bwd_rows, py::arg("dy"), py::arg("x"), py::arg("mean"), py::arg("rstd"),
+        py::arg("gamma"), py::arg("dgamma"), py::arg("dbeta"), py::arg("accum"), py::arg("dres"), py::arg("inv"),
+        py::arg("B"), py::arg("res_y"), py::arg("res_scale") = py::none(), py::arg("res_mask") = py::none(),
+        py::arg("res_dscale") = py::none(), py::arg("res_dbias") = py::none(), py::arg("res_seed") = py::none(),
+        py::arg("res_rate") = 0.0, py::arg("res_ioff") = 0, py::arg("hx") = py::none(), py::arg("beta") = py::none(),
+        py::arg("out") = py::none(), py::arg("res_out") = py::none());
   m.def("mix_patches", &mix_patches);
-  m.def("patch_mse_bwd", &patch_mse_bwd);
+  m.def("patch_mse_bwd", &patch_mse_bwd, py::arg("pred"), py::arg("img"), py::arg("dmse"), py::arg("p"),
+        py::arg("norm_pix"), py::arg("rows") = py::none(), py::arg("C") = 0);
   m.def("recon", &recon, py::arg("pred"), py::arg("images"), py::arg("mask"), py::arg("p"), py::arg("norm_pix"),
         py::arg("fill") = 127, py::arg("out") = py::none(),
         "MAE reconstruction panels -> (recon, paste, masked uint8 [B, 3, H, W], err fp32 [B, N])");
diff --git a/jumbo_mae_tpu_amd/csrc/jm_api.h b/jumbo_mae_tpu_amd/csrc/jm_api.h
--- a/jumbo_mae_tpu_amd/csrc/jm_api.h
+++ b/jumbo_mae_tpu_amd/csrc/jm_api.h
@@ -68,12 +68,16 @@
                      const float* mean, const float* rstd, const float* gamma, float* dx_ptr, long oB, long oT,
                      const float* dres, long rB, long rT, float* dgamma, float* dbeta, int accum_params, float* ws,
                      const JmLnRes* res, hipStream_t st, const uint16_t* hx = nullptr,
-                     const float* beta = nullptr);
+                     const float* beta = nullptr, const int* inv = nullptr, long invB = 0, int Nm = 0);
 int jm_layernorm_bwd_blocks(int rows, int D);
 int jm_residual_ln_fwd(const float* x, long sB, long sT, const uint16_t* y, const float* scale, const float* mask,
                        float* x1, long oB, long oT, uint16_t* h, float* mean, float* rstd, int B, int T, int T0,
                        int D, const float* gamma, const float* beta, float eps, hipStream_t st, int R0 = 0,
                        JmDrop drop = JmDrop{nullptr, 0u, 1.f, 0});
+int jm_residual_ln_fwd_idx(const float* x, long sB, long sT, const uint16_t* y, const float* scale, const float* mask,
+                           const int* idx, long idsB, float* x1, uint16_t* h, float* mean, float* rstd, int B, int T,
+                           int Nm, int D, const float* gamma, const float* beta, float eps, hipStream_t st,
+                           JmDrop drop = JmDrop{nullptr, 0u, 1.f, 0});
 int jm_debug_line_layernorm();
 
 int jm_gelu_fwd(const uint16_t* h, uint16_t* a, long n, hipStream_t st);
@@ -150,9 +154,12 @@
 int jm_mix_patches(const uint8_t* img, const int* perm, const float* prm, const int* box, uint16_t* out, int B, int H,
                    int W, int p, hipStream_t st);
 int jm_patch_mse_fwd(const uint16_t* pred, long ldp, const uint8_t* img, float* mse, long rows, int N, int H, int W,
-                     int p, int norm_pix, hipStream_t st);
+                     int p, int norm_pix, hipStream_t st, const int* idx = nullptr, long idsB = 0, int Nm = 0,
+                     int C = 0);
 int jm_patch_mse_bwd(const uint16_t* pred, long ldp, const uint8_t* img, const float* dmse, uint16_t* dpred, long rows,
-                     int N, int H, int W, int p, int norm_pix, hipStream_t st);
+                     int N, int H, int W, int p, int norm_pix, hipStream_t st, const int* idx = nullptr,
+                     long idsB = 0, int Nm = 0, int C = 0);
+int jm_mask_rows(const float* mask, int R, int N, int C, int Nm, int* rows, int* inv, hipStream_t st);
 int jm_debug_line_mae();
 
 int jm_recon(const void* pred, int pred_bf16, const uint8_t* img, const float* mask, long maskB, uint8_t* recon,
diff --git a/jumbo_mae_tpu_amd/csrc/layernorm.hip b/jumbo_mae_tpu_amd/csrc/layernorm.hip
--- a/jumbo_mae_tpu_amd/csrc/layernorm.hip
+++ b/jumbo_mae_tpu_amd/csrc/layernorm.hip
@@ -154,6 +154,79 @@
   }
 }
 
+template <int V>
+__global__ __launch_bounds__(256) void res_ln_fwd_idx_kernel(ResLnIO io, const int* __restrict__ idx, long idsB,
+                                                             int T, int Nm, int rows, int D,
+                                                             const float* __restrict__ gamma,
+                                                             const float* __restrict__ beta, float eps) {
+  const int wave = threadIdx.x >> 6, lane = threadIdx.x & 63;
+  const int row = blockIdx.x * 4 + wave;
+  if (row >= rows) return;
+  const int b = row / Nm;
+  int t = idx[b * idsB + (row - b * Nm)];
+  JM_DASSERT(t >= 0 && t < T);
+  t = min(max(t, 0), T - 1);
+  const float* xr = io.x + b * io.sB + t * io.sT;
+  const uint16_t* yr = io.y + ((long)b * T + t) * D;
+  float* x1r = io.x1 + (long)row * D;
+  const float m = io.mask ? io.mask[b] : 1.f;
+  float v[V][4];
+  float s = 0.f;
+#pragma unroll
+  for (int i = 0; i < V; ++i) {
+    const int col = (i * 64 + lane) * 4;
+    if (col < D) {
+      float xv[4], yv[4], sc[4] = {1.f, 1.f, 1.f, 1.f};
+      load4(xr + col, xv);
+      load4(yr + col, yv);
+      if (io.scale) load4(io.scale + col, sc);
+      if (io.drop.seed) {
+        float f[4];
+        drop_factors<4>(io.drop, io.drop.ioff + (yr - io.y) + col, f);
+#pragma unroll
+        for (int j = 0; j < 4; ++j) yv[j] *= f[j];
+      }
+#pragma unroll
+      for (int j = 0; j < 4; ++j) v[i][j] = xv[j] + m * sc[j] * yv[j];
+      store4(x1r + col, v[i]);
+    } else {
+      v[i][0] = v[i][1] = v[i][2] = v[i][3] = 0.f;
+    }
+    s += v[i][0] + v[i][1] + v[i][2] + v[i][3];
+  }
+  const float mean = wave_sum(s) / D;
+  float s2 = 0.f;
+#pragma unroll
+  for (int i = 0; i < V; ++i) {
+    const int col = (i * 64 + lane) * 4;
+    if (col < D) {
+#pragma unroll
+      for (int j = 0; j < 4; ++j) {
+        const float d = v[i][j] - mean;
+        s2 += d * d;
+      }
+    }
+  }
+  const float rstd = rsqrtf(wave_sum(s2) / D + eps);
+  uint16_t* hr = io.h + (long)row * D;
+#pragma unroll
+  for (int i = 0; i < V; ++i) {
+    const int col = (i * 64 + lane) * 4;
+    if (col < D) {
+      float gg[4], bb[4], o[4];
+      load4(gamma + col, gg);
+      load4(beta + col, bb);
+#pragma unroll
+      for (int j = 0; j < 4; ++j) o[j] = (v[i][j] - mean) * rstd * gg[j] + bb[j];
+      store4(hr + col, o);
+    }
+  }
+  if (lane == 0) {
+    io.mean[row] = mean;
+    io.rstd[row] = rstd;
+  }
+}
+
 struct LnBwdIO {
   float* dx;
   long oB, oT;
@@ -161,6 +234,9 @@
   long rB, rT;
   const uint16_t* hx;
   const float* beta;
+  const int* inv;
+  long invB;
+  int Nm;
 };
 
 JM_DEVICE bool ln_h_ok(float g, float b) { return fabsf(g) >= 1e-20f && fabsf(b) <= fabsf(g); }
@@ -179,7 +255,7 @@
   float* p[4];
 };
 
-template <int V, typename TI, bool RES, bool ER = false, bool SC = true, int R = 1>
+template <int V, typename TI, bool RES, bool ER = false, bool SC = true, int R = 1, bool IDX = false>
 __global__ __launch_bounds__(256) void ln_bwd_kernel(const TI* __restrict__ dy, const float* __restrict__ x,
                                                      long sB, long sT, int T, int rows, int D,
                                                      const float* __restrict__ mean, const float* __restrict__ rstd,
@@ -249,33 +325,37 @@
       const int row = rw * R + sub;
       const bool valid = R == 1 || row < rows;
       const int b = row / T, t = row - b * T;
-      const float* xr = x + b * sB + t * sT;
-      const TI* dyr = dy + (long)row * D;
-      const float mu = valid ? mean[row] : 0.f, rs = valid ? rstd[row] : 0.f;
+      const int ci = (IDX && valid) ? io.inv[b * io.invB + t] : 0;
+      JM_DASSERT(!IDX || ci < io.Nm);
+      const bool live = IDX ? (valid && ci >= 0 && ci < io.Nm) : valid;
+      const long lrow = IDX ? (live ? (long)b * io.Nm + ci : 0) : row;
+      const float* xr = IDX ? x + lrow * D : x + b * sB + t * sT;
+      const TI* dyr = dy + lrow * D;
+      const float mu = live ? mean[lrow] : 0.f, rs = live ? rstd[lrow] : 0.f;
       const bool rrow = RES && t >= rio.T0;
       const long yoff = RES ? b * rio.yB + (long)(t - rio.T0) * rio.yT : 0;
       float xh[VL][4], g[VL][4], yv[VL][4];
       float rvp[ER ? VL : 1][4];
-      const float* rr = io.dres ? io.dres + b * io.rB + t * io.rT : nullptr;
+      const float* rr = !io.dres ? nullptr : IDX ? io.dres + lrow * D : io.dres + b * io.rB + t * io.rT;
       float sg = 0.f, sgx = 0.f;
       if constexpr (HP) {
-        const uint16_t* hr = io.hx + (long)row * D;
+        const uint16_t* hr = io.hx + lrow * D;
 #pragma unroll
         for (int i = 0; i < VL; ++i) {
           const int col = (i * LPR + l) * 4;
-          if (valid && col < D) load4(hr + col, xh[i]);
+          if (live && col < D) load4(hr + col, xh[i]);
         }
       } else {
 #pragma unroll
         for (int i = 0; i < VL; ++i) {
           const int col = (i * LPR + l) * 4;
-          if (valid && col < D) load4(xr + col, xh[i]);
+          if (live && col < D) load4(xr + col, xh[i]);
         }
       }
 #pragma unroll
       for (int i = 0; i < VL; ++i) {
         const int col = (i * LPR + l) * 4;
-        if (valid && col < D) {
+        if (live && col < D) {
           float dv[4];
           if constexpr (HP) {
             float bb[4], ig[4];
@@ -316,6 +396,14 @@
       for (int i = 0; i < VL; ++i) {
         const int col = (i * LPR + l) * 4;
         if (valid && col < D) {
+          if constexpr (IDX) {
+            if (!live) {
+              const float z[4] = {0.f, 0.f, 0.f, 0.f};
+              store4(dxr + col, z);
+              if (RES && rrow) store4(rio.dy + yoff + col, z);
+              continue;
+            }
+          }
           float o[4], rv[4] = {0.f, 0.f, 0.f, 0.f};
           if constexpr (ER) {
 #pragma unroll
@@ -603,13 +691,13 @@
 
 
 #define LN_BWD_R(VV) ((VV) == 2 ? 2 : 1)
-template <typename TI, bool RES, bool SC = true>
+template <typename TI, bool RES, bool SC = true, bool IDX = false>
 void launch_bwd(int V, dim3 grid, size_t smem, hipStream_t st, const TI* dy, const float* x, long sB, long sT,
                 int T, int rows, int D, const float* m, const float* r, const float* g, LnBwdIO dx, LnResIO rio,
                 float* ws, int acc, ParamOuts outs) {
 #define JM_LNB(VV)                                                                                          \
   case VV:                                                                                                  \
-    ln_bwd_kernel<VV, TI, RES, (VV >= 2 && VV <= 4), SC, LN_BWD_R(VV)><<<grid, 256, smem, st>>>(             \
+    ln_bwd_kernel<VV, TI, RES, (VV >= 2 && VV <= 4), SC, LN_BWD_R(VV), IDX><<<grid, 256, smem, st>>>(        \
         dy, x, sB, sT, T, rows, D, m, r, g, dx, rio, ws, acc, outs);                                         \
     break;
   switch (V) {
@@ -679,6 +767,28 @@
   return 0;
 }
 
+int jm_residual_ln_fwd_idx(const float* x, long sB, long sT, const uint16_t* y, const float* scale, const float* mask,
+                           const int* idx, long idsB, float* x1, uint16_t* h, float* mean, float* rstd, int B, int T,
+                           int Nm, int D, const float* gamma, const float* beta, float eps, hipStream_t st,
+                           JmDrop drop) {
+  const ResLnIO io{x, sB, sT, y, scale, mask, x1, (long)Nm * D, D, h, mean, rstd, drop};
+  const int V = pick_v(D);
+  if (V < 0 || (D % 4) != 0 || idx == nullptr || Nm <= 0 || Nm > T) return -1;
+  const int rows = B * Nm;
+  if (rows == 0) return 0;
+  dim3 grid((rows + 3) / 4);
+#define JM_RLNI(VV)                                                                                          \
+  case VV:                                                                                                   \
+    res_ln_fwd_idx_kernel<VV><<<grid, 256, 0, st>>>(io, idx, idsB, T, Nm, rows, D, gamma, beta, eps);        \
+    break;
+  switch (V) {
+    JM_RLNI(1) JM_RLNI(2) JM_RLNI(3) JM_RLNI(4) JM_RLNI(6) JM_RLNI(8) JM_RLNI(9) JM_RLNI(12) JM_RLNI(16)
+    default: return -1;
+  }
+#undef JM_RLNI
+  return 0;
+}
+
 constexpr int LN_BWD_CUS = 256;
 int ln_bwd_blocks_per_cu(int V) { return V <= 1 ? 4 : V <= 4 ? 3 : 2; }
 
@@ -693,9 +803,11 @@
 int jm_layernorm_bwd(const void* dy, int dy_bf16, const float* x, long sB, long sT, int B, int T, int D,
                      const float* mean, const float* rstd, const float* gamma, float* dx_ptr, long oB, long oT,
                      const float* dres, long rB, long rT, float* dgamma, float* dbeta, int accum_params, float* ws,
-                     const JmLnRes* res, hipStream_t st, const uint16_t* hx, const float* beta) {
+                     const JmLnRes* res, hipStream_t st, const uint16_t* hx, const float* beta, const int* inv,
+                     long invB, int Nm) {
   if (hx != nullptr && beta == nullptr) return -3;
-  const LnBwdIO dx{dx_ptr, oB, oT, dres, rB, rT, hx, beta};
+  if (inv != nullptr && (res == nullptr || !dy_bf16 || Nm <= 0 || Nm > T)) return -4;
+  const LnBwdIO dx{dx_ptr, oB, oT, dres, rB, rT, hx, beta, inv, invB, Nm};
   const int V = pick_v(D);
   if (V < 0 || (D % 4) != 0) return -1;
   const int rows = B * T;
@@ -728,7 +840,14 @@
   float* wsk = ws;
   LnResIO rio{nullptr, nullptr, 0, 0, nullptr, nullptr, 0, JmDrop{nullptr, 0u, 1.f, 0}};
   if (res) rio = LnResIO{res->y, res->dy, res->yB, res->yT, res->scale, res->mask, res->T0, res->drop};
-  if (dy_bf16) {
+  if (inv != nullptr) {
+    if (res->scale)
+      launch_bwd<uint16_t, true, true, true>(V, grid, smem, st, (const uint16_t*)dy, x, sB, sT, T, rows, D, mean, rstd,
+                                             gamma, dx, rio, wsk, accum_params, outs);
+    else
+      launch_bwd<uint16_t, true, false, true>(V, grid, smem, st, (const uint16_t*)dy, x, sB, sT, T, rows, D, mean,
+                                              rstd, gamma, dx, rio, wsk, accum_params, outs);
+  } else if (dy_bf16) {
     if (res && res->scale)
       launch_bwd<uint16_t, true>(V, grid, smem, st, (const uint16_t*)dy, x, sB, sT, T, rows, D, mean, rstd, gamma,
                                  dx, rio, wsk, accum_params, outs);
diff --git a/jumbo_mae_tpu_amd/csrc/mae.hip b/jumbo_mae_tpu_amd/csrc/mae.hip
--- a/jumbo_mae_tpu_amd/csrc/mae.hip
+++ b/jumbo_mae_tpu_amd/csrc/mae.hip
@@ -332,13 +332,29 @@
   }
 }
 
+struct MseRows {
+  const int* idx;
+  long idsB;
+  int Nm, C;
+};
+
+JM_DEVICE long mse_image_row(const MseRows& mr, long row, int N) {
+  if (mr.idx == nullptr) return row;
+  const long b = row / mr.Nm;
+  int n = mr.idx[b * mr.idsB + (row - b * mr.Nm)] - mr.C;
+  JM_DASSERT(n >= 0 && n < N);
+  n = min(max(n, 0), N - 1);
+  return b * N + n;
+}
+
 template <int NJ, bool P16>
 __global__ __launch_bounds__(256) void patch_mse_fwd_kernel(const uint16_t* __restrict__ pred, long ldp,
                                                             const uint8_t* __restrict__ img, float* __restrict__ mse,
                                                             long rows, int N, int H, int W, int p, int norm_pix,
-                                                            int vec) {
+                                                            int vec, MseRows mr) {
   const long row = (long)blockIdx.x * 4 + (threadIdx.x >> 6);
   if (row >= rows) return;
+  const long irow = mse_image_row(mr, row, N);
   const int P3 = 3 * p * p;
   __shared__ __attribute__((aligned(16))) uint8_t pix[4][64 * NJ];
   double t[NJ];
@@ -346,7 +362,7 @@
   if constexpr (P16) {
     float f[12];
     p16_load_pred(pred + row * ldp + 12 * lane, f, vec & P16_PRED);
-    p16_target(img, row, N, H, W, norm_pix != 0, vec & P16_IMG, pix[threadIdx.x >> 6], t);
+    p16_target(img, irow, N, H, W, norm_pix != 0, vec & P16_IMG, pix[threadIdx.x >> 6], t);
     double s = 0.0;
 #pragma unroll
     for (int j = 0; j < 12; ++j) s += (t[j] - (double)f[j]) * (t[j] - (double)f[j]);
@@ -354,7 +370,7 @@
     if (lane == 0) mse[row] = (float)(s / 768.0);
     return;
   }
-  patch_target<NJ>(img, row, N, H, W, p, P3, norm_pix != 0, pix[threadIdx.x >> 6], t);
+  patch_target<NJ>(img, irow, N, H, W, p, P3, norm_pix != 0, pix[threadIdx.x >> 6], t);
   double s = 0.0;
 #pragma unroll
   for (int j = 0; j < NJ; ++j) {
@@ -373,9 +389,10 @@
                                                             const uint8_t* __restrict__ img,
                                                             const float* __restrict__ dmse, uint16_t* __restrict__ dpred,
                                                             long rows, int N, int H, int W, int p, int norm_pix,
-                                                            int vec) {
+                                                            int vec, MseRows mr) {
   const long row = (long)blockIdx.x * 4 + (threadIdx.x >> 6);
   if (row >= rows) return;
+  const long irow = mse_image_row(mr, row, N);
   const int P3 = 3 * p * p;
   const int lane = threadIdx.x & 63;
   const float gsc = dmse[row];
@@ -397,7 +414,7 @@
     }
     float f[12];
     p16_load_pred(pred + row * ldp + 12 * lane, f, pv);
-    p16_target(img, row, N, H, W, norm_pix != 0, vec & P16_IMG, pix[threadIdx.x >> 6], t);
+    p16_target(img, irow, N, H, W, norm_pix != 0, vec & P16_IMG, pix[threadIdx.x >> 6], t);
     const double k = 2.0 * (double)gsc / 768.0;
     float r[12];
 #pragma unroll
@@ -416,7 +433,7 @@
     for (int o = lane; o < P3; o += 64) dpred[row * P3 + o] = 0;
     return;
   }
-  patch_target<NJ>(img, row, N, H, W, p, P3, norm_pix != 0, pix[threadIdx.x >> 6], t);
+  patch_target<NJ>(img, irow, N, H, W, p, P3, norm_pix != 0, pix[threadIdx.x >> 6], t);
   const double k = 2.0 * (double)gsc / P3;
 #pragma unroll
   for (int j = 0; j < NJ; ++j) {
@@ -474,38 +491,43 @@
 }
 
 int jm_patch_mse_fwd(const uint16_t* pred, long ldp, const uint8_t* img, float* mse, long rows, int N, int H, int W,
-                     int p, int norm_pix, hipStream_t st) {
+                     int p, int norm_pix, hipStream_t st, const int* idx, long idsB, int Nm, int C) {
   const int P3 = 3 * p * p;
   if (H % p || W % p || P3 > 64 * 16) return -1;
+  if (idx != nullptr && (Nm <= 0 || Nm > N || C < 0)) return -2;
+  const MseRows mr{idx, idsB, Nm, C};
   const int nb = cdiv(rows, 4);
   if (nb == 0) return 0;
   if (p == 16) {
     const int vec = (ldp % 4 == 0 && aligned(pred, 8) ? P16_PRED : 0) | (aligned(img, 16) ? P16_IMG : 0);
-    patch_mse_fwd_kernel<12, true><<<nb, 256, 0, st>>>(pred, ldp, img, mse, rows, N, H, W, p, norm_pix, vec);
+    patch_mse_fwd_kernel<12, true><<<nb, 256, 0, st>>>(pred, ldp, img, mse, rows, N, H, W, p, norm_pix, vec, mr);
   } else if (P3 <= 64 * 4)
-    patch_mse_fwd_kernel<4, false><<<nb, 256, 0, st>>>(pred, ldp, img, mse, rows, N, H, W, p, norm_pix, 0);
+    patch_mse_fwd_kernel<4, false><<<nb, 256, 0, st>>>(pred, ldp, img, mse, rows, N, H, W, p, norm_pix, 0, mr);
   else if (P3 <= 64 * 12)
-    patch_mse_fwd_kernel<12, false><<<nb, 256, 0, st>>>(pred, ldp, img, mse, rows, N, H, W, p, norm_pix, 0);
-  else patch_mse_fwd_kernel<16, false><<<nb, 256, 0, st>>>(pred, ldp, img, mse, rows, N, H, W, p, norm_pix, 0);
+    patch_mse_fwd_kernel<12, false><<<nb, 256, 0, st>>>(pred, ldp, img, mse, rows, N, H, W, p, norm_pix, 0, mr);
+  else patch_mse_fwd_kernel<16, false><<<nb, 256, 0, st>>>(pred, ldp, img, mse, rows, N, H, W, p, norm_pix, 0, mr);
   return 0;
 }
 
 int jm_patch_mse_bwd(const uint16_t* pred, long ldp, const uint8_t* img, const float* dmse, uint16_t* dpred, long rows,
-                     int N, int H, int W, int p, int norm_pix, hipStream_t st) {
+                     int N, int H, int W, int p, int norm_pix, hipStream_t st, const int* idx, long idsB, int Nm,
+                     int C) {
   const int P3 = 3 * p * p;
   if (H % p || W % p || P3 > 64 * 16) return -1;
+  if (idx != nullptr && (Nm <= 0 || Nm > N || C < 0)) return -2;
+  const MseRows mr{idx, idsB, Nm, C};
   const int nb = cdiv(rows, 4);
   if (nb == 0) return 0;
   if (p == 16) {
     const int vec =
         (ldp % 4 == 0 && aligned(pred, 8) && aligned(dpred, 8) ? P16_PRED : 0) | (aligned(img, 16) ? P16_IMG : 0);
-    patch_mse_bwd_kernel<12, true><<<nb, 256, 0, st>>>(pred, ldp, img, dmse, dpred, rows, N, H, W, p, norm_pix, vec);
+    patch_mse_bwd_kernel<12, true><<<nb, 256, 0, st>>>(pred, ldp, img, dmse, dpred, rows, N, H, W, p, norm_pix, vec, mr);
   } else if (P3 <= 64 * 4)
-    patch_mse_bwd_kernel<4, false><<<nb, 256, 0, st>>>(pred, ldp, img, dmse, dpred, rows, N, H, W, p, norm_pix, 0);
+    patch_mse_bwd_kernel<4, false><<<nb, 256, 0, st>>>(pred, ldp, img, dmse, dpred, rows, N, H, W, p, norm_pix, 0, mr);
   else if (P3 <= 64 * 12)
-    patch_mse_bwd_kernel<12, false><<<nb, 256, 0, st>>>(pred, ldp, img, dmse, dpred, rows, N, H, W, p, norm_pix, 0);
+    patch_mse_bwd_kernel<12, false><<<nb, 256, 0, st>>>(pred, ldp, img, dmse, dpred, rows, N, H, W, p, norm_pix, 0, mr);
   else
-    patch_mse_bwd_kernel<16, false><<<nb, 256, 0, st>>>(pred, ldp, img, dmse, dpred, rows, N, H, W, p, norm_pix, 0);
+    patch_mse_bwd_kernel<16, false><<<nb, 256, 0, st>>>(pred, ldp, img, dmse, dpred, rows, N, H, W, p, norm_pix, 0, mr);
   return 0;
 }
 
@@ -636,4 +658,29 @@
   return 0;
 }
 
+namespace {
+__global__ __launch_bounds__(256) void mask_rows_kernel(const float* __restrict__ mask, int N, int C, int Nm,
+                                                        int* __restrict__ rows, int* __restrict__ inv) {
+  __shared__ int f[1024];
+  const long r = blockIdx.x;
+  for (int i = threadIdx.x; i < N; i += 256) f[i] = mask[r * N + i] > 0.f ? 1 : 0;
+  for (int j = threadIdx.x; j < Nm; j += 256) rows[r * Nm + j] = C;
+  for (int t = threadIdx.x; t < C; t += 256) inv[r * (C + N) + t] = -1;
+  __syncthreads();
+  for (int i = threadIdx.x; i < N; i += 256) {
+    int pos = 0;
+    for (int j = 0; j < i; ++j) pos += f[j];
+    const bool m = f[i] && pos < Nm;
+    if (m) rows[r * Nm + pos] = C + i;
+    inv[r * (C + N) + C + i] = m ? pos : -1;
+  }
+}
+}
+
+int jm_mask_rows(const float* mask, int R, int N, int C, int Nm, int* rows, int* inv, hipStream_t st) {
+  if (N > 1024 || N <= 0 || Nm <= 0 || Nm > N || C < 0 || R <= 0) return -1;
+  mask_rows_kernel<<<R, 256, 0, st>>>(mask, N, C, Nm, rows, inv);
+  return 0;
+}
+
 JM_DEBUG_EXPORT(mae)
diff --git a/jumbo_mae_tpu_amd/models/mae.py b/jumbo_mae_tpu_amd/models/mae.py
--- a/jumbo_mae_tpu_amd/models/mae.py
+++ b/jumbo_mae_tpu_amd/models/mae.py
@@ -7,6 +7,7 @@
 from ..data.constants import IMAGENET_DEFAULT_MEAN, IMAGENET_DEFAULT_STD
 from ..ops import attn_stats as AS
 from ..ops import mae as mae_ops
+from ..ops import prims as P
 from ..utils.mae import masking_ids
 from .params import ParamStore, trunc_normal_
 from .vit import Dense, JumboViT, MAEDecoder, cls_features
@@ -49,8 +50,20 @@
             noise = torch.rand(shape, generator=noise_rng, device=self.device)
         return masking_ids(noise, self.cfg.keep_len)
 
+    def _prune(self, images_u8: torch.Tensor) -> bool:
+        from .vit import use_fused_blocks
+        dc, cfg = self.dec_cfg, self.cfg
+        return (P._DEC_PRUNE_OURS and P._FUSE_LN_RES and P.hip(images_u8) and use_fused_blocks()
+                and mae_ops.compact_rows_ok(images_u8, self.store.compute_dtype, cfg.patch_size, cfg.seq_patches)
+                and AS._COLLECTOR is None and dc.dec_dropout == 0.0 and not dc.grad_ckpt
+                and 0 < cfg.keep_len < cfg.seq_patches and len(self.decoder.layers) > 0)
+
     def _predict(self, images_u8: torch.Tensor, rngs: dict, det: bool, enc_det: bool,
                  noise: torch.Tensor | None):
+        return self._decode(images_u8, rngs, det, enc_det, noise, False)[:3]
+
+    def _decode(self, images_u8: torch.Tensor, rngs: dict, det: bool, enc_det: bool,
+                noise: torch.Tensor | None, prune: bool):
         cfg = self.cfg
         B = images_u8.shape[0]
         C = cfg.num_cls_tokens
@@ -63,16 +76,22 @@
         h = self.encoder.norm(x)
         y = self.decoder_proj(h).view(B, C + K, -1)
         dec_in = mae_ops.unshuffle_fused(y, self.mask_token, ids_restore, self.decoder.posemb_table(y.device), C)
+        if prune and self._prune(images_u8):
+            rows = mae_ops.masked_rows(mask, C, N - K)
+            xd = self.decoder.blocks(dec_in, drop, det=det, rows=rows)
+            pred = self.decoder_image_output(self.decoder.dec_norm(xd))
+            return pred.view(B, N - K, -1), mask, (ids_shuffle, ids_restore, ids_keep), rows[0]
         xd = self.decoder.blocks(dec_in, drop, det=det)
         hd = self.decoder.dec_norm(xd, row0=C)
         pred = self.decoder_image_output(hd)
-        return pred.view(B, N, -1), mask, (ids_shuffle, ids_restore, ids_keep)
+        return pred.view(B, N, -1), mask, (ids_shuffle, ids_restore, ids_keep), None
 
     def forward(self, images_u8: torch.Tensor, rngs: dict | None = None, det: bool = False,
                 noise: torch.Tensor | None = None, per_sample: bool = False) -> dict:
-        pred, mask, _ = self._predict(images_u8, rngs or {}, det, False, noise)
-        per_patch = mae_ops.patch_mse(pred, images_u8, self.cfg.patch_size, self.norm_pix_loss)
-        loss = mae_ops.masked_mean_loss(per_patch, mask, per_sample)
+        pred, mask, _, rows = self._decode(images_u8, rngs or {}, det, False, noise, True)
+        per_patch = mae_ops.patch_mse(pred, images_u8, self.cfg.patch_size, self.norm_pix_loss, rows,
+                                      self.cfg.num_cls_tokens)
+        loss = mae_ops.masked_mean_loss(per_patch, mask, per_sample, compact=rows is not None)
         return {"loss": loss}
 
     __call__ = forward
diff --git a/jumbo_mae_tpu_amd/models/vit.py b/jumbo_mae_tpu_amd/models/vit.py
--- a/jumbo_mae_tpu_amd/models/vit.py
+++ b/jumbo_mae_tpu_amd/models/vit.py
@@ -266,14 +266,15 @@
     def dropout_rate(self):
         return self.attn.dropout
 
-    def __call__(self, x, rng=None, det=True, link_in=None, link_out=None, masks=None, seeds=None):
+    def __call__(self, x, rng=None, det=True, link_in=None, link_out=None, masks=None, seeds=None, rows=None):
         B, S, D = x.shape
         p = self.droppath
         sd = seeds if seeds is not None else _layer_seeds(self.attn.dropout, rng, x.device, det, 4)
         if use_fused_blocks() and self.attn.dropout < 1.0:
             m1 = _mask(masks, 0, p, B, rng, x.device, det)
             m2 = _mask(masks, 1, p, B, rng, x.device, det)
-            return blocks.vit_block(self, x, m1, m2, link_in, link_out, _drops(sd, self.attn.dropout, False))
+            return blocks.vit_block(self, x, m1, m2, link_in, link_out, _drops(sd, self.attn.dropout, False), rows)
+        assert rows is None, "row pruning needs the fused block"
         h = self.norm1(x)
         a = self.attn(h, B, S, rng, det, sd and sd[0:2])
         x = Fn.residual(x, a, self.scale1, _mask(masks, 0, p, B, rng, x.device, det))
@@ -351,7 +352,7 @@
     return h.reshape(B, C * cfg.dim)
 
 
-def _run_layers(layers, x, rng, det, grad_ckpt, in_dropout=0.0):
+def _run_layers(layers, x, rng, det, grad_ckpt, in_dropout=0.0, last_rows=None):
     masks = droppath_masks(layers, x.shape[0], rng, x.device, det)
     x, seeds = dropout_seed_pool(layers, rng, x.device, det, head=(x, in_dropout))
     if grad_ckpt and torch.is_grad_enabled():
@@ -365,7 +366,10 @@
             up = layers[i + 1] if i + 1 < len(layers) else None
             ln1 = (up.norm1.g, up.norm1.b) if up is not None and blocks.FWD_LINKS else None
             nxt = blocks.Link(ln1)
-        x = layer(x, rng, det, link_in=link, link_out=nxt, masks=masks[i], seeds=seeds[i])
+        if last_rows is not None and i + 1 == len(layers):
+            x = layer(x, rng, det, link_in=link, link_out=nxt, masks=masks[i], seeds=seeds[i], rows=last_rows)
+        else:
+            x = layer(x, rng, det, link_in=link, link_out=nxt, masks=masks[i], seeds=seeds[i])
         link = nxt
     return x
 
@@ -409,8 +413,9 @@
             self._posemb_cache[key] = fixed_sincos2d_embeddings(g, g, self.cfg.dec_dim, device).reshape(g * g, -1)
         return self._posemb_cache[key]
 
-    def blocks(self, x, rng=None, det=True):
-        return _run_layers(self.layers, x, rng, det, self.cfg.grad_ckpt)
+    def blocks(self, x, rng=None, det=True, rows=None):
+        assert rows is None or not (self.cfg.grad_ckpt or self.cfg.dec_dropout > 0.0)
+        return _run_layers(self.layers, x, rng, det, self.cfg.grad_ckpt, last_rows=rows)
 
 
 class LinearCLS:
diff --git a/jumbo_mae_tpu_amd/ops/blocks.py b/jumbo_mae_tpu_amd/ops/blocks.py
--- a/jumbo_mae_tpu_amd/ops/blocks.py
+++ b/jumbo_mae_tpu_amd/ops/blocks.py
@@ -218,13 +218,17 @@
 
 class ViTBlockFn(torch.autograd.Function):
     @staticmethod
-    def forward(ctx, x, anchor, layer, m1, m2, link_in, link_out, train=True, dr=None):
+    def forward(ctx, x, anchor, layer, m1, m2, link_in, link_out, train=True, dr=None, rows=None):
         B, S, D = x.shape
         dt = layer.norm1.g.store.compute_dtype
         h1, mu1, rs1 = _ln1_fwd(x, layer, link_in, dt)
         qkv, o, lse, a = _attn_fwd(layer.attn, h1, B, S, dr)
-        x1, h2, mu2, rs2 = P.residual_ln_fwd(x, a, layer.scale1, m1, layer.norm2.g, layer.norm2.b, 0,
-                                             drop=_od(dr, "wo", a))
+        if rows is not None:
+            assert dr is None and (link_out is None or link_out.ln1 is None)
+            x1, h2, mu2, rs2 = P.residual_ln_fwd_rows(x, a, layer.scale1, m1, layer.norm2.g, layer.norm2.b, rows[0])
+        else:
+            x1, h2, mu2, rs2 = P.residual_ln_fwd(x, a, layer.scale1, m1, layer.norm2.g, layer.norm2.b, 0,
+                                                 drop=_od(dr, "wo", a))
         fpre, fg, fy, fd = _ff_fwd(layer.ff, h2, train, dr.rate if dr is not None else 0.0, dr and dr.fh,
                                    dr and dr.fo)
         nl = link_out.ln1 if link_out is not None else None
@@ -239,7 +243,8 @@
         ctx.gelu_deriv = (False, fd)
         ctx.gelu_rate = dr.rate if dr is not None else 0.0
         ctx.dr = dr
-        if link_out is not None:
+        ctx.inv = rows[1] if rows is not None else None
+        if link_out is not None and rows is None:
             link_out.spec = P.ResSpec(fy, layer.scale2, m2, layer.ff.w2.b, 0, drop=_od(dr, "fo", fy))
         return x2
 
@@ -247,7 +252,7 @@
     def backward(ctx, dx2):
         with P.paired_wgrads():
             dx = _vit_bwd(ctx, dx2)
-        return dx, None, None, None, None, None, None, None, None
+        return dx, None, None, None, None, None, None, None, None, None
 
 
 def _vit_bwd(ctx, dx2):
@@ -263,15 +268,19 @@
     else:
         dfy, bd = P.residual_bwd(dx2, fy, layer.scale2, m2, dt, layer.ff.w2.b, drop=_od(dr, "fo", fy))
     dh2 = _ff_bwd(layer.ff, dfy, h2, fpre, fg, bd, deriv=ctx.gelu_deriv[1], rate=ctx.gelu_rate)
-    dx1, da, bd = P.ln_bwd(dh2, x1, mu2, rs2, layer.norm2.g, layer.norm2.b, dres=dx2,
-                           res=P.ResSpec(a, layer.scale1, m1, layer.attn.wo_b, drop=_od(dr, "wo", a)), h=h2)
+    if ctx.inv is not None:
+        dx1, da, bd = P.ln_bwd_rows(dh2, x1, mu2, rs2, layer.norm2.g, layer.norm2.b, dx2, ctx.inv,
+                                    P.ResSpec(a, layer.scale1, m1, layer.attn.wo_b), h=h2)
+    else:
+        dx1, da, bd = P.ln_bwd(dh2, x1, mu2, rs2, layer.norm2.g, layer.norm2.b, dres=dx2,
+                               res=P.ResSpec(a, layer.scale1, m1, layer.attn.wo_b, drop=_od(dr, "wo", a)), h=h2)
     dh1 = _attn_bwd(layer.attn, da, h1, qkv, o, lse, B, S, bd, dr)
     return _ln1_bwd(ctx, dh1, x, mu1, rs1, layer, dx1, h1)
 
 
 def vit_block(layer, x, m1=None, m2=None, link_in: Link | None = None, link_out: Link | None = None,
-              dr: Drops | None = None):
+              dr: Drops | None = None, rows=None):
     _note_uses(layer.norm1.g, layer.norm1.b, layer.norm2.g, layer.norm2.b, layer.scale1, layer.scale2,
                *_attn_handles(layer.attn), *_ff_handles(layer.ff))
     return ViTBlockFn.apply(x.contiguous(), layer.norm1.g.param, layer, m1, m2, link_in, link_out,
-                            torch.is_grad_enabled(), dr)
+                            torch.is_grad_enabled(), dr, rows)
diff --git a/jumbo_mae_tpu_amd/ops/mae.py b/jumbo_mae_tpu_amd/ops/mae.py
--- a/jumbo_mae_tpu_amd/ops/mae.py
+++ b/jumbo_mae_tpu_amd/ops/mae.py
@@ -154,34 +154,55 @@
 class _PatchMSE(torch.autograd.Function):
 
     @staticmethod
-    def forward(ctx, pred, images_u8, patch_size, norm_pix):
+    def forward(ctx, pred, images_u8, patch_size, norm_pix, rows=None, num_cls=0):
         B = images_u8.shape[0]
         pred2 = pred.reshape(-1, pred.shape[-1])
-        mse = _ext.load().patch_mse_fwd(pred2, images_u8.contiguous(), patch_size, norm_pix)
+        mse = _ext.load().patch_mse_fwd(pred2, images_u8.contiguous(), patch_size, norm_pix, rows, num_cls)
         ctx.save_for_backward(pred2, images_u8)
         ctx.p, ctx.norm_pix, ctx.pshape = patch_size, norm_pix, pred.shape
+        ctx.rows, ctx.num_cls = rows, num_cls
         return mse.view(B, -1)
 
     @staticmethod
     def backward(ctx, dmse):
         pred2, images_u8 = ctx.saved_tensors
         dpred = _ext.load().patch_mse_bwd(pred2, images_u8.contiguous(), dmse.reshape(-1).contiguous().float(),
-                                          ctx.p, ctx.norm_pix)
-        return dpred.view(ctx.pshape), None, None, None
-
-
-def patch_mse(pred: torch.Tensor, images_u8: torch.Tensor, patch_size: int, norm_pix_loss: bool) -> torch.Tensor:
+                                          ctx.p, ctx.norm_pix, ctx.rows, ctx.num_cls)
+        return dpred.view(ctx.pshape), None, None, None, None, None
+
+
+def compact_rows_ok(images_u8: torch.Tensor, dtype, patch_size: int, n_patches: int) -> bool:
+    return (_ext.use_hip(images_u8) and dtype == torch.bfloat16 and 3 * patch_size * patch_size <= 1024
+            and n_patches <= 1024)
+
+
+def masked_rows(mask: torch.Tensor, num_cls: int, n_masked: int):
+    rows, inv = _ext.load().mask_rows(mask.float().contiguous(), num_cls, n_masked)
+    return rows, inv
+
+
+def patch_mse(pred: torch.Tensor, images_u8: torch.Tensor, patch_size: int, norm_pix_loss: bool,
+              rows: torch.Tensor | None = None, num_cls: int = 0) -> torch.Tensor:
     B = images_u8.shape[0]
     fits = 3 * patch_size * patch_size <= 1024
     if fits and _ext.use_hip(pred) and pred.dtype == torch.bfloat16 and pred.stride(-1) == 1:
-        return _PatchMSE.apply(pred, images_u8, patch_size, bool(norm_pix_loss))
+        return _PatchMSE.apply(pred, images_u8, patch_size, bool(norm_pix_loss), rows, num_cls)
+    if rows is not None:
+        raise RuntimeError("patch_mse: compact rows need the HIP kernel (bf16 pred, 3 p^2 <= 1024)")
     t = normalized_patches(images_u8, patch_size)
     if norm_pix_loss:
         t = norm_pix(t)
     return (t - pred.float().view(B, t.shape[1], -1)).square().mean(-1)
 
 
-def masked_mean_loss(per_patch: torch.Tensor, mask: torch.Tensor, per_sample: bool = False) -> torch.Tensor:
+def masked_mean_loss(per_patch: torch.Tensor, mask: torch.Tensor, per_sample: bool = False,
+                     compact: bool = False) -> torch.Tensor:
+    if compact:
+        msum = mask.sum(-1)
+        if per_sample:
+            return per_patch.sum(-1) / msum
+        n = mask.shape[-1]
+        return ((per_patch.sum(-1) / n) / (msum / n)).mean()
     if mask.dim() == 1:
         mask = mask.unsqueeze(0).expand_as(per_patch)
     if per_sample:
diff --git a/jumbo_mae_tpu_amd/ops/prims.py b/jumbo_mae_tpu_amd/ops/prims.py
--- a/jumbo_mae_tpu_amd/ops/prims.py
+++ b/jumbo_mae_tpu_amd/ops/prims.py
@@ -125,6 +125,7 @@
 _KNN_OURS = True
 _NORMS_OURS = True
 _ATTN_STATS_OURS = True
+_DEC_PRUNE_OURS = True
 
 
 NARROW_MAX_M = 4096
@@ -520,6 +521,25 @@
     return dx, dyr, done
 
 
+def ln_bwd_rows(dy: torch.Tensor, x1c: torch.Tensor, mean, rstd, hg: Handle, hb: Handle, dres: torch.Tensor,
+                inv: torch.Tensor, res: ResSpec, h: torch.Tensor | None = None):
+    B = x1c.shape[0]
+    tr = _trainable(hg)
+    hx = h if (_LN_BWD_FROM_H and h is not None and h.dtype == torch.bfloat16 and h.is_contiguous()) else None
+    hs, hbias = res.hs, res.hbias
+    dseed, drate, dioff = _drop_args(res.y, res.drop)
+    dx, dyr = _ext.load().layernorm_bwd_rows(
+        dy.contiguous(), x1c, mean, rstd, hg.master, hg.grad, hb.grad, tr, dres.contiguous(), inv, B, res.y,
+        hs.master if hs is not None else None, res.mask, hs.grad if _trainable(hs) else None,
+        hbias.grad if _trainable(hbias) else None, dseed, drate, dioff, hx, hb.master if hx is not None else None)
+    if tr:
+        hg.ready()
+        hb.ready()
+    if _trainable(hs):
+        hs.ready()
+    return dx, dyr, _trainable(hbias)
+
+
 def residual_fwd(x3: torch.Tensor, y2: torch.Tensor, hs: Handle | None, mask, out=None, drop=None) -> torch.Tensor:
     B, T, D = x3.shape
     if hip(x3):
@@ -559,6 +579,16 @@
         residual_fwd(x3[:, r0:], y2, hs, mask, out=x1[:, r0:], drop=drop)
     h, mean, rstd = ln_fwd(x1[:, t0:], hg, hb, hg.store.compute_dtype)
     return x1, h, mean, rstd
+
+
+def residual_ln_fwd_rows(x3: torch.Tensor, y2: torch.Tensor, hs: Handle | None, mask, hg: Handle, hb: Handle,
+                         rows: torch.Tensor, drop=None):
+    B, T, D = x3.shape
+    if drop is not None:
+        assert y2.data_ptr() == drop[2].data_ptr() and y2.numel() == drop[2].numel()
+    return tuple(_ext.load().residual_ln_fwd_rows(x3, y2.reshape(B * T, D), hs.master if hs is not None else None,
+                                                  mask, hg.master, hb.master, LN_EPS, rows,
+                                                  drop[0] if drop else None, drop[1] if drop else 0.0))
 
 
 def residual_bwd(dout3: torch.Tensor, y2: torch.Tensor | None, hs: Handle | None, mask, ydtype,
```

Measured after the change: 6730 images/sec (median of 6 runs). About the same (+0.6%).
